# gitouni/Spatial-Temporal-LiDAR-camera-Calibration

Measured on NVIDIA B200. Metric: extrinsic_cost_evals_per_s, higher is better.
Workload: dtype f64

## Files before the change

include/stlcalib.h:

```cpp
#ifndef STLCALIB_H_
#define STLCALIB_H_

#include <stdint.h>

#ifdef __cplusplus
extern "C" {
#endif

#define STL_ABI_VERSION 2
#define STL_MAX_COVIS 10

typedef enum stl_status {
    STL_OK = 0,
    STL_ERR_INVALID = 1,
    STL_ERR_CUDA = 2,
    STL_ERR_NO_DEVICE = 3,
    STL_ERR_STATE = 4,
    STL_ERR_CAPACITY = 5
} stl_status_t;

typedef struct stl_params {
    double max_pixel_dist;
    double corr_3d_2d_threshold;
    double corr_3d_3d_threshold;
// ... 38 lines not shown
    const double *he_Tl;
    const uint8_t *he_valid;
} stl_pack_t;

typedef struct stl_eval_sums {
    double sum_3d2d;
    double sum_3d3d;
    double sum_he;
    double cnt_he;
    double cnt_3d2d;
    double valid_3d2d;
    double cnt_3d3d;
    double valid_3d3d;
    double valid_pl;
    double valid_pt;
    double n_frames;
    double n_corr;
} stl_eval_sums_t;
#define STL_EVAL_NSUMS 12

typedef struct stl_ba_error {
    double f1;
    double f2;
    double C;
    int32_t valid_cnt_3d_2d;
    int32_t cnt_3d_2d;
} stl_ba_error_t;

typedef struct stl_lin_sums {
    double cost;
    double g[7];
    double H[49];
    double n_blocks_2d;
    double n_blocks_pt;
    double n_blocks_pl;
    double n_residuals;
    double n_blocks_gpr;
} stl_lin_sums_t;
#define STL_LIN_NSUMS 62

typedef struct stl_step_sums {
    stl_eval_sums_t eval;
    stl_lin_sums_t lin;
} stl_step_sums_t;
#define STL_STEP_NSUMS (STL_EVAL_NSUMS + STL_LIN_NSUMS)

typedef struct stl_ctx stl_ctx_t;


void stl_default_params(stl_params_t *p);

stl_status_t stl_create(const stl_params_t *params, int32_t device, stl_ctx_t **out);
void stl_destroy(stl_ctx_t *ctx);
const char *stl_last_error(const stl_ctx_t *ctx);
int32_t stl_abi_version(void);

stl_status_t stl_upload_pack(stl_ctx_t *ctx, const stl_pack_t *pack);

stl_status_t stl_allow_oversize_keyframes(stl_ctx_t *ctx, int32_t allow);

stl_status_t stl_oversize_keyframes(stl_ctx_t *ctx, int32_t *kf, int32_t cap, int32_t *n);


stl_status_t stl_eval_batch(stl_ctx_t *ctx, const double *x, int32_t B, stl_eval_sums_t *sums);

stl_status_t stl_eval_batch_device(stl_ctx_t *ctx, const double *x, int32_t B, double *d_sums,
                                   void *stream);

void stl_finalize(const stl_params_t *params, const stl_eval_sums_t *sums, stl_ba_error_t *out);

void stl_bbo(const stl_params_t *params, const stl_ba_error_t *e, double bbo[4]);


stl_status_t stl_associate(stl_ctx_t *ctx, const double *x0, int64_t n_blocks[4]);

stl_status_t stl_linearize_batch(stl_ctx_t *ctx, const double *x, int32_t B, stl_lin_sums_t *out);
stl_status_t stl_linearize_batch_device(stl_ctx_t *ctx, const double *x, int32_t B, double *d_out,
                                        void *stream);

stl_status_t stl_eval_blocks(stl_ctx_t *ctx, const double *x, int32_t rmax, int64_t cap_blocks, int32_t *type, int32_t *kf,
                             int32_t *kp, int32_t *n_res, double *residuals, double *jacobians, int64_t *n_blocks_out);

stl_status_t stl_gpr_nlml(const double *x, const double *y, int32_t n, double sigma_noise, double sigma, double l, int32_t flavour,
                          double *cost, double grad[2]);
stl_status_t stl_gpr_fit(const double *x, const double *y, int32_t n, double sigma_noise, double sigma0, double l0, int32_t max_iter,
                         int32_t flavour, double out[6]);
stl_status_t stl_gpr_hyper(stl_ctx_t *ctx, double *sigma_l, int64_t cap_blocks);

stl_status_t stl_block_counts(stl_ctx_t *ctx, int64_t n_blocks[4]);

#define STL_MAX_PROBLEMS 256

stl_status_t stl_associate_multi(stl_ctx_t *ctx, const double *x0, int32_t P, const uint8_t *rebuild, int64_t *n_blocks);
stl_status_t stl_block_counts_multi(stl_ctx_t *ctx, int64_t *n_blocks, int32_t cap_problems);

stl_status_t stl_linearize_multi(stl_ctx_t *ctx, const double *x, int32_t B, const int32_t *problem, stl_lin_sums_t *out);
stl_status_t stl_linearize_multi_device(stl_ctx_t *ctx, const double *x, int32_t B, const int32_t *problem, double *d_out, void *stream);

stl_status_t stl_step_multi(stl_ctx_t *ctx, const double *x, int32_t P, const uint8_t *rebuild, stl_step_sums_t *out);
stl_status_t stl_step_multi_device(stl_ctx_t *ctx, const double *x, int32_t P, const uint8_t *rebuild, double *d_out, void *stream);

stl_status_t stl_step_batch(stl_ctx_t *ctx, const double *x, int32_t B, int32_t reassociate, stl_step_sums_t *out);
stl_status_t stl_step_batch_device(stl_ctx_t *ctx, const double *x, int32_t B, int32_t reassociate, double *d_out, void *stream);

typedef struct stl_he_edges {
    int32_t n;
    const double *Ta;
    const double *Tb;
    const double *info;
    double huber_delta;
    double regulation;
} stl_he_edges_t;
stl_status_t stl_he_linearize(stl_ctx_t *ctx, const stl_he_edges_t *edges, const double *x, int32_t B, stl_lin_sums_t *out, double *chi2);

typedef struct stl_calib_edges {
    int32_t n_kf;
    int64_t n_edges;
    const int64_t *edge_offset;
    const double *Tlw_quat;
    const float *intrinsics;
    const double *Xw;
    const double *obs;
    const float *inv_sigma2;
    const uint8_t *level;
    double huber_delta;
} stl_calib_edges_t;
stl_status_t stl_calib_linearize(stl_ctx_t *ctx, const stl_calib_edges_t *edges, const double *x, int32_t B, stl_lin_sums_t *out, double *chi2);

#define STL_COMM_ID_BYTES 128
stl_status_t stl_comm_unique_id(uint8_t id[STL_COMM_ID_BYTES]);
stl_status_t stl_comm_init(stl_ctx_t *ctx, const uint8_t id[STL_COMM_ID_BYTES], int32_t rank, int32_t n_ranks);
stl_status_t stl_comm_info(stl_ctx_t *ctx, int32_t *rank, int32_t *n_ranks);
stl_status_t stl_comm_stats(stl_ctx_t *ctx, int64_t out[3]);

stl_status_t stl_select_keyframes(stl_ctx_t *ctx, const int32_t *kf, int32_t n);

stl_status_t stl_eval_frames(stl_ctx_t *ctx, const double *x, int32_t B, double *out);


stl_status_t stl_debug_corrset(stl_ctx_t *ctx, int32_t b, int32_t kf, uint32_t *kp_idx,
                               uint32_t *pt_idx, int32_t cap, int32_t *n);

stl_status_t stl_debug_align(stl_ctx_t *ctx, int32_t b, int32_t kf, uint32_t *kp_idx,
                             uint32_t *nn_idx, int32_t *n_neigh, int32_t *is_plane, double *dist,
                             uint32_t *knn_idx, int32_t cap, int32_t *n);

stl_status_t stl_debug_frame(stl_ctx_t *ctx, int32_t b, int32_t kf, double out[13]);

stl_status_t stl_knn3d(stl_ctx_t *ctx, int32_t kf, const double *q, int32_t nq, int32_t k,
                       double radius2, uint32_t *out_idx, double *out_d2, int32_t *out_count);

stl_status_t stl_debug_trig(stl_ctx_t *ctx, const double *x, int32_t n, double *acos_out, double *cos_out);


#define STL_STAGE_ASSOC2D 0
#define STL_STAGE_KNN3D 1
#define STL_STAGE_REDUCE 2
#define STL_STAGE_LINEARIZE 3
#define STL_STAGE_BUILD 4
#define STL_STAGE_ASSOC_LM 5
#define STL_STAGE_ALLREDUCE 6
#define STL_STAGE_PLANE_INDEX 7
#define STL_NSTAGES 8

stl_status_t stl_set_stream(stl_ctx_t *ctx, void *stream);

stl_status_t stl_set_profiling(stl_ctx_t *ctx, int32_t enabled);
stl_status_t stl_stage_stats(stl_ctx_t *ctx, double ms[STL_NSTAGES], int64_t launches[STL_NSTAGES]);

stl_status_t stl_work_counters(stl_ctx_t *ctx, double out[8]);

#ifdef __cplusplus
}
#endif
#endif
```

spatial-temporal-lidar-camera-calibration_b200/_abi.py:

```python
from __future__ import annotations

import ctypes as C
import os

_HERE = os.path.dirname(os.path.abspath(__file__))

STL_MAX_COVIS = 10
STL_EVAL_NSUMS = 12
STL_LIN_NSUMS = 62
STL_STEP_NSUMS = STL_EVAL_NSUMS + STL_LIN_NSUMS
STL_COMM_ID_BYTES = 128
STL_MAX_PROBLEMS = 256
STL_NSTAGES = 8
STAGE_NAMES = ("assoc2d", "knn3d", "reduce", "linearize", "build", "assoc_lm", "allreduce", "plane_index")

STATUS = {0: "STL_OK", 1: "STL_ERR_INVALID", 2: "STL_ERR_CUDA", 3: "STL_ERR_NO_DEVICE",
          4: "STL_ERR_STATE", 5: "STL_ERR_CAPACITY"}


class StlError(RuntimeError):
    def __init__(self, code: int, msg: str = ""):
        self.code = code
        super().__init__(f"{STATUS.get(code, code)}: {msg}")


class Params(C.Structure):
    _fields_ = [
        ("max_pixel_dist", C.c_double),
        ("corr_3d_2d_threshold", C.c_double),
        ("corr_3d_3d_threshold", C.c_double),
        ("norm_radius", C.c_double),
        ("norm_reg_threshold", C.c_double),
        ("min_diff_dist", C.c_double),
        ("err_weight", C.c_double * 2),
        ("he_threshold", C.c_double),
        ("valid_rate", C.c_double),
        ("max_3d_dist", C.c_double),
        ("robust_kernel_delta", C.c_double),
        ("robust_kernel_3ddelta", C.c_double),
        ("num_min_corr", C.c_int32),
        ("norm_max_pts", C.c_int32),
        ("norm_min_pts", C.c_int32),
        ("use_plane", C.c_int32),
        ("use_gpr", C.c_int32),
        ("gpr_sigma", C.c_double),
        ("gpr_l", C.c_double),
        ("gpr_sigma_noise", C.c_double),
        ("plane_index", C.c_int32),
        ("variant", C.c_int32),
        ("gpr_optimize", C.c_int32),
        ("gpr_grad_flavour", C.c_int32),
    ]


class Pack(C.Structure):
    _fields_ = [
        ("n_kf", C.c_int32),
        ("n_covis", C.c_int32),
        ("scan_offset", C.POINTER(C.c_int64)),
        ("scan_xyz", C.POINTER(C.c_float)),
        ("intrinsics", C.POINTER(C.c_float)),
        ("image_wh", C.POINTER(C.c_int32)),
        ("kp_offset", C.POINTER(C.c_int64)),
        ("kp_xy", C.POINTER(C.c_float)),
        ("kp_mappoint", C.POINTER(C.c_float)),
        ("Tcw", C.POINTER(C.c_float)),
        ("covis_relpose", C.POINTER(C.c_float)),
        ("covis_valid", C.POINTER(C.c_uint8)),
        ("covis_uv", C.POINTER(C.c_float)),
        ("he_Tc", C.POINTER(C.c_float)),
        ("he_Tl", C.POINTER(C.c_double)),
        ("he_valid", C.POINTER(C.c_uint8)),
    ]


class EvalSums(C.Structure):
    _fields_ = [(n, C.c_double) for n in (
        "sum_3d2d", "sum_3d3d", "sum_he", "cnt_he", "cnt_3d2d", "valid_3d2d", "cnt_3d3d",
        "valid_3d3d", "valid_pl", "valid_pt", "n_frames", "n_corr")]


class BAErrorOut(C.Structure):
    _fields_ = [("f1", C.c_double), ("f2", C.c_double), ("C", C.c_double),
                ("valid_cnt_3d_2d", C.c_int32), ("cnt_3d_2d", C.c_int32)]


class LinSums(C.Structure):
    _fields_ = [("cost", C.c_double), ("g", C.c_double * 7), ("H", C.c_double * 49),
                ("n_blocks_2d", C.c_double), ("n_blocks_pt", C.c_double),
                ("n_blocks_pl", C.c_double), ("n_residuals", C.c_double), ("n_blocks_gpr", C.c_double)]


class StepSums(C.Structure):
    _fields_ = [("eval", EvalSums), ("lin", LinSums)]


class HeEdges(C.Structure):
    _fields_ = [("n", C.c_int32), ("Ta", C.POINTER(C.c_double)), ("Tb", C.POINTER(C.c_double)), ("info", C.POINTER(C.c_double)),
                ("huber_delta", C.c_double), ("regulation", C.c_double)]


class CalibEdges(C.Structure):
    _fields_ = [("n_kf", C.c_int32), ("n_edges", C.c_int64), ("edge_offset", C.POINTER(C.c_int64)), ("Tlw_quat", C.POINTER(C.c_double)),
                ("intrinsics", C.POINTER(C.c_float)), ("Xw", C.POINTER(C.c_double)), ("obs", C.POINTER(C.c_double)),
                ("inv_sigma2", C.POINTER(C.c_float)), ("level", C.POINTER(C.c_uint8)), ("huber_delta", C.c_double)]


class SynthCfg(C.Structure):
    _fields_ = [
        ("n_kf", C.c_int32), ("kf_begin", C.c_int32), ("n_kf_total", C.c_int32),
        ("beams", C.c_int32), ("az_steps", C.c_int32), ("n_kp", C.c_int32), ("n_covis", C.c_int32),
        ("width", C.c_int32), ("height", C.c_int32),
        ("fx", C.c_float), ("fy", C.c_float), ("cx", C.c_float), ("cy", C.c_float),
        ("anchored_frac", C.c_double), ("mappoint_frac", C.c_double), ("match_frac", C.c_double),
        ("outlier_frac", C.c_double), ("scale_gt", C.c_double), ("kf_spacing", C.c_double),
        ("max_range", C.c_double), ("elev_top_deg", C.c_double), ("elev_bottom_deg", C.c_double),
        ("x_gt", C.c_double * 7), ("seed", C.c_uint64),
    ]


_vp = C.c_void_p
_dp = C.POINTER(C.c_double)
_u32p = C.POINTER(C.c_uint32)
_i32p = C.POINTER(C.c_int32)
_i64p = C.POINTER(C.c_int64)
_u8p = C.POINTER(C.c_uint8)

CALIB_SYMBOLS = {
    "stl_default_params": (None, [C.POINTER(Params)]),
    "stl_create": (C.c_int, [C.POINTER(Params), C.c_int32, C.POINTER(_vp)]),
    "stl_destroy": (None, [_vp]),
    "stl_last_error": (C.c_char_p, [_vp]),
    "stl_abi_version": (C.c_int32, []),
    "stl_upload_pack": (C.c_int, [_vp, C.POINTER(Pack)]),
    "stl_eval_batch": (C.c_int, [_vp, _dp, C.c_int32, C.POINTER(EvalSums)]),
    "stl_eval_batch_device": (C.c_int, [_vp, _dp, C.c_int32, _vp, _vp]),
    "stl_finalize": (None, [C.POINTER(Params), C.POINTER(EvalSums), C.POINTER(BAErrorOut)]),
    "stl_bbo": (None, [C.POINTER(Params), C.POINTER(BAErrorOut), _dp]),
    "stl_associate": (C.c_int, [_vp, _dp, _i64p]),
    "stl_linearize_batch": (C.c_int, [_vp, _dp, C.c_int32, C.POINTER(LinSums)]),
    "stl_linearize_batch_device": (C.c_int, [_vp, _dp, C.c_int32, _vp, _vp]),
    "stl_eval_blocks": (C.c_int, [_vp, _dp, C.c_int32, C.c_int64, _i32p, _i32p, _i32p, _i32p, _dp, _dp, C.POINTER(C.c_int64)]),
    "stl_block_counts": (C.c_int, [_vp, _i64p]),
    "stl_gpr_nlml": (C.c_int, [_dp, _dp, C.c_int32, C.c_double, C.c_double, C.c_double, C.c_int32, _dp, _dp]),
    "stl_gpr_fit": (C.c_int, [_dp, _dp, C.c_int32, C.c_double, C.c_double, C.c_double, C.c_int32, C.c_int32, _dp]),
    "stl_gpr_hyper": (C.c_int, [_vp, _dp, C.c_int64]),
    "stl_step_batch": (C.c_int, [_vp, _dp, C.c_int32, C.c_int32, C.POINTER(StepSums)]),
    "stl_step_batch_device": (C.c_int, [_vp, _dp, C.c_int32, C.c_int32, _vp, _vp]),
    "stl_associate_multi": (C.c_int, [_vp, _dp, C.c_int32, _u8p, _i64p]),
    "stl_block_counts_multi": (C.c_int, [_vp, _i64p, C.c_int32]),
    "stl_linearize_multi": (C.c_int, [_vp, _dp, C.c_int32, _i32p, C.POINTER(LinSums)]),
    "stl_linearize_multi_device": (C.c_int, [_vp, _dp, C.c_int32, _i32p, _vp, _vp]),
    "stl_step_multi": (C.c_int, [_vp, _dp, C.c_int32, _u8p, C.POINTER(StepSums)]),
    "stl_step_multi_device": (C.c_int, [_vp, _dp, C.c_int32, _u8p, _vp, _vp]),
    "stl_he_linearize": (C.c_int, [_vp, C.POINTER(HeEdges), _dp, C.c_int32, C.POINTER(LinSums), _dp]),
    "stl_calib_linearize": (C.c_int, [_vp, C.POINTER(CalibEdges), _dp, C.c_int32, C.POINTER(LinSums), _dp]),
    "stl_comm_unique_id": (C.c_int, [C.POINTER(C.c_uint8)]),
    "stl_comm_init": (C.c_int, [_vp, C.POINTER(C.c_uint8), C.c_int32, C.c_int32]),
    "stl_comm_info": (C.c_int, [_vp, _i32p, _i32p]),
    "stl_comm_stats": (C.c_int, [_vp, _i64p]),
    "stl_select_keyframes": (C.c_int, [_vp, _i32p, C.c_int32]),
    "stl_eval_frames": (C.c_int, [_vp, _dp, C.c_int32, _dp]),
    "stl_allow_oversize_keyframes": (C.c_int, [_vp, C.c_int32]),
    "stl_oversize_keyframes": (C.c_int, [_vp, _i32p, C.c_int32, _i32p]),
    "stl_debug_corrset": (C.c_int, [_vp, C.c_int32, C.c_int32, _u32p, _u32p, C.c_int32, _i32p]),
    "stl_debug_align": (C.c_int, [_vp, C.c_int32, C.c_int32, _u32p, _u32p, _i32p, _i32p, _dp, _u32p,
                                  C.c_int32, _i32p]),
    "stl_debug_frame": (C.c_int, [_vp, C.c_int32, C.c_int32, _dp]),
    "stl_debug_trig": (C.c_int, [_vp, _dp, C.c_int32, _dp, _dp]),
    "stl_knn3d": (C.c_int, [_vp, C.c_int32, _dp, C.c_int32, C.c_int32, C.c_double, _u32p, _dp, _i32p]),
    "stl_set_stream": (C.c_int, [_vp, _vp]),
    "stl_set_profiling": (C.c_int, [_vp, C.c_int32]),
    "stl_stage_stats": (C.c_int, [_vp, _dp, _i64p]),
    "stl_work_counters": (C.c_int, [_vp, _dp]),
}

SYNTH_SYMBOLS = {
    "stl_synth_default_cfg": (None, [C.POINTER(SynthCfg)]),
    "stl_synth_create": (_vp, [C.POINTER(SynthCfg)]),
    "stl_synth_pack": (C.POINTER(Pack), [_vp]),
    "stl_synth_x_gt": (_dp, [_vp]),
    "stl_synth_Twl": (_dp, [_vp]),
    "stl_synth_destroy": (None, [_vp]),
    "stl_synth_candidates": (None, [_dp, C.c_uint64, C.c_int32, C.c_double, _dp]),
}


def _bind(lib, table):
    for name, (res, args) in table.items():
        fn = getattr(lib, name)
        fn.restype = res
        fn.argtypes = args
    return lib


CALIB_LIB_PATH = os.path.join(_HERE, "libstlcalib.so")
SYNTH_LIB_PATH = os.path.join(_HERE, "libstlsynth.so")

_calib = None
_synth = None


def load_calib():
    global _calib
    if _calib is None:
        if not os.path.exists(CALIB_LIB_PATH):
            raise ImportError(
                f"{CALIB_LIB_PATH} is not built; run `python -c 'import __graft_entry__ as g; g.build()'`."
                " There is no CPU fallback for the cost-evaluation path.")
        _calib = _bind(C.CDLL(CALIB_LIB_PATH), CALIB_SYMBOLS)
    return _calib


def load_synth():
    global _synth
    if _synth is None:
        if not os.path.exists(SYNTH_LIB_PATH):
            raise ImportError(f"{SYNTH_LIB_PATH} is not built; run __graft_entry__.build()")
        _synth = _bind(C.CDLL(SYNTH_LIB_PATH), SYNTH_SYMBOLS)
    return _synth
```

spatial-temporal-lidar-camera-calibration_b200/capi.py:

```python
from __future__ import annotations

import ctypes as C

import numpy as np

from . import _abi
from .pack import KeyFramePack, default_params

_dp = _abi._dp


def _check(lib, h, code):
    if code != 0:
        msg = lib.stl_last_error(h).decode() if h else ""
        raise _abi.StlError(code, msg)


class Context:

    def __init__(self, params: _abi.Params | None = None, device: int = 0):
        self.lib = _abi.load_calib()
        self.params = params if params is not None else default_params()
        h = C.c_void_p()
        code = self.lib.stl_create(C.byref(self.params), device, C.byref(h))
# ... 162 lines not shown
        return nb if wait else None

    def block_counts_multi(self) -> np.ndarray:
        nb = np.zeros((_abi.STL_MAX_PROBLEMS, 4), np.int64)
        _check(self.lib, self.h, self.lib.stl_block_counts_multi(self.h, nb.ctypes.data_as(_abi._i64p), _abi.STL_MAX_PROBLEMS))
        return nb[: self.n_problems].copy()

    def linearize_multi(self, X, problem=None) -> np.ndarray:
        X = np.ascontiguousarray(np.atleast_2d(X), dtype=np.float64)
        B = X.shape[0]
        keep, pp = self._problems(problem, B)
        out = np.empty((B, _abi.STL_LIN_NSUMS), dtype=np.float64)
        _check(self.lib, self.h, self.lib.stl_linearize_multi(self.h, X.ctypes.data_as(_dp), B, pp,
                                                              out.ctypes.data_as(C.POINTER(_abi.LinSums))))
        return out

    def linearize_multi_device(self, X, d_out_ptr: int, problem=None, stream_ptr: int = 0):
        X = np.ascontiguousarray(np.atleast_2d(X), dtype=np.float64)
        keep, pp = self._problems(problem, X.shape[0])
        _check(self.lib, self.h, self.lib.stl_linearize_multi_device(self.h, X.ctypes.data_as(_dp), X.shape[0], pp,
                                                                     C.c_void_p(d_out_ptr), C.c_void_p(stream_ptr)))

    def step_multi(self, X, rebuild=None) -> np.ndarray:
        X = np.ascontiguousarray(np.atleast_2d(X), dtype=np.float64)
        P = X.shape[0]
        keep, m = self._mask(rebuild, P)
        out = np.empty((P, _abi.STL_STEP_NSUMS), dtype=np.float64)
        _check(self.lib, self.h, self.lib.stl_step_multi(self.h, X.ctypes.data_as(_dp), P, m, out.ctypes.data_as(C.POINTER(_abi.StepSums))))
        self.n_blocks = None
        self.n_problems = P
        return out

    def step_multi_device(self, X, d_out_ptr: int, rebuild=None, stream_ptr: int = 0):
        X = np.ascontiguousarray(np.atleast_2d(X), dtype=np.float64)
        keep, m = self._mask(rebuild, X.shape[0])
        _check(self.lib, self.h, self.lib.stl_step_multi_device(self.h, X.ctypes.data_as(_dp), X.shape[0], m,
                                                                C.c_void_p(d_out_ptr), C.c_void_p(stream_ptr)))
        self.n_blocks = None
        self.n_problems = X.shape[0]

    def gpr_hyper(self):
        nb = self.block_counts()
        out = np.zeros((max(int(nb[3]), 1), 2))
        _check(self.lib, self.h, self.lib.stl_gpr_hyper(self.h, out.ctypes.data_as(_dp), int(nb[3])))
        return out[: int(nb[3])]

    def he_linearize(self, edges: "HandEyeEdges", x, want_chi2: bool = False):
        x = np.ascontiguousarray(np.atleast_2d(x), dtype=np.float64)
        B = x.shape[0]
        out = np.zeros((B, _abi.STL_LIN_NSUMS))
        chi2 = np.zeros((B, max(edges.n, 1))) if want_chi2 else None
        c = edges.as_c()
        _check(self.lib, self.h, self.lib.stl_he_linearize(self.h, C.byref(c), x.ctypes.data_as(_dp), B, out.ctypes.data_as(C.POINTER(_abi.LinSums)),
                                                           chi2.ctypes.data_as(_dp) if want_chi2 else None))
        return (out, chi2[:, : edges.n]) if want_chi2 else out

    def calib_linearize(self, edges: "CalibBAEdges", x, want_chi2: bool = False):
        x = np.ascontiguousarray(np.atleast_2d(x), dtype=np.float64)
        B = x.shape[0]
        out = np.zeros((B, _abi.STL_LIN_NSUMS))
        chi2 = np.zeros((B, max(edges.n_edges, 1))) if want_chi2 else None
        c = edges.as_c()
        _check(self.lib, self.h, self.lib.stl_calib_linearize(self.h, C.byref(c), x.ctypes.data_as(_dp), B, out.ctypes.data_as(C.POINTER(_abi.LinSums)),
                                                              chi2.ctypes.data_as(_dp) if want_chi2 else None))
        return (out, chi2[:, : edges.n_edges]) if want_chi2 else out

    def comm_unique_id(self) -> bytes:
        buf = (C.c_uint8 * _abi.STL_COMM_ID_BYTES)()
        _check(self.lib, self.h, self.lib.stl_comm_unique_id(buf))
        return bytes(buf)

    def comm_init(self, uid: bytes, rank: int, n_ranks: int):
        buf = (C.c_uint8 * _abi.STL_COMM_ID_BYTES).from_buffer_copy(uid)
        _check(self.lib, self.h, self.lib.stl_comm_init(self.h, buf, rank, n_ranks))

    def comm_stats(self):
        out = np.zeros(3, np.int64)
        _check(self.lib, self.h, self.lib.stl_comm_stats(self.h, out.ctypes.data_as(_abi._i64p)))
        return dict(p2p=bool(out[0]), p2p_exchanges=int(out[1]), nccl_exchanges=int(out[2]))

    def comm_info(self):
        r, n = C.c_int32(0), C.c_int32(1)
        _check(self.lib, self.h, self.lib.stl_comm_info(self.h, C.byref(r), C.byref(n)))
        return r.value, n.value

    def linearize(self, x) -> np.ndarray:
        x = np.ascontiguousarray(np.atleast_2d(x), dtype=np.float64)
        B = x.shape[0]
        out = np.empty((B, _abi.STL_LIN_NSUMS), dtype=np.float64)
        _check(self.lib, self.h, self.lib.stl_linearize_batch(self.h, x.ctypes.data_as(_dp), B,
                                                              out.ctypes.data_as(C.POINTER(_abi.LinSums))))
        return out

    def linearize_device(self, x, d_out_ptr: int, stream_ptr: int = 0):
        x = np.ascontiguousarray(np.atleast_2d(x), dtype=np.float64)
        _check(self.lib, self.h, self.lib.stl_linearize_batch_device(self.h, x.ctypes.data_as(_dp), x.shape[0],
                                                                     C.c_void_p(d_out_ptr), C.c_void_p(stream_ptr)))

    def eval_blocks(self, x, rmax: int = 0):
        x = np.ascontiguousarray(x, dtype=np.float64).reshape(7)
        ncov = int(self.pack.n_covis) if self.pack is not None else _abi.STL_MAX_COVIS
        rmax = int(rmax) if rmax else max(3, 2 * ncov)
        if getattr(self, "n_blocks", None) is None:
            self.block_counts()
        nb = int(self.n_blocks.sum())
        cap = max(nb, 1)
        out = dict(type=np.zeros(cap, np.int32), kf=np.zeros(cap, np.int32), kp=np.zeros(cap, np.int32), n_res=np.zeros(cap, np.int32),
                   residuals=np.zeros((cap, rmax)), jacobians=np.zeros((cap, rmax, 7)))
        n = C.c_int64(0)
        _check(self.lib, self.h, self.lib.stl_eval_blocks(
            self.h, x.ctypes.data_as(_dp), rmax, cap, out["type"].ctypes.data_as(_abi._i32p), out["kf"].ctypes.data_as(_abi._i32p),
            out["kp"].ctypes.data_as(_abi._i32p), out["n_res"].ctypes.data_as(_abi._i32p), out["residuals"].ctypes.data_as(_dp),
            out["jacobians"].ctypes.data_as(_dp), C.byref(n)))
        return {k: v[: n.value] for k, v in out.items()}

    def debug_corrset(self, b: int, kf: int):
        cap = int(self.pack.kp_offset[kf + 1] - self.pack.kp_offset[kf]) if self.pack is not None else 65536
        kp = np.zeros(max(cap, 1), np.uint32)
        pt = np.zeros(max(cap, 1), np.uint32)
        n = C.c_int32(0)
        _check(self.lib, self.h, self.lib.stl_debug_corrset(self.h, b, kf, kp.ctypes.data_as(_abi._u32p),
                                                            pt.ctypes.data_as(_abi._u32p), cap, C.byref(n)))
        return kp[:n.value], pt[:n.value]

    def debug_align(self, b: int, kf: int):
        cap = int(self.pack.kp_offset[kf + 1] - self.pack.kp_offset[kf]) if self.pack is not None else 65536
        cap = max(cap, 1)
        kp = np.zeros(cap, np.uint32)
        nn = np.zeros(cap, np.uint32)
        m = np.zeros(cap, np.int32)
        pl = np.zeros(cap, np.int32)
        d = np.zeros(cap, np.float64)
        knn = np.zeros((cap, 32), np.uint32)
        n = C.c_int32(0)
        _check(self.lib, self.h, self.lib.stl_debug_align(
            self.h, b, kf, kp.ctypes.data_as(_abi._u32p), nn.ctypes.data_as(_abi._u32p), m.ctypes.data_as(_abi._i32p),
            pl.ctypes.data_as(_abi._i32p), d.ctypes.data_as(_dp), knn.ctypes.data_as(_abi._u32p), cap, C.byref(n)))
        k = n.value
        return dict(kp=kp[:k], nn=nn[:k], m=m[:k], is_plane=pl[:k], dist=d[:k], knn=knn[:k])

    def debug_frame(self, b: int, kf: int):
        out = np.zeros(13)
        _check(self.lib, self.h, self.lib.stl_debug_frame(self.h, b, kf, out.ctypes.data_as(_dp)))
        names = ("sum_3d2d", "valid_3d2d", "cnt_3d2d", "sum_he", "cnt_he", "kept", "n_corr", "n_queries",
                 "sum_3d3d", "valid_3d3d", "cnt_3d3d", "valid_pl", "valid_pt")
        return dict(zip(names, out))

    def debug_trig(self, x):
        x = np.ascontiguousarray(x, dtype=np.float64).reshape(-1)
        a, c = np.zeros_like(x), np.zeros_like(x)
        _check(self.lib, self.h, self.lib.stl_debug_trig(self.h, x.ctypes.data_as(_dp), len(x), a.ctypes.data_as(_dp), c.ctypes.data_as(_dp)))
        return a, c

    def knn3d(self, kf: int, q, k: int, radius2: float = 0.0):
        q = np.ascontiguousarray(q, dtype=np.float64).reshape(-1, 3)
        nq = q.shape[0]
        idx = np.zeros((nq, k), np.uint32)
        d2 = np.zeros((nq, k), np.float64)
        cnt = np.zeros(nq, np.int32)
        _check(self.lib, self.h, self.lib.stl_knn3d(self.h, kf, q.ctypes.data_as(_dp), nq, k, radius2,
                                                    idx.ctypes.data_as(_abi._u32p), d2.ctypes.data_as(_dp),
                                                    cnt.ctypes.data_as(_abi._i32p)))
        return idx, d2, cnt

    def set_stream(self, stream_ptr: int = 0):
        _check(self.lib, self.h, self.lib.stl_set_stream(self.h, C.c_void_p(stream_ptr)))

    def set_profiling(self, on: bool):
        _check(self.lib, self.h, self.lib.stl_set_profiling(self.h, int(on)))

    def stage_stats(self):
        ms = np.zeros(_abi.STL_NSTAGES)
        n = np.zeros(_abi.STL_NSTAGES, np.int64)
        _check(self.lib, self.h, self.lib.stl_stage_stats(self.h, ms.ctypes.data_as(_dp), n.ctypes.data_as(_abi._i64p)))
        return {name: (float(ms[i]), int(n[i])) for i, name in enumerate(_abi.STAGE_NAMES)}

    def work_counters(self):
        out = np.zeros(8)
        _check(self.lib, self.h, self.lib.stl_work_counters(self.h, out.ctypes.data_as(_dp)))
        return dict(points=out[0], q2d=out[1], q3d_nn=out[2], q3d_knn=out[3], k1_bytes=out[4], launches=out[5], k1_overflow_units=out[6],
                    assoc_reused=out[7])


class HandEyeEdges:

    def __init__(self, Ta, Tb, info=None, huber_delta: float = 0.0, regulation: float = 0.0):
        self.Ta = np.ascontiguousarray(Ta, dtype=np.float64).reshape(-1, 12)
        self.Tb = np.ascontiguousarray(Tb, dtype=np.float64).reshape(-1, 12)
        self.n = len(self.Ta)
        self.info = None if info is None else np.ascontiguousarray(info, dtype=np.float64)
        self.huber_delta, self.regulation = float(huber_delta), float(regulation)

    def as_c(self):
        c = _abi.HeEdges(self.n, self.Ta.ctypes.data_as(_dp), self.Tb.ctypes.data_as(_dp),
                         self.info.ctypes.data_as(_dp) if self.info is not None else None, self.huber_delta, self.regulation)
        c._keep = self
        return c


class CalibBAEdges:

    def __init__(self, edge_offset, Tlw_quat, intrinsics, Xw, obs, inv_sigma2, level=None, huber_delta: float = 5.991 ** 0.5):
        self.edge_offset = np.ascontiguousarray(edge_offset, dtype=np.int64)
        self.Tlw_quat = np.ascontiguousarray(Tlw_quat, dtype=np.float64).reshape(-1, 6)
        self.intrinsics = np.ascontiguousarray(intrinsics, dtype=np.float32).reshape(-1, 4)
        self.Xw = np.ascontiguousarray(Xw, dtype=np.float64).reshape(-1, 3)
        self.obs = np.ascontiguousarray(obs, dtype=np.float64).reshape(-1, 2)
        self.inv_sigma2 = np.ascontiguousarray(inv_sigma2, dtype=np.float32)
        self.level = None if level is None else np.ascontiguousarray(level, dtype=np.uint8)
        self.n_kf, self.n_edges = len(self.Tlw_quat), len(self.Xw)
        self.huber_delta = float(huber_delta)

    def as_c(self):
        c = _abi.CalibEdges(self.n_kf, self.n_edges, self.edge_offset.ctypes.data_as(_abi._i64p), self.Tlw_quat.ctypes.data_as(_dp),
                            self.intrinsics.ctypes.data_as(C.POINTER(C.c_float)), self.Xw.ctypes.data_as(_dp), self.obs.ctypes.data_as(_dp),
                            self.inv_sigma2.ctypes.data_as(C.POINTER(C.c_float)),
                            self.level.ctypes.data_as(C.POINTER(C.c_uint8)) if self.level is not None else None, self.huber_delta)
        c._keep = self
        return c


def gpr_nlml(x, y, sigma, l, sigma_noise: float = 1e-10, flavour: int = 0):
    lib = _abi.load_calib()
    x = np.ascontiguousarray(x, dtype=np.float64).reshape(-1, 2)
    y = np.ascontiguousarray(y, dtype=np.float64)
    cost, g = C.c_double(0), np.zeros(2)
    code = lib.stl_gpr_nlml(x.ctypes.data_as(_dp), y.ctypes.data_as(_dp), len(y), sigma_noise, sigma, l, flavour, C.byref(cost), g.ctypes.data_as(_dp))
    if code != 0:
        raise _abi.StlError(code, "Cholesky factorisation of the kernel matrix failed")
    return cost.value, g


def gpr_fit(x, y, sigma0: float = 10.0, l0: float = 10.0, sigma_noise: float = 1e-10, max_iter: int = 15, flavour: int = 0):
    lib = _abi.load_calib()
    x = np.ascontiguousarray(x, dtype=np.float64).reshape(-1, 2)
    y = np.ascontiguousarray(y, dtype=np.float64)
    out = np.zeros(6)
    code = lib.stl_gpr_fit(x.ctypes.data_as(_dp), y.ctypes.data_as(_dp), len(y), sigma_noise, sigma0, l0, max_iter, flavour, out.ctypes.data_as(_dp))
    if code != 0:
        raise _abi.StlError(code, "the objective could not be evaluated at the starting point")
    return dict(sigma=out[0], l=out[1], cost0=out[2], cost=out[3], iterations=int(out[4]), evaluations=int(out[5]))
```

spatial-temporal-lidar-camera-calibration_b200/csrc/build.cu:

```cuda
#include <cub/cub.cuh>

#include "kernels.h"

namespace stl {
namespace {

__device__ __forceinline__ unsigned long long spread16(unsigned v) {
    unsigned long long x = v & 0xffffull;
    x = (x | (x << 16)) & 0x0000ff0000ffull;
    x = (x | (x << 8)) & 0x00f00f00f00full;
    x = (x | (x << 4)) & 0x0c30c30c30c3ull;
    x = (x | (x << 2)) & 0x249249249249ull;
    return x;
}

__global__ void k_bbox(const float *__restrict__ raw, const long long *__restrict__ raw_off, float *__restrict__ bbox, DevKf *kf,
                       int kf_begin) {
    const int f = blockIdx.x;
    const long long b = raw_off[f], e = raw_off[f + 1];
    float lo[3] = {INFINITY, INFINITY, INFINITY}, hi[3] = {-INFINITY, -INFINITY, -INFINITY};
    for (long long i = b + threadIdx.x; i < e; i += blockDim.x) {
#pragma unroll
        for (int a = 0; a < 3; ++a) {
            const float v = raw[i * 3 + a];
            lo[a] = fminf(lo[a], v);
            hi[a] = fmaxf(hi[a], v);
        }
    }
    __shared__ float slo[3][32], shi[3][32];
    const int lane = threadIdx.x & 31, w = threadIdx.x >> 5;
#pragma unroll
    for (int a = 0; a < 3; ++a) {
        for (int o = 16; o; o >>= 1) {
            lo[a] = fminf(lo[a], __shfl_xor_sync(0xffffffffu, lo[a], o));
            hi[a] = fmaxf(hi[a], __shfl_xor_sync(0xffffffffu, hi[a], o));
        }
        if (lane == 0) { slo[a][w] = lo[a]; shi[a][w] = hi[a]; }
    }
    __syncthreads();
    if (threadIdx.x == 0) {
        const int nw = blockDim.x >> 5;
        float pm = 0.f;
        for (int a = 0; a < 3; ++a) {
            float l = slo[a][0], h = shi[a][0];
            for (int i = 1; i < nw; ++i) { l = fminf(l, slo[a][i]); h = fmaxf(h, shi[a][i]); }
            bbox[f * 6 + a] = l;
            bbox[f * 6 + 3 + a] = h;
            pm = fmaxf(pm, fmaxf(fabsf(l), fabsf(h)));
        }
        if (!(pm >= 1.f)) pm = 1.f;
        kf[kf_begin + f].pmax = pm;
    }
}

__global__ void k_morton(const float *__restrict__ raw, const long long *__restrict__ raw_off, const float *__restrict__ bbox,
                         unsigned long long *__restrict__ keys, uint32_t *__restrict__ vals) {
    const int f = blockIdx.y;
    const long long b = raw_off[f], e = raw_off[f + 1];
    const float lx = bbox[f * 6], ly = bbox[f * 6 + 1], lz = bbox[f * 6 + 2];
    float ext = fmaxf(fmaxf(bbox[f * 6 + 3] - lx, bbox[f * 6 + 4] - ly), bbox[f * 6 + 5] - lz);
    if (!(ext > 0.f)) ext = 1.f;
    const float scale = 65535.0f / ext;
    for (long long i = b + (long long)blockIdx.x * blockDim.x + threadIdx.x; i < e; i += (long long)gridDim.x * blockDim.x) {
        const float x = raw[i * 3], y = raw[i * 3 + 1], z = raw[i * 3 + 2];
        const unsigned qx = (unsigned)fminf(fmaxf((x - lx) * scale, 0.f), 65535.f);
        const unsigned qy = (unsigned)fminf(fmaxf((y - ly) * scale, 0.f), 65535.f);
        const unsigned qz = (unsigned)fminf(fmaxf((z - lz) * scale, 0.f), 65535.f);
        const unsigned long long m = spread16(qx) | (spread16(qy) << 1) | (spread16(qz) << 2);
        keys[i] = ((unsigned long long)f << 48) | m;
        vals[i] = (uint32_t)(i - b);
    }
}

__global__ void k_scatter(const float *__restrict__ raw, const long long *__restrict__ raw_off, const uint32_t *__restrict__ vals,
                          const DevKf *__restrict__ kf, int kf_begin, float *__restrict__ px, float *__restrict__ py,
                          float *__restrict__ pz, uint32_t *__restrict__ orig) {
    const int f = blockIdx.y;
    const DevKf K = kf[kf_begin + f];
    const long long b = raw_off[f];
    for (int j = blockIdx.x * blockDim.x + threadIdx.x; j < K.n_pad; j += gridDim.x * blockDim.x) {
        const long long dst = K.pt_off + j;
        if (j < K.n_pts) {
            const uint32_t v = vals[b + j];
            const float *p = raw + (b + v) * 3;
            px[dst] = p[0]; py[dst] = p[1]; pz[dst] = p[2];
            orig[dst] = v;
        } else {
            const float qn = __int_as_float(0x7fc00000);
            px[dst] = qn; py[dst] = qn; pz[dst] = qn;
            orig[dst] = 0xffffffffu;
        }
    }
}


constexpr int kGroup = 8192;
constexpr int kRefThreads = 1024;
constexpr int kGroupLevels = 8;

__device__ __forceinline__ int f2ord(float f) { const int b = __float_as_int(f); return b >= 0 ? b : b ^ 0x7fffffff; }

struct RefineSmem {
    float x[kGroup], y[kGroup], z[kGroup];
    uint32_t o[kGroup];
    float key[kGroup];
    unsigned short perm[kGroup];
    int bb[128][6];
    unsigned char axis[128];
};

__device__ __forceinline__ void cmp_swap(RefineSmem &S, int i, int l) {
    const float ki = S.key[i], kl = S.key[l];
    const unsigned short pi = S.perm[i], pl = S.perm[l];
    if (ki > kl || (ki == kl && pi > pl)) { S.key[i] = kl; S.key[l] = ki; S.perm[i] = pl; S.perm[l] = pi; }
}

__global__ void __launch_bounds__(kRefThreads, 1)
k_kd_refine(const DevKf *__restrict__ kf, int kf_begin, float *__restrict__ px, float *__restrict__ py, float *__restrict__ pz,
            uint32_t *__restrict__ orig) {
    extern __shared__ __align__(16) unsigned char refine_raw[];
    RefineSmem &S = *reinterpret_cast<RefineSmem *>(refine_raw);
    const DevKf K = kf[kf_begin + blockIdx.y];
    const int g0 = blockIdx.x * kGroup;
    if (g0 >= K.n_pad) return;
    const int M = min(kGroup, K.n_pad - g0);
    const long long base = K.pt_off + g0;
    const int tid = threadIdx.x;
    const float qn = __int_as_float(0x7fc00000);
    for (int i = tid; i < kGroup; i += kRefThreads) {
        const bool in = i < M;
        S.x[i] = in ? px[base + i] : qn;
        S.y[i] = in ? py[base + i] : qn;
        S.z[i] = in ? pz[base + i] : qn;
        S.o[i] = in ? orig[base + i] : 0xffffffffu;
        S.perm[i] = (unsigned short)i;
    }
    __syncthreads();
    for (int lev = 0; lev < kGroupLevels; ++lev) {
        const int seg_size = kGroup >> lev, nseg = 1 << lev, seg_shift = 13 - lev;
        for (int i = tid; i < nseg * 6; i += kRefThreads) S.bb[i / 6][i % 6] = (i % 6) < 3 ? 0x7fffffff : (int)0x80000000;
        __syncthreads();
        for (int i = tid; i < kGroup; i += kRefThreads) {
            const int p = S.perm[i];
            const float x = S.x[p];
            if (x == x) {
                const int sg = i >> seg_shift;
                atomicMin(&S.bb[sg][0], f2ord(x)); atomicMax(&S.bb[sg][3], f2ord(x));
                atomicMin(&S.bb[sg][1], f2ord(S.y[p])); atomicMax(&S.bb[sg][4], f2ord(S.y[p]));
                atomicMin(&S.bb[sg][2], f2ord(S.z[p])); atomicMax(&S.bb[sg][5], f2ord(S.z[p]));
            }
        }
        __syncthreads();
        if (tid < nseg) {
            int ax = 0;
            if (S.bb[tid][0] <= S.bb[tid][3]) {
                float e[3];
                for (int a = 0; a < 3; ++a) {
                    const int lo = S.bb[tid][a], hi = S.bb[tid][3 + a];
                    const float fl = __int_as_float(lo >= 0 ? lo : lo ^ 0x7fffffff), fh = __int_as_float(hi >= 0 ? hi : hi ^ 0x7fffffff);
                    e[a] = fh - fl;
                }
                if (e[1] > e[ax]) ax = 1;
                if (e[2] > e[ax]) ax = 2;
            }
            S.axis[tid] = (unsigned char)ax;
        }
        __syncthreads();
        for (int i = tid; i < kGroup; i += kRefThreads) {
            const int p = S.perm[i], ax = S.axis[i >> seg_shift];
            const float v = ax == 0 ? S.x[p] : (ax == 1 ? S.y[p] : S.z[p]);
            S.key[i] = (v == v) ? v : INFINITY;
        }
        __syncthreads();
        for (int k = 2; k <= seg_size; k <<= 1) {
            const int hk = k >> 1;
            for (int p = tid; p < kGroup / 2; p += kRefThreads) {
                const int i = (p / hk) * k + (p % hk);
                cmp_swap(S, i, i ^ (k - 1));
            }
            __syncthreads();
            for (int j = hk >> 1; j > 0; j >>= 1) {
                for (int p = tid; p < kGroup / 2; p += kRefThreads) {
                    const int i = (p / j) * 2 * j + (p % j);
                    cmp_swap(S, i, i + j);
                }
                __syncthreads();
            }
        }
    }
    for (int i = tid; i < M; i += kRefThreads) {
        const int p = S.perm[i];
        px[base + i] = S.x[p]; py[base + i] = S.y[p]; pz[base + i] = S.z[p];
        orig[base + i] = S.o[p];
    }
}

__device__ __forceinline__ void warp_box(float4 &lo, float4 &hi) {
    for (int o = 16; o; o >>= 1) {
        lo.x = fminf(lo.x, __shfl_xor_sync(0xffffffffu, lo.x, o));
        lo.y = fminf(lo.y, __shfl_xor_sync(0xffffffffu, lo.y, o));
        lo.z = fminf(lo.z, __shfl_xor_sync(0xffffffffu, lo.z, o));
        hi.x = fmaxf(hi.x, __shfl_xor_sync(0xffffffffu, hi.x, o));
        hi.y = fmaxf(hi.y, __shfl_xor_sync(0xffffffffu, hi.y, o));
        hi.z = fmaxf(hi.z, __shfl_xor_sync(0xffffffffu, hi.z, o));
    }
}

__global__ void k_leaf_aabb(const DevKf *__restrict__ kf, int kf_begin, const float *__restrict__ px, const float *__restrict__ py,
                            const float *__restrict__ pz, float4 *__restrict__ node_lo, float4 *__restrict__ node_hi) {
    const DevKf K = kf[kf_begin + blockIdx.y];
    const int lane = threadIdx.x & 31;
    const int leaf = blockIdx.x * (blockDim.x >> 5) + (threadIdx.x >> 5);
    if (leaf >= K.n0) return;
    float4 lo = make_float4(INFINITY, INFINITY, INFINITY, 0.f), hi = make_float4(-INFINITY, -INFINITY, -INFINITY, 0.f);
    const int j = leaf * kLeaf + lane;
    if (j < K.n_pts) {
        const long long s = K.pt_off + j;
        lo.x = hi.x = px[s]; lo.y = hi.y = py[s]; lo.z = hi.z = pz[s];
    }
    warp_box(lo, hi);
    if (lane == 0) { node_lo[K.node_off + leaf] = lo; node_hi[K.node_off + leaf] = hi; }
}

__global__ void k_inner_aabb(const DevKf *__restrict__ kf, int kf_begin, int level, float4 *__restrict__ node_lo,
                             float4 *__restrict__ node_hi) {
    const DevKf K = kf[kf_begin + blockIdx.y];
    const int lane = threadIdx.x & 31;
    const int node = blockIdx.x * (blockDim.x >> 5) + (threadIdx.x >> 5);
    const int n_here = level == 1 ? K.n1 : 32;
    if (node >= n_here) return;
    const long long child_base = K.node_off + (level == 1 ? 0 : K.n0);
    const int n_child = level == 1 ? K.n0 : K.n1;
    const long long out_base = K.node_off + (level == 1 ? K.n0 : K.n0 + K.n1);
    float4 lo = make_float4(INFINITY, INFINITY, INFINITY, 0.f), hi = make_float4(-INFINITY, -INFINITY, -INFINITY, 0.f);
    const int c = node * 32 + lane;
    if (c < n_child) { lo = node_lo[child_base + c]; hi = node_hi[child_base + c]; }
    warp_box(lo, hi);
    if (lane == 0) { node_lo[out_base + node] = lo; node_hi[out_base + node] = hi; }
}

constexpr int kAdjCand = 256;

__device__ __forceinline__ float boxbox_lb(float4 alo, float4 ahi, float4 blo, float4 bhi) {
    const float dx = fmaxf(fmaxf(__fsub_rd(blo.x, ahi.x), __fsub_rd(alo.x, bhi.x)), 0.f);
    const float dy = fmaxf(fmaxf(__fsub_rd(blo.y, ahi.y), __fsub_rd(alo.y, bhi.y)), 0.f);
    const float dz = fmaxf(fmaxf(__fsub_rd(blo.z, ahi.z), __fsub_rd(alo.z, bhi.z)), 0.f);
    const float s = __fadd_rd(__fadd_rd(__fmul_rd(dx, dx), __fmul_rd(dy, dy)), __fmul_rd(dz, dz));
    return __fmul_rd(s, 0.99999976f);
}

__device__ __forceinline__ unsigned long long warp_min64(unsigned long long v) {
    for (int o = 16; o; o >>= 1) {
        const unsigned long long w = __shfl_xor_sync(0xffffffffu, v, o);
        v = w < v ? w : v;
    }
    return v;
}

__global__ void __launch_bounds__(256)
k_leaf_adj(const DevKf *__restrict__ kf, int kf_begin, const float4 *__restrict__ node_lo, const float4 *__restrict__ node_hi,
           uint16_t *__restrict__ adj, float *__restrict__ adj_cov, const float r2, const float min_cov) {
    __shared__ unsigned long long cand[8][kAdjCand];
    constexpr unsigned long long kNone = 0xffffffffffffffffull;
    const DevKf K = kf[kf_begin + blockIdx.y];
    const int lane = threadIdx.x & 31, warp = threadIdx.x >> 5;
    const int leaf = blockIdx.x * 8 + warp;
    if (leaf >= K.n0) return;
    const float4 *lo0 = node_lo + K.node_off, *hi0 = node_hi + K.node_off;
    const float4 *lo1 = lo0 + K.n0, *hi1 = hi0 + K.n0, *lo2 = lo1 + K.n1, *hi2 = hi1 + K.n1;
    const float4 alo = lo0[leaf], ahi = hi0[leaf];
    int cnt = 0;
    bool over = !(alo.x <= ahi.x) || K.n0 > 65535;
    if (!over) {
        unsigned m2 = __ballot_sync(0xffffffffu, boxbox_lb(alo, ahi, lo2[lane], hi2[lane]) <= r2);
        while (m2 && !over) {
            const int s2 = __ffs(m2) - 1;
            m2 &= m2 - 1;
            unsigned m1 = __ballot_sync(0xffffffffu, boxbox_lb(alo, ahi, lo1[s2 * 32 + lane], hi1[s2 * 32 + lane]) <= r2);
            while (m1 && !over) {
                const int s1 = __ffs(m1) - 1;
                m1 &= m1 - 1;
                const int n0i = (s2 * 32 + s1) * 32 + lane;
                const float lb = boxbox_lb(alo, ahi, lo0[n0i], hi0[n0i]);
                const unsigned m0 = __ballot_sync(0xffffffffu, lb <= r2);
                const int c = __popc(m0);
                if (cnt + c > kAdjCand) { over = true; break; }
                if ((m0 >> lane) & 1u) cand[warp][cnt + __popc(m0 & ((1u << lane) - 1))] = ((unsigned long long)__float_as_uint(lb) << 32) | (unsigned)n0i;
                cnt += c;
            }
        }
    }
    __syncwarp();
    unsigned long long mine = kNone;
    float cov = -1.f;
    if (!over) {
        for (int t = 0; t <= 32; ++t) {
            unsigned long long best = kNone;
            for (int i = lane; i < cnt; i += 32) best = cand[warp][i] < best ? cand[warp][i] : best;
            best = warp_min64(best);
            if (t == 32) {
                cov = best == kNone ? __int_as_float(0x7f800000) : __uint_as_float((unsigned)(best >> 32));
                break;
            }
            if (best == kNone) { cov = __int_as_float(0x7f800000); break; }
            if (lane == t) mine = best;
            for (int i = lane; i < cnt; i += 32)
                if (cand[warp][i] == best) cand[warp][i] = kNone;
            __syncwarp();
        }
    }
    if (cov >= 0.f && cov < min_cov) { cov = -1.f; mine = kNone; }
    adj[(K.node_off + leaf) * 32 + lane] = mine == kNone ? (uint16_t)0xffffu : (uint16_t)(mine & 0xffffu);
    if (lane == 0) adj_cov[K.node_off + leaf] = cov;
}

}

cudaError_t build_scan_index(const float *d_raw, const long long *h_raw_off, int nkf, int kf_begin, const DevKf *h_kf, DevPack &pack,
                             float adj_r2, cudaStream_t st, BuildScratch &scr, float *kernel_ms) {
    const long long n = h_raw_off[nkf] - h_raw_off[0];
    cudaError_t err = cudaSuccess;
    cudaEvent_t ev0 = nullptr, ev1 = nullptr;
    long long *d_off = nullptr;
    float *d_bbox = nullptr;
    unsigned long long *d_keys = nullptr, *d_keys2 = nullptr;
    uint32_t *d_vals = nullptr, *d_vals2 = nullptr;
    void *d_tmp = nullptr;
    size_t tmp_bytes = 0;
    int max_pad = 0, max_n0 = 0, max_n1 = 0;
    for (int f = 0; f < nkf; ++f) {
        max_pad = max_pad > h_kf[kf_begin + f].n_pad ? max_pad : h_kf[kf_begin + f].n_pad;
        max_n0 = max_n0 > h_kf[kf_begin + f].n0 ? max_n0 : h_kf[kf_begin + f].n0;
        max_n1 = max_n1 > h_kf[kf_begin + f].n1 ? max_n1 : h_kf[kf_begin + f].n1;
    }
    long long *h_rel = (long long *)malloc(sizeof(long long) * (nkf + 1));
    for (int f = 0; f <= nkf; ++f) h_rel[f] = h_raw_off[f] - h_raw_off[0];
#define STL_TRY(x) do { err = (x); if (err != cudaSuccess) goto done; } while (0)
    STL_TRY(scr.need(0, sizeof(long long) * (nkf + 1))); d_off = (long long *)scr.buf[0];
    STL_TRY(cudaMemcpyAsync(d_off, h_rel, sizeof(long long) * (nkf + 1), cudaMemcpyHostToDevice, st));
    STL_TRY(scr.need(1, sizeof(float) * 6 * nkf)); d_bbox = (float *)scr.buf[1];
    if (n > 0) {
        STL_TRY(scr.need(2, sizeof(unsigned long long) * n)); d_keys = (unsigned long long *)scr.buf[2];
        STL_TRY(scr.need(3, sizeof(unsigned long long) * n)); d_keys2 = (unsigned long long *)scr.buf[3];
        STL_TRY(scr.need(4, sizeof(uint32_t) * n)); d_vals = (uint32_t *)scr.buf[4];
        STL_TRY(scr.need(5, sizeof(uint32_t) * n)); d_vals2 = (uint32_t *)scr.buf[5];
    }
    if (n > 0) {
        int kf_bits0 = 1;
        while ((1 << kf_bits0) < nkf) ++kf_bits0;
        STL_TRY(cub::DeviceRadixSort::SortPairs(nullptr, tmp_bytes, d_keys, d_keys2, d_vals, d_vals2, n, 0, 48 + kf_bits0, st));
        STL_TRY(scr.need(6, tmp_bytes)); d_tmp = scr.buf[6];
    }
    if (kernel_ms) {
        STL_TRY(cudaEventCreate(&ev0)); STL_TRY(cudaEventCreate(&ev1));
        STL_TRY(cudaEventRecord(ev0, st));
    }
    k_bbox<<<nkf, 512, 0, st>>>(d_raw, d_off, d_bbox, pack.kf, kf_begin);
    if (n > 0) {
        const int tiles = (max_pad + 256 * 8 - 1) / (256 * 8);
        k_morton<<<dim3(tiles, nkf), 256, 0, st>>>(d_raw, d_off, d_bbox, d_keys, d_vals);
        int kf_bits = 1;
        while ((1 << kf_bits) < nkf) ++kf_bits;
        STL_TRY(cub::DeviceRadixSort::SortPairs(d_tmp, tmp_bytes, d_keys, d_keys2, d_vals, d_vals2, n, 0, 48 + kf_bits, st));
    }
    {
        const int tiles = (max_pad + 256 * 8 - 1) / (256 * 8);
        k_scatter<<<dim3(tiles > 0 ? tiles : 1, nkf), 256, 0, st>>>(d_raw, d_off, d_vals2, pack.kf, kf_begin, pack.px, pack.py, pack.pz,
                                                                    pack.orig);
        if (max_pad > 0) {
            static bool configured = false;
            if (!configured) {
                STL_TRY(cudaFuncSetAttribute(k_kd_refine, cudaFuncAttributeMaxDynamicSharedMemorySize, (int)sizeof(RefineSmem)));
                configured = true;
            }
            k_kd_refine<<<dim3((max_pad + kGroup - 1) / kGroup, nkf), kRefThreads, sizeof(RefineSmem), st>>>(pack.kf, kf_begin, pack.px, pack.py,
                                                                                                          pack.pz, pack.orig);
        }
        k_leaf_aabb<<<dim3((max_n0 + 7) / 8, nkf), 256, 0, st>>>(pack.kf, kf_begin, pack.px, pack.py, pack.pz, pack.node_lo, pack.node_hi);
        k_inner_aabb<<<dim3((max_n1 + 7) / 8, nkf), 256, 0, st>>>(pack.kf, kf_begin, 1, pack.node_lo, pack.node_hi);
        k_inner_aabb<<<dim3(4, nkf), 256, 0, st>>>(pack.kf, kf_begin, 2, pack.node_lo, pack.node_hi);
        if (pack.adj && adj_r2 > 0.f)
            k_leaf_adj<<<dim3((max_n0 + 7) / 8, nkf), 256, 0, st>>>(pack.kf, kf_begin, pack.node_lo, pack.node_hi, pack.adj, pack.adj_cov, adj_r2,
                                                                    adj_r2 * (getenv("STL_ADJ_TRUNC") ? (float)atof(getenv("STL_ADJ_TRUNC")) : 1.f / 9.f));
    }
    STL_TRY(cudaGetLastError());
    if (kernel_ms) STL_TRY(cudaEventRecord(ev1, st));
    STL_TRY(cudaStreamSynchronize(st));
    if (kernel_ms) {
        float ms = 0.f;
        STL_TRY(cudaEventElapsedTime(&ms, ev0, ev1));
        *kernel_ms += ms;
    }
#undef STL_TRY
done:
    if (ev0) cudaEventDestroy(ev0);
    if (ev1) cudaEventDestroy(ev1);
    free(h_rel);
    return err;
}

}
```

spatial-temporal-lidar-camera-calibration_b200/csrc/capi.cu:

```cuda
#include <algorithm>
#include <cfloat>
#include <climits>
#include <cmath>
#include <cstdarg>
#include <cstdio>
#include <cstdlib>
#include <cstring>
#include <mutex>
#include <string>
#include <vector>

#include <nccl.h>

#include "../../include/stlcalib.h"
#include "gprfit.hpp"
#include "hostmath.hpp"
#include "kernels.h"
#include "lm.h"
#include "packlayout.hpp"

using namespace stl;

struct stl_ctx {
    int device = 0;
    stl_params_t params;
    DevParams dpr;
    cudaStream_t own_stream = nullptr;
    cudaStream_t stream = nullptr;
    cudaStream_t last_stream = nullptr;
    cudaEvent_t handoff = nullptr;
    cudaStream_t aux_stream = nullptr;
    cudaEvent_t ev_k1 = nullptr, ev_k2a = nullptr, ev_k3 = nullptr, ev_aux = nullptr;
    long long overlapped_steps = 0;
    long long launches = 0;
    std::mutex mu;
    std::string err;
    bool has_pack = false;
    float adj_r2 = 0.f;
    DevPack pk;
    int n_sm = 0;
    PackLayout lay;
    bool allow_oversize = false;
    OvKf *d_ov = nullptr;
    KfRoute route;
    struct DevRoute {
        int *lists = nullptr;
        int *sel = nullptr;
        int2 *sel_mp = nullptr;
        int cap = 0;
    } d_all, d_sel;
    double *d_frames = nullptr;
    DevWork wk;
    int wk_cap = 0;
    bool dbg_alloc = false;
    double *d_sums = nullptr;
    int d_sums_cap = 0;
    DevCand *h_cand = nullptr;
    double *h_sums = nullptr;
    int h_cap = 0;
    cudaEvent_t h2d_done = nullptr;
    std::vector<double> last_x;
    int dbg_b = -1;
    std::vector<double> wk_x;
    bool wk_has_nn = false;
    long long assoc_reused = 0;
    ncclComm_t comm = nullptr;
    int comm_rank = 0, comm_size = 1;
    bool p2p_on = false;
    unsigned p2p_seq = 0;
    P2pView p2p;
    double *p2p_data = nullptr;
    unsigned *p2p_flag = nullptr;
    long long p2p_exchanges = 0, nccl_exchanges = 0;
    LmState lm;
    double *d_lin = nullptr;
    double *h_lin = nullptr;
    long long lin_cap = 0;
    bool profiling = false;
    struct Ev { cudaEvent_t a, b; int stage; bool count; };
    std::vector<Ev> evs;
    std::vector<cudaEvent_t> ev_pool;
    double stage_ms[STL_NSTAGES] = {0};
    long long stage_n[STL_NSTAGES] = {0};
    double counters[8] = {0};
};

namespace {

stl_status_t fail(stl_ctx *c, stl_status_t code, const char *fmt, ...) {
    char buf[512];
    va_list ap;
    va_start(ap, fmt);
    vsnprintf(buf, sizeof(buf), fmt, ap);
    va_end(ap);
    if (c) c->err = buf;
    return code;
}

cudaStream_t acquire_stream(stl_ctx *c, void *requested) {
    cudaStream_t st = requested ? (cudaStream_t)requested : c->stream;
    if (st != c->last_stream) {
        if (c->last_stream) {
            cudaEventRecord(c->handoff, c->last_stream);
            cudaStreamWaitEvent(st, c->handoff, 0);
        }
        c->last_stream = st;
    }
    return st;
}

#define CK(call)                                                                                          \
    do {                                                                                                  \
        cudaError_t e_ = (call);                                                                          \
        if (e_ != cudaSuccess) return fail(ctx, STL_ERR_CUDA, "%s: %s (%s:%d)", #call, cudaGetErrorString(e_), __FILE__, __LINE__); \
    } while (0)

template <class T> void dfree(T *&p) { if (p) { cudaFree(p); p = nullptr; } }

void free_pack(stl_ctx *c) {
    DevPack &p = c->pk;
    dfree(p.kf); dfree(p.px); dfree(p.py); dfree(p.pz); dfree(p.orig); dfree(p.node_lo); dfree(p.node_hi); dfree(p.adj); dfree(p.adj_cov);
    dfree(p.pl_rec); dfree(p.pl_m);
    dfree(p.k1tab); dfree(p.bitmap); dfree(p.grid_start); dfree(p.grid_kp); dfree(p.kp_xy); dfree(p.kp_xyd); dfree(p.kp_mp); dfree(p.Tcw);
    dfree(p.relpose); dfree(p.covis_valid); dfree(p.covis_uv); dfree(p.he_Tc); dfree(p.he_Tl);
    p = DevPack();
    dfree(c->d_frames); dfree(c->d_ov);
    for (stl_ctx::DevRoute *d : {&c->d_all, &c->d_sel}) { dfree(d->lists); dfree(d->sel); dfree(d->sel_mp); *d = stl_ctx::DevRoute(); }
    c->lay = PackLayout();
    c->route = KfRoute();
    c->has_pack = false;
}
void free_work(stl_ctx *c) {
    DevWork &w = c->wk;
    dfree(w.cand); dfree(w.corr_kp); dfree(w.corr_pt); dfree(w.corr_sp); dfree(w.q_corr); dfree(w.q_kpsp); dfree(w.n_corr); dfree(w.n_q);
    dfree(w.k1_ticket); dfree(w.k1_rec); dfree(w.k1_match); dfree(w.k1_ov_match); dfree(w.k1_surv); dfree(w.k1_cnt); dfree(w.k1_best_d2); dfree(w.k1_best_key);
    dfree(w.frame); dfree(w.align); dfree(w.nn_pos); dfree(w.nn_g2); dfree(w.nb); dfree(w.nbx); dfree(w.nb_m); dfree(w.nb_last); dfree(w.dbg_nn); dfree(w.dbg_m); dfree(w.dbg_plane); dfree(w.dbg_dist); dfree(w.dbg_knn); dfree(w.dbg_stats);
    dfree(w.overflow); dfree(w.k1_clk);
    w = DevWork();
    dfree(c->d_frames);
    c->wk_cap = 0;
    c->dbg_alloc = false;
}

void set_dev_params(stl_ctx *c) {
    const stl_params_t &p = c->params;
    DevParams &d = c->dpr;
    d.max_pixel_dist2 = p.max_pixel_dist * p.max_pixel_dist;
    d.thr2d = p.corr_3d_2d_threshold;
    d.thr3d = p.corr_3d_3d_threshold;
    d.radius2 = p.norm_radius * p.norm_radius;
    d.reg_thr = p.norm_reg_threshold;
    d.min_diff2 = p.min_diff_dist * p.min_diff_dist;
    d.max_3d_dist2 = p.max_3d_dist * p.max_3d_dist;
    d.delta2d = p.robust_kernel_delta;
    d.delta3d = p.robust_kernel_3ddelta;
    d.w0 = p.err_weight[0];
    d.w1 = p.err_weight[1];
    d.num_min_corr = p.num_min_corr;
    d.k = p.norm_max_pts;
    d.min_pts = p.norm_min_pts;
    d.use_plane = p.use_plane;
    d.use_gpr = p.use_gpr; d.plane_index = p.plane_index;
    d.variant = p.variant; d.min_diff = p.min_diff_dist;
    c->adj_r2 = 0.f; d.adj_r = 0.f;
    if (!getenv("STL_NO_ADJ") && p.use_plane && p.norm_radius > 0 && p.norm_radius < 1e3) {
        c->adj_r2 = nextafterf((float)d.radius2, INFINITY);
        d.adj_r = nextafterf((float)sqrt(d.radius2), 0.f);
    }
    d.gpr_sigma = p.gpr_sigma; d.gpr_l = p.gpr_l; d.gpr_noise = p.gpr_sigma_noise;
}

struct StageTimer {
    stl_ctx *c; int stage; cudaStream_t st; cudaEvent_t a = nullptr, b = nullptr; bool count;
    StageTimer(stl_ctx *c_, int s, cudaStream_t st_, bool count_ = true) : c(c_), stage(s), st(st_), count(count_) {
        if (!c->profiling) return;
        auto get = [&]() { cudaEvent_t e; if (c->ev_pool.empty()) cudaEventCreate(&e); else { e = c->ev_pool.back(); c->ev_pool.pop_back(); } return e; };
        a = get(); b = get();
        cudaEventRecord(a, st);
    }
    ~StageTimer() {
        if (!a) return;
        cudaEventRecord(b, st);
        c->evs.push_back({a, b, stage, count});
    }
};

void drain_events(stl_ctx *c) {
    for (auto &e : c->evs) {
        cudaEventSynchronize(e.b);
        float ms = 0;
        if (cudaEventElapsedTime(&ms, e.a, e.b) == cudaSuccess) { c->stage_ms[e.stage] += ms; c->stage_n[e.stage] += e.count ? 1 : 0; }
        c->ev_pool.push_back(e.a);
        c->ev_pool.push_back(e.b);
    }
    c->evs.clear();
}

P2pView p2p_view(stl_ctx *ctx, int B, int off, int width) {
    P2pView v;
    if (!ctx->p2p_on || B > kP2pMaxB || width > kP2pWidth) return v;
    v = ctx->p2p;
    v.seq = ++ctx->p2p_seq;
    v.off = off; v.width = width;
    ctx->p2p_exchanges += 1;
    return v;
}

stl_status_t ensure_work(stl_ctx *ctx, int B, bool debug) {
    const DevPack &pk = ctx->pk;
    if (ctx->wk_cap == 0) {
        size_t free_b = 0, total_b = 0;
        CK(cudaMemGetInfo(&free_b, &total_b));
        const size_t per_cand = (size_t)pk.n_kp_total * 24 + (size_t)pk.n_mp_total * (20 * kMaxK + 16) + (size_t)pk.n_kf * (sizeof(FrameRec) + 4 * sizeof(AlignRec) + 24) + (size_t)pk.n_ov_match * sizeof(ulonglong2) + (size_t)pk.n_ov_surv * 4 + (size_t)pk.n_kp_total * 16 + sizeof(DevCand);
        size_t budget = std::min<size_t>((size_t)12 << 30, free_b / 4);
        int cap = (int)std::max<size_t>(1, std::min<size_t>(budget / std::max<size_t>(per_cand, 1), 256));
        if (const char *e = getenv("STL_MAX_CHUNK")) cap = std::max(1, std::min(cap, atoi(e)));
        DevWork &w = ctx->wk;
        w.Bc = cap;
        w.sub = 4;
        if (getenv("STL_SUB")) w.sub = std::max(1, std::min(16, atoi(getenv("STL_SUB"))));
        const size_t nk = (size_t)std::max<long long>(pk.n_kp_total, 1) * cap, nf = (size_t)pk.n_kf * cap;
        const size_t nm = (size_t)std::max<long long>(pk.n_mp_total, 1) * cap;
        auto alloc_all = [&]() -> cudaError_t {
            cudaError_t e;
#define A_(p, bytes) do { e = cudaMalloc(&(p), (bytes)); if (e != cudaSuccess) return e; } while (0)
            A_(w.cand, sizeof(DevCand) * cap);
            A_(w.corr_kp, 4 * nk); A_(w.corr_pt, 4 * nk); A_(w.corr_sp, 4 * nk); A_(w.q_corr, 4 * nk); A_(w.q_kpsp, 8 * nk);
            A_(w.n_corr, 4 * nf); A_(w.n_q, 4 * nf);
            if (ctx->lay.n_fit > 0) {
                w.k1_slots = 2 * std::max(ctx->n_sm, 1);
                A_(w.k1_match, sizeof(ulonglong2) * kK1MatchCap * (size_t)w.k1_slots);
                A_(w.k1_rec, sizeof(float4) * kK1SurvCap * (size_t)w.k1_slots);
                A_(w.k1_ticket, 8);
                e = cudaMemsetAsync(w.k1_ticket, 0, 8, ctx->last_stream); if (e != cudaSuccess) return e;
            }
            if (pk.n_ov > 0) {
                const size_t c = (size_t)cap;
                A_(w.k1_ov_match, sizeof(ulonglong2) * (size_t)pk.n_ov_match * c); A_(w.k1_surv, 4 * (size_t)pk.n_ov_surv * c);
                A_(w.k1_cnt, 16 * (size_t)pk.n_ov * c);
                A_(w.k1_best_d2, 8 * (size_t)std::max<long long>(pk.n_ov_kp, 1) * c); A_(w.k1_best_key, 8 * (size_t)std::max<long long>(pk.n_ov_kp, 1) * c);
            }
            A_(w.frame, sizeof(FrameRec) * nf); A_(w.align, sizeof(AlignRec) * nf * w.sub);
            A_(w.nn_pos, 4 * nm); A_(w.nn_g2, 4 * nm); A_(w.nb, 4 * nm * kMaxK); A_(w.nbx, sizeof(float4) * nm * kMaxK); A_(w.nb_m, 4 * nm); A_(w.nb_last, 8 * nm);
            w.nbx_stride = (long long)nm;
            if (getenv("STL_K1_CLK")) { A_(w.k1_clk, 64 * nf); e = cudaMemsetAsync(w.k1_clk, 0, 64 * nf, ctx->last_stream); if (e != cudaSuccess) return e; }
            A_(w.overflow, 4);
#undef A_
            return cudaMemsetAsync(w.overflow, 0, 4, ctx->last_stream);
        };
        const cudaError_t e = alloc_all();
        if (e != cudaSuccess) {
            free_work(ctx);
            return fail(ctx, STL_ERR_CUDA, "workspace allocation: %s", cudaGetErrorString(e));
        }
        ctx->wk_cap = cap;
    }
    if (debug && !ctx->dbg_alloc) {
        DevWork &w = ctx->wk;
        const size_t nk = (size_t)std::max<long long>(pk.n_kp_total, 1);
        cudaError_t e = cudaMalloc(&w.dbg_nn, 4 * nk);
        if (e == cudaSuccess) e = cudaMalloc(&w.dbg_m, 4 * nk);
        if (e == cudaSuccess) e = cudaMalloc(&w.dbg_plane, 4 * nk);
        if (e == cudaSuccess) e = cudaMalloc(&w.dbg_dist, 8 * nk);
        if (e == cudaSuccess) e = cudaMalloc(&w.dbg_knn, 4 * nk * kMaxK);
        if (e == cudaSuccess) e = cudaMalloc(&w.dbg_stats, 64);
        if (e == cudaSuccess) e = cudaMemsetAsync(w.dbg_stats, 0, 64, ctx->last_stream);
        if (e != cudaSuccess) {
            dfree(w.dbg_nn); dfree(w.dbg_m); dfree(w.dbg_plane); dfree(w.dbg_dist); dfree(w.dbg_knn); dfree(w.dbg_stats);
            return fail(ctx, STL_ERR_CUDA, "debug workspace allocation: %s", cudaGetErrorString(e));
        }
        ctx->dbg_alloc = true;
    }
    if (B > ctx->h_cap) {
        if (ctx->h_cand) cudaFreeHost(ctx->h_cand);
// ... 175 lines not shown

void use_route(stl_ctx *c, KfRoute &&r) {
    const stl_ctx::DevRoute &d = r.all ? c->d_all : c->d_sel;
    DevPack &pk = c->pk;
    pk.sel = r.all ? nullptr : d.sel; pk.sel_mp = r.all ? nullptr : d.sel_mp;
    pk.n_sel = r.n_sel; pk.n_sel_mp = r.n_sel_mp;
    pk.ov_sel = d.lists ? d.lists + pk.n_kf : nullptr; pk.n_ov_sel = r.n_ov;
    c->route = std::move(r);
}

void drop_selection_state(stl_ctx *c) {
    c->lm.ready = false;
    c->wk_x.clear();
    c->wk_has_nn = false;
    c->last_x.clear();
    c->dbg_b = -1;
}

bool kf_selected(const stl_ctx *c, int kf) { return c->route.mask[(size_t)kf] != 0; }

stl_status_t run_debug(stl_ctx *ctx, int b) {
    if (!ctx->has_pack) return fail(ctx, STL_ERR_STATE, "no pack uploaded");
    if (b < 0 || (size_t)b * 7 + 7 > ctx->last_x.size()) return fail(ctx, STL_ERR_INVALID, "candidate %d was not part of the last batch", b);
    if (ctx->dbg_b == b) return STL_OK;
    std::vector<double> keep = ctx->last_x;
    double xb[7];
    memcpy(xb, &keep[(size_t)b * 7], sizeof(xb));
    stl_status_t s = ensure_work(ctx, 1, true);
    if (s != STL_OK) return s;
    cudaStream_t st = acquire_stream(ctx, nullptr);
    s = enqueue_eval(ctx, xb, 1, ctx->d_sums, st, true);
    ctx->last_x = keep;
    if (s != STL_OK) return s;
    CK(cudaStreamSynchronize(st));
    ctx->dbg_b = b;
    return STL_OK;
}

}

extern "C" {

int32_t stl_abi_version(void) { return STL_ABI_VERSION; }

void stl_default_params(stl_params_t *p) {
    memset(p, 0, sizeof(*p));
    p->max_pixel_dist = 1.5; p->corr_3d_2d_threshold = 40.0; p->corr_3d_3d_threshold = 10.0;
    p->norm_radius = 0.6; p->norm_reg_threshold = 0.02; p->min_diff_dist = 0.2;
    p->err_weight[0] = 1.0; p->err_weight[1] = 1.0;
    p->he_threshold = 0.094; p->valid_rate = 0.95;
    p->max_3d_dist = 1.0; p->robust_kernel_delta = 2.98; p->robust_kernel_3ddelta = 1.0;
    p->num_min_corr = 30; p->norm_max_pts = 30; p->norm_min_pts = 5; p->use_plane = 1;
    p->use_gpr = 0; p->gpr_sigma = 10.0; p->gpr_l = 10.0; p->gpr_sigma_noise = 1e-10;
    p->plane_index = 1; p->variant = 0;
    p->gpr_optimize = 0; p->gpr_grad_flavour = 0;
}

stl_status_t stl_create(const stl_params_t *params, int32_t device, stl_ctx_t **out) {
    if (!out || !params) return STL_ERR_INVALID;
    *out = nullptr;
    int n = 0;
    if (cudaGetDeviceCount(&n) != cudaSuccess || n <= 0 || device < 0 || device >= n) { cudaGetLastError(); return STL_ERR_NO_DEVICE; }
    cudaDeviceProp prop;
    if (cudaGetDeviceProperties(&prop, device) != cudaSuccess) return STL_ERR_NO_DEVICE;
    if (prop.major != 10 || prop.minor != 0) return STL_ERR_NO_DEVICE;
    if (params->norm_max_pts < 1 || params->norm_max_pts > kMaxK) return STL_ERR_CAPACITY;
    if (params->variant != 0 && params->variant != 1) return STL_ERR_INVALID;
    if (cudaSetDevice(device) != cudaSuccess) return STL_ERR_CUDA;
    stl_ctx *c = new stl_ctx();
    c->device = device;
    c->params = *params;
    set_dev_params(c);
    if (cudaStreamCreateWithFlags(&c->own_stream, cudaStreamNonBlocking) != cudaSuccess) { delete c; return STL_ERR_CUDA; }
    c->stream = c->own_stream;
    c->last_stream = c->own_stream;
    cudaEventCreateWithFlags(&c->handoff, cudaEventDisableTiming);
    *out = c;
    return STL_OK;
}

void stl_destroy(stl_ctx_t *c) {
    if (!c) return;
    cudaSetDevice(c->device);
    cudaDeviceSynchronize();
    for (int q = 0; q < kP2pMaxRanks; ++q) {
        if (q != c->comm_rank && c->p2p.data[q]) cudaIpcCloseMemHandle(c->p2p.data[q]);
        if (q != c->comm_rank && c->p2p.flag[q]) cudaIpcCloseMemHandle(c->p2p.flag[q]);
    }
    dfree(c->p2p_data); dfree(c->p2p_flag); dfree(c->p2p.err);
    if (c->comm) { ncclCommDestroy(c->comm); c->comm = nullptr; }
    drain_events(c);
    for (auto e : c->ev_pool) cudaEventDestroy(e);
    free_work(c);
    free_pack(c);
    lm_free(c->lm);
    dfree(c->d_sums); dfree(c->d_lin);
    if (c->h_cand) cudaFreeHost(c->h_cand);
    if (c->h_sums) cudaFreeHost(c->h_sums);
    if (c->h_lin) cudaFreeHost(c->h_lin);
    if (c->h2d_done) cudaEventDestroy(c->h2d_done);
    if (c->handoff) cudaEventDestroy(c->handoff);
    if (c->aux_stream) cudaStreamDestroy(c->aux_stream);
    for (cudaEvent_t e : {c->ev_k1, c->ev_k2a, c->ev_k3, c->ev_aux}) if (e) cudaEventDestroy(e);
    if (c->own_stream) cudaStreamDestroy(c->own_stream);
    delete c;
}

const char *stl_last_error(const stl_ctx_t *c) { return c ? c->err.c_str() : "null context"; }

stl_status_t stl_upload_pack(stl_ctx_t *ctx, const stl_pack_t *p) {
    if (!ctx || !p) return STL_ERR_INVALID;
    std::lock_guard<std::mutex> lk(ctx->mu);
    CK(cudaSetDevice(ctx->device));
    K1Limits lim;
    CK(cudaDeviceGetAttribute(&lim.smem_optin, cudaDevAttrMaxSharedMemoryPerBlockOptin, ctx->device));
    lim.k1_smem = assoc2d_smem_bytes;
    lim.split_smem = assoc2d_split_smem_bytes;
    lim.allow_oversize = ctx->allow_oversize;
    const char *route_env = getenv("STL_K1_OVERSIZE");
    lim.route_all = (route_env && strcmp(route_env, "all") == 0) || getenv("STL_K1_SPLIT");
    PackLayout lay;
    const stl_status_t s = layout_pack(p, lim, lay, ctx->err);
    if (s != STL_OK) return s;
    if (lay.n_fit > 0) CK(assoc2d_configure(lay.k1_smem));
    if (!lay.ov.empty()) CK(assoc2d_split_configure(lay.k1_split_smem));

    free_work(ctx);
    free_pack(ctx);
    lm_free(ctx->lm);
    ctx->lay = std::move(lay);
    const PackLayout &L = ctx->lay;
    std::vector<DevKf> &hk = ctx->lay.kf;
    const int F = L.n_kf, C = L.n_covis;
    const long long NK = L.n_kp_total;
    CK(cudaDeviceGetAttribute(&ctx->n_sm, cudaDevAttrMultiProcessorCount, ctx->device));
    cudaStream_t st = acquire_stream(ctx, nullptr);
    struct Scope {
        cudaEvent_t ev0 = nullptr, ev1 = nullptr; float *d_raw = nullptr; BuildScratch scr;
        ~Scope() { if (ev0) cudaEventDestroy(ev0); if (ev1) cudaEventDestroy(ev1); if (d_raw) cudaFree(d_raw); scr.release(); }
    } scope;
    CK(cudaEventCreate(&scope.ev0)); CK(cudaEventCreate(&scope.ev1));
    cudaEvent_t ev0 = scope.ev0, ev1 = scope.ev1;
    CK(cudaEventRecord(ev0, st));
    PackTables tab;
    build_tables(p, L, ctx->params.variant, ctx->params.max_pixel_dist, tab);
    KfRoute all = route_keyframes(L, nullptr, 0);

    DevPack &pk = ctx->pk;
    pk.n_kf = F; pk.n_covis = C; pk.n_pad_total = L.n_pad_total; pk.n_nodes_total = L.n_nodes_total; pk.n_kp_total = NK; pk.n_mp_total = L.n_mp_total;
    const long long nodes = L.n_nodes_total;
    const size_t npt = (size_t)std::max<long long>(L.n_pad_total, 4), nkk = (size_t)std::max<long long>(NK, 1);
    CK(cudaMalloc(&pk.kf, sizeof(DevKf) * F));
    CK(cudaMalloc(&pk.px, 4 * npt)); CK(cudaMalloc(&pk.py, 4 * npt)); CK(cudaMalloc(&pk.pz, 4 * npt)); CK(cudaMalloc(&pk.orig, 4 * npt));
    CK(cudaMalloc(&pk.node_lo, sizeof(float4) * nodes)); CK(cudaMalloc(&pk.node_hi, sizeof(float4) * nodes));
    if (ctx->adj_r2 > 0.f) { CK(cudaMalloc(&pk.adj, sizeof(uint16_t) * 32 * (size_t)nodes)); CK(cudaMalloc(&pk.adj_cov, sizeof(float) * (size_t)nodes)); }
    CK(cudaMalloc(&pk.k1tab, tab.k1tab.size()));
    CK(cudaMemcpyAsync(pk.k1tab, tab.k1tab.data(), tab.k1tab.size(), cudaMemcpyHostToDevice, st));
    CK(cudaMalloc(&pk.bitmap, 4 * (size_t)L.bm_words)); CK(cudaMalloc(&pk.grid_start, 4 * (size_t)L.grid_cells)); CK(cudaMalloc(&pk.grid_kp, 4 * nkk));
    CK(cudaMalloc(&pk.kp_xy, sizeof(float2) * nkk)); CK(cudaMalloc(&pk.kp_mp, 12 * nkk));
    CK(cudaMalloc(&pk.Tcw, 48 * (size_t)F)); CK(cudaMalloc(&pk.relpose, 48 * (size_t)std::max(F * C, 1)));
    CK(cudaMalloc(&pk.covis_valid, (size_t)std::max(F * C, 1))); CK(cudaMalloc(&pk.covis_uv, sizeof(float2) * std::max<size_t>(nkk * C, 1)));
    CK(cudaMalloc(&pk.he_Tc, 48 * (size_t)F)); CK(cudaMalloc(&pk.he_Tl, 96 * (size_t)F));
    CK(cudaMemcpyAsync(pk.kf, hk.data(), sizeof(DevKf) * F, cudaMemcpyHostToDevice, st));
    CK(cudaMemcpyAsync(pk.bitmap, tab.bitmap.data(), 4 * (size_t)L.bm_words, cudaMemcpyHostToDevice, st));
    CK(cudaMemcpyAsync(pk.grid_start, tab.grid_start.data(), 4 * (size_t)L.grid_cells, cudaMemcpyHostToDevice, st));
    if (NK > 0) {
        CK(cudaMemcpyAsync(pk.grid_kp, tab.grid_kp.data(), 4 * (size_t)NK, cudaMemcpyHostToDevice, st));
        CK(cudaMemcpyAsync(pk.kp_xy, tab.kp_xy, 8 * (size_t)NK, cudaMemcpyHostToDevice, st));
        if (ctx->params.variant == 1) {
            CK(cudaMalloc(&pk.kp_xyd, sizeof(double2) * nkk));
            CK(cudaMemcpyAsync(pk.kp_xyd, tab.kp_xyd.data(), 16 * (size_t)NK, cudaMemcpyHostToDevice, st));
        }
        CK(cudaMemcpyAsync(pk.kp_mp, p->kp_mappoint, 12 * (size_t)NK, cudaMemcpyHostToDevice, st));
        if (C > 0) CK(cudaMemcpyAsync(pk.covis_uv, p->covis_uv, 8 * (size_t)NK * C, cudaMemcpyHostToDevice, st));
    }
    CK(cudaMemcpyAsync(pk.Tcw, p->Tcw, 48 * (size_t)F, cudaMemcpyHostToDevice, st));
    if (C > 0) {
        CK(cudaMemcpyAsync(pk.relpose, p->covis_relpose, 48 * (size_t)F * C, cudaMemcpyHostToDevice, st));
        CK(cudaMemcpyAsync(pk.covis_valid, p->covis_valid, (size_t)F * C, cudaMemcpyHostToDevice, st));
    }
    CK(cudaMemcpyAsync(pk.he_Tc, p->he_Tc, 48 * (size_t)F, cudaMemcpyHostToDevice, st));
    CK(cudaMemcpyAsync(pk.he_Tl, p->he_Tl, 96 * (size_t)F, cudaMemcpyHostToDevice, st));
    if (!L.ov.empty()) {
        const int n_ov = (int)L.ov.size();
        pk.n_ov = n_ov; pk.n_ov_kp = L.n_ov_kp; pk.n_ov_surv = L.n_ov_surv; pk.n_ov_match = L.n_ov_match;
        CK(cudaMalloc(&ctx->d_ov, sizeof(OvKf) * (size_t)n_ov));
        CK(cudaMemcpyAsync(ctx->d_ov, L.ov.data(), sizeof(OvKf) * (size_t)n_ov, cudaMemcpyHostToDevice, st));
        pk.ov = ctx->d_ov;
        CK(cudaMalloc(&ctx->d_all.lists, sizeof(int) * 2 * (size_t)F));
        CK(cudaMalloc(&ctx->d_sel.lists, sizeof(int) * 2 * (size_t)F));
        CK(cudaMemcpyAsync(ctx->d_all.lists, all.lists.data(), sizeof(int) * 2 * (size_t)F, cudaMemcpyHostToDevice, st));
    }
    CK(cudaStreamSynchronize(st));

    {
        const long long chunk_pts = 32ll << 20;
        float *&d_raw = scope.d_raw;
        float k0_ms = 0.f;
        long long raw_cap = 0;
        int f0 = 0;
        while (f0 < F) {
            int f1 = f0 + 1;
            while (f1 < F && p->scan_offset[f1 + 1] - p->scan_offset[f0] <= chunk_pts && f1 - f0 < 32768) ++f1;
            const long long n = p->scan_offset[f1] - p->scan_offset[f0];
            if (n > raw_cap) { dfree(d_raw); raw_cap = std::max(n, std::min(chunk_pts, (long long)p->scan_offset[F])); CK(cudaMalloc(&d_raw, 12 * (size_t)std::max<long long>(raw_cap, 1))); }
            if (n > 0) CK(cudaMemcpyAsync(d_raw, p->scan_xyz + p->scan_offset[f0] * 3, 12 * (size_t)n, cudaMemcpyHostToDevice, st));
            std::vector<long long> off(f1 - f0 + 1);
            for (int f = f0; f <= f1; ++f) off[f - f0] = p->scan_offset[f];
            cudaError_t e = build_scan_index(d_raw, off.data(), f1 - f0, f0, hk.data(), pk, ctx->adj_r2, st, scope.scr, &k0_ms);
            if (e != cudaSuccess) return fail(ctx, STL_ERR_CUDA, "index build: %s", cudaGetErrorString(e));
            f0 = f1;
        }
        dfree(d_raw);
        ctx->stage_ms[STL_STAGE_BUILD] += k0_ms;
        ctx->stage_n[STL_STAGE_BUILD] += 1;
    }
    CK(cudaMemcpy(hk.data(), pk.kf, sizeof(DevKf) * F, cudaMemcpyDeviceToHost));
    if (pk.adj && getenv("STL_DEBUG_STATS")) {
        long long real = 0, empty = 0, entries = 0, partial = 0;
        double cov_sum = 0;
        std::vector<uint16_t> row;
        std::vector<float> cov;
        for (int f = 0; f < F; f += std::max(1, F / 16)) {
            const int nl = (hk[f].n_pts + kLeaf - 1) / kLeaf;
            row.resize((size_t)nl * 32);
            CK(cudaMemcpy(row.data(), pk.adj + hk[f].node_off * 32, row.size() * 2, cudaMemcpyDeviceToHost));
            cov.resize((size_t)nl);
            CK(cudaMemcpy(cov.data(), pk.adj_cov + hk[f].node_off, cov.size() * 4, cudaMemcpyDeviceToHost));
            for (int l = 0; l < nl; ++l) if (cov[l] >= 0 && cov[l] < 1e30f) { ++partial; cov_sum += std::sqrt((double)cov[l]); }
            for (int l = 0; l < nl; ++l) {
                int c = 0;
                for (int t = 0; t < 32; ++t) c += row[(size_t)l * 32 + t] != 0xffffu;
                ++real; empty += c == 0; entries += c;
            }
        }
        fprintf(stderr, "[stl] leaf adjacency (sampled keyframes): %lld leaves, %.2f%% without a row, %.1f neighbours per row, %.1f%% truncated (mean coverage %.3f m)\n", real,
                100.0 * empty / std::max<long long>(real, 1), (double)entries / std::max<long long>(real - empty, 1),
                100.0 * partial / std::max<long long>(real, 1), cov_sum / std::max<long long>(partial, 1));
    }
    if (ctx->params.plane_index) {
        CK(cudaMalloc(&pk.pl_rec, sizeof(PlaneRec) * npt));
        CK(cudaMalloc(&pk.pl_m, 4 * npt));
        CK(cudaEventRecord(ev0, st));
        for (int f0 = 0; f0 < F;) {
            int f1 = f0 + 1;
            long long pts = hk[f0].n_pad;
            while (f1 < F && pts + hk[f1].n_pad <= (4ll << 20)) pts += hk[f1++].n_pad;
            cudaError_t e = build_plane_index(pk, hk.data(), f0, f1 - f0, ctx->dpr, st, scope.scr);
            if (e != cudaSuccess) return fail(ctx, STL_ERR_CUDA, "plane index: %s", cudaGetErrorString(e));
            f0 = f1;
        }
        CK(cudaEventRecord(ev1, st));
        CK(cudaStreamSynchronize(st));
        float ms = 0;
        CK(cudaEventElapsedTime(&ms, ev0, ev1));
        ctx->stage_ms[STL_STAGE_PLANE_INDEX] += ms;
        ctx->stage_n[STL_STAGE_PLANE_INDEX] += 1;
    }
    use_route(ctx, std::move(all));
    ctx->has_pack = true;
    return STL_OK;
}

stl_status_t stl_eval_batch_device(stl_ctx_t *ctx, const double *x, int32_t B, double *d_sums, void *stream) {
    if (!ctx || !x || !d_sums || B <= 0) return STL_ERR_INVALID;
    std::lock_guard<std::mutex> lk(ctx->mu);
    if (!ctx->has_pack) return fail(ctx, STL_ERR_STATE, "stl_upload_pack has not been called");
    CK(cudaSetDevice(ctx->device));
    cudaStream_t st = acquire_stream(ctx, stream);
    bool done = false;
    stl_status_t s = enqueue_eval(ctx, x, B, d_sums, st, false, STL_EVAL_NSUMS, true, &done);
    if (s != STL_OK || done) return s;
    return allreduce_record(ctx, d_sums, (size_t)B * STL_EVAL_NSUMS, st);
}

stl_status_t stl_eval_batch(stl_ctx_t *ctx, const double *x, int32_t B, stl_eval_sums_t *sums) {
    if (!ctx || !x || !sums || B <= 0) return STL_ERR_INVALID;
    std::lock_guard<std::mutex> lk(ctx->mu);
    if (!ctx->has_pack) return fail(ctx, STL_ERR_STATE, "stl_upload_pack has not been called");
    CK(cudaSetDevice(ctx->device));
    stl_status_t s = ensure_work(ctx, B, false);
    if (s != STL_OK) return s;
    cudaStream_t st = acquire_stream(ctx, nullptr);
    bool done = false;
    s = enqueue_eval(ctx, x, B, ctx->d_sums, st, false, STL_EVAL_NSUMS, true, &done);
    if (s != STL_OK) return s;
    if (!done) s = allreduce_record(ctx, ctx->d_sums, (size_t)B * STL_EVAL_NSUMS, st);
    if (s != STL_OK) return s;
    CK(cudaMemcpyAsync(ctx->h_sums, ctx->d_sums, sizeof(double) * STL_EVAL_NSUMS * B, cudaMemcpyDeviceToHost, st));
    CK(cudaStreamSynchronize(st));
    memcpy(sums, ctx->h_sums, sizeof(double) * STL_EVAL_NSUMS * B);
    double q3 = 0;
    for (int b = 0; b < B; ++b) q3 += sums[b].cnt_3d3d;
    set_query_counters(ctx, q3);
    return STL_OK;
}

void stl_finalize(const stl_params_t *pr, const stl_eval_sums_t *s, stl_ba_error_t *o) {
    if (s->valid_3d2d == 0 && pr->err_weight[0] > 1e-10) o->f1 = DBL_MAX; else o->f1 = s->sum_3d2d / s->valid_3d2d;
    if (s->valid_3d3d == 0 && pr->err_weight[1] > 1e-10) o->f2 = DBL_MAX; else o->f2 = s->sum_3d3d / s->valid_3d3d;
    o->C = s->sum_he / s->cnt_he;
    o->valid_cnt_3d_2d = (int32_t)s->valid_3d2d;
    o->cnt_3d_2d = (int32_t)s->cnt_3d2d;
}

void stl_bbo(const stl_params_t *pr, const stl_ba_error_t *e, double bbo[4]) {
// ... 56 lines not shown
    std::lock_guard<std::mutex> lk(ctx->mu);
    CK(cudaSetDevice(ctx->device));
    stl_status_t s = run_debug(ctx, b);
    if (s != STL_OK) return s;
    if (kf < 0 || kf >= ctx->pk.n_kf) return fail(ctx, STL_ERR_INVALID, "keyframe out of range");
    if (!kf_selected(ctx, kf)) { for (int i = 0; i < 13; ++i) out[i] = 0; return STL_OK; }
    FrameRec r;
    CK(cudaMemcpy(&r, ctx->wk.frame + kf, sizeof(r), cudaMemcpyDeviceToHost));
    std::vector<AlignRec> a(ctx->wk.sub);
    CK(cudaMemcpy(a.data(), ctx->wk.align + (size_t)kf * ctx->wk.sub, sizeof(AlignRec) * ctx->wk.sub, cudaMemcpyDeviceToHost));
    out[0] = r.s2d; out[1] = r.v2d; out[2] = r.c2d; out[3] = r.she; out[4] = r.che; out[5] = r.kept; out[6] = r.ncorr; out[7] = r.nq;
    for (int i = 8; i < 13; ++i) out[i] = 0;
    if (ctx->wk.k1_clk) {
        std::vector<long long> h((size_t)ctx->pk.n_kf * 8);
        cudaMemcpy(h.data(), ctx->wk.k1_clk, 64 * (size_t)ctx->pk.n_kf, cudaMemcpyDeviceToHost);
        double a[8] = {0};
        for (int f = 0; f < ctx->pk.n_kf; ++f) for (int i = 0; i < 8; ++i) a[i] += (double)h[(size_t)f * 8 + i] / ctx->pk.n_kf;
        fprintf(stderr, "[stl] K1 mean clocks/unit: prologue %.0f | cells + table wait %.0f | stream %.0f | exact-1 %.0f | tie pass %.0f | corrset + covisible term %.0f | reduction %.0f | epilogue %.0f\n", a[7], a[0], a[1], a[2], a[3], a[4], a[5], a[6]);
    }
    if (getenv("STL_DEBUG_STATS")) {
        unsigned long long st[8];
        cudaMemcpy(st, ctx->wk.dbg_stats, 64, cudaMemcpyDeviceToHost);
        if (st[0] + st[4]) fprintf(stderr, "[stl] K2a search paths (cumulative): k-NN %llu = adjacency %.1f%% + restart %.1f%% + no row %.1f%% | 1-NN %llu = adjacency %.1f%% + descent after scan %.1f%% + no row %.1f%%\n",
                st[0], 100.0 * st[1] / std::max(st[0], 1ull), 100.0 * st[2] / std::max(st[0], 1ull), 100.0 * st[3] / std::max(st[0], 1ull),
                st[4], 100.0 * st[5] / std::max(st[4], 1ull), 100.0 * st[6] / std::max(st[4], 1ull), 100.0 * st[7] / std::max(st[4], 1ull));
    }
    for (auto &x : a) { out[8] += x.s3d; out[9] += x.v3d; out[10] += x.c3d; out[11] += x.vpl; out[12] += x.vpt; }
    return STL_OK;
}

stl_status_t stl_select_keyframes(stl_ctx_t *ctx, const int32_t *kf, int32_t n) {
    if (!ctx) return STL_ERR_INVALID;
    std::lock_guard<std::mutex> lk(ctx->mu);
    if (!ctx->has_pack) return fail(ctx, STL_ERR_STATE, "stl_upload_pack has not been called");
    const int F = ctx->pk.n_kf;
    if (kf) {
        if (n < 0 || n > F) return fail(ctx, STL_ERR_INVALID, "stl_select_keyframes: n = %d is outside [0, n_kf = %d]", n, F);
        for (int i = 0; i < n; ++i) {
            if (kf[i] < 0 || kf[i] >= F) return fail(ctx, STL_ERR_INVALID, "stl_select_keyframes: kf[%d] = %d is outside [0, %d)", i, kf[i], F);
            if (i > 0 && kf[i] <= kf[i - 1]) return fail(ctx, STL_ERR_INVALID, "stl_select_keyframes: the list is not strictly increasing at %d", i);
        }
    }
    CK(cudaSetDevice(ctx->device));
    cudaStream_t st = acquire_stream(ctx, nullptr);
    CK(cudaStreamSynchronize(st));
    drop_selection_state(ctx);
    use_route(ctx, route_keyframes(ctx->lay, nullptr, 0));
    if (!kf) return STL_OK;
    KfRoute r = route_keyframes(ctx->lay, kf, n);
    stl_ctx::DevRoute &d = ctx->d_sel;
    cudaError_t e = cudaSuccess;
    if (n > d.cap || !d.sel) {
        dfree(d.sel); dfree(d.sel_mp);
        d.cap = 0;
        const size_t cap = (size_t)std::max(n, 1);
        e = cudaMalloc(&d.sel, sizeof(int) * cap);
        if (e == cudaSuccess) e = cudaMalloc(&d.sel_mp, sizeof(int2) * (cap + 1));
        if (e == cudaSuccess) d.cap = (int)cap;
        else { dfree(d.sel); dfree(d.sel_mp); }
    }
    if (e == cudaSuccess && n > 0) e = cudaMemcpyAsync(d.sel, r.sel.data(), sizeof(int) * (size_t)n, cudaMemcpyHostToDevice, st);
    if (e == cudaSuccess) e = cudaMemcpyAsync(d.sel_mp, r.sel_mp.data(), sizeof(int2) * ((size_t)n + 1), cudaMemcpyHostToDevice, st);
    if (e == cudaSuccess && d.lists) e = cudaMemcpyAsync(d.lists, r.lists.data(), sizeof(int) * 2 * (size_t)F, cudaMemcpyHostToDevice, st);
    if (e == cudaSuccess) e = cudaStreamSynchronize(st);
    if (e != cudaSuccess) return fail(ctx, STL_ERR_CUDA, "stl_select_keyframes: %s (every keyframe stays selected)", cudaGetErrorString(e));
    use_route(ctx, std::move(r));
    return STL_OK;
}

stl_status_t stl_allow_oversize_keyframes(stl_ctx_t *ctx, int32_t allow) {
    if (!ctx) return STL_ERR_INVALID;
    std::lock_guard<std::mutex> lk(ctx->mu);
    if (allow != 0 && allow != 1) return fail(ctx, STL_ERR_INVALID, "stl_allow_oversize_keyframes: allow = %d is neither 0 nor 1", allow);
    ctx->allow_oversize = allow != 0;
    return STL_OK;
}

stl_status_t stl_oversize_keyframes(stl_ctx_t *ctx, int32_t *kf, int32_t cap, int32_t *n) {
    if (!ctx || !n || cap < 0) return STL_ERR_INVALID;
    std::lock_guard<std::mutex> lk(ctx->mu);
    if (!ctx->has_pack) return fail(ctx, STL_ERR_STATE, "stl_upload_pack has not been called");
    *n = (int32_t)ctx->lay.ov.size();
    const int m = std::min(*n, cap);
    if (kf) for (int i = 0; i < m; ++i) kf[i] = ctx->lay.ov[(size_t)i].f;
    return STL_OK;
}

stl_status_t stl_eval_frames(stl_ctx_t *ctx, const double *x, int32_t B, double *out) {
    if (!ctx || !x || !out || B <= 0) return STL_ERR_INVALID;
    std::lock_guard<std::mutex> lk(ctx->mu);
    if (!ctx->has_pack) return fail(ctx, STL_ERR_STATE, "stl_upload_pack has not been called");
    CK(cudaSetDevice(ctx->device));
    stl_status_t s = ensure_work(ctx, B, false);
    if (s != STL_OK) return s;
    const int F = ctx->pk.n_kf, Bc = ctx->wk.Bc;
    const size_t row = (size_t)F * 13;
    if (!ctx->d_frames) CK(cudaMalloc(&ctx->d_frames, sizeof(double) * row * Bc));
    cudaStream_t st = acquire_stream(ctx, nullptr);
    for (int c0 = 0; c0 < B; c0 += Bc) {
        const int nb = std::min(Bc, B - c0);
        s = enqueue_eval(ctx, x + (size_t)c0 * 7, nb, ctx->d_sums, st, false);
        if (s != STL_OK) return s;
        CK(cudaMemsetAsync(ctx->d_frames, 0, sizeof(double) * row * nb, st));
        CK(launch_frames(ctx->pk, ctx->wk, ctx->dpr, nb, ctx->d_frames, st));
        ctx->launches += 1;
        CK(cudaMemcpyAsync(out + row * c0, ctx->d_frames, sizeof(double) * row * nb, cudaMemcpyDeviceToHost, st));
    }
    CK(cudaStreamSynchronize(st));
    set_eval_counters(ctx, B);
    double q3 = 0;
    for (size_t r = 0; r < (size_t)B * F; ++r) q3 += out[r * 13 + 10];
    set_query_counters(ctx, q3);
    ctx->last_x.assign(x, x + (size_t)B * 7);
    return STL_OK;
}

stl_status_t stl_knn3d(stl_ctx_t *ctx, int32_t kf, const double *q, int32_t nq, int32_t k, double radius2, uint32_t *out_idx, double *out_d2,
                       int32_t *out_count) {
    if (!ctx || !q || nq < 0 || k < 1 || k > kMaxK) return STL_ERR_INVALID;
    std::lock_guard<std::mutex> lk(ctx->mu);
    if (!ctx->has_pack) return fail(ctx, STL_ERR_STATE, "no pack uploaded");
    if (kf < 0 || kf >= ctx->pk.n_kf) return fail(ctx, STL_ERR_INVALID, "keyframe out of range");
    if (nq == 0) return STL_OK;
    CK(cudaSetDevice(ctx->device));
    double *dq = nullptr, *dd = nullptr; uint32_t *di = nullptr; int *dc = nullptr;
    CK(cudaMalloc(&dq, 24 * (size_t)nq)); CK(cudaMalloc(&dd, 8 * (size_t)nq * k)); CK(cudaMalloc(&di, 4 * (size_t)nq * k)); CK(cudaMalloc(&dc, 4 * (size_t)nq));
    cudaStream_t st = acquire_stream(ctx, nullptr);
    CK(cudaMemcpyAsync(dq, q, 24 * (size_t)nq, cudaMemcpyHostToDevice, st));
    cudaError_t e = launch_knn3d(ctx->pk, kf, dq, nq, k, radius2, di, dd, dc, st);
    if (e == cudaSuccess && out_idx) e = cudaMemcpyAsync(out_idx, di, 4 * (size_t)nq * k, cudaMemcpyDeviceToHost, st);
    if (e == cudaSuccess && out_d2) e = cudaMemcpyAsync(out_d2, dd, 8 * (size_t)nq * k, cudaMemcpyDeviceToHost, st);
    if (e == cudaSuccess && out_count) e = cudaMemcpyAsync(out_count, dc, 4 * (size_t)nq, cudaMemcpyDeviceToHost, st);
    if (e == cudaSuccess) e = cudaStreamSynchronize(st);
    cudaFree(dq); cudaFree(dd); cudaFree(di); cudaFree(dc);
    if (e != cudaSuccess) return fail(ctx, STL_ERR_CUDA, "knn3d: %s", cudaGetErrorString(e));
    return STL_OK;
}

stl_status_t stl_debug_trig(stl_ctx_t *ctx, const double *x, int32_t n, double *acos_out, double *cos_out) {
    if (!ctx || !x || !acos_out || !cos_out || n < 0) return STL_ERR_INVALID;
    std::lock_guard<std::mutex> lk(ctx->mu);
    CK(cudaSetDevice(ctx->device));
    if (n == 0) return STL_OK;
    double *d = nullptr;
    CK(cudaMalloc(&d, 24 * (size_t)n));
    cudaStream_t st = acquire_stream(ctx, nullptr);
    cudaError_t e = cudaMemcpyAsync(d, x, 8 * (size_t)n, cudaMemcpyHostToDevice, st);
    if (e == cudaSuccess) e = launch_debug_trig(d, n, d + n, d + 2 * (size_t)n, st);
    if (e == cudaSuccess) e = cudaMemcpyAsync(acos_out, d + n, 8 * (size_t)n, cudaMemcpyDeviceToHost, st);
    if (e == cudaSuccess) e = cudaMemcpyAsync(cos_out, d + 2 * (size_t)n, 8 * (size_t)n, cudaMemcpyDeviceToHost, st);
    if (e == cudaSuccess) e = cudaStreamSynchronize(st);
    cudaFree(d);
    if (e != cudaSuccess) return fail(ctx, STL_ERR_CUDA, "debug_trig: %s", cudaGetErrorString(e));
    return STL_OK;
}


static stl_status_t check_set_args(stl_ctx *ctx, const char *call, int P, const uint8_t *rebuild) {
    if (P < 1) return fail(ctx, STL_ERR_INVALID, "%s: P = %d", call, P);
    if (P > STL_MAX_PROBLEMS) return fail(ctx, STL_ERR_CAPACITY, "%s: P = %d exceeds STL_MAX_PROBLEMS = %d", call, P, STL_MAX_PROBLEMS);
    if (rebuild && (!ctx->lm.ready || ctx->lm.P != P))
        return fail(ctx, STL_ERR_INVALID, "%s: a rebuild mask needs P equal to the size of the frozen set (%d)", call, ctx->lm.ready ? ctx->lm.P : 0);
    if (!ctx->has_pack) return fail(ctx, STL_ERR_STATE, "stl_upload_pack has not been called");
    if (ctx->params.variant != 0)
        return fail(ctx, STL_ERR_STATE, "%s follows iba_local.cpp, which has no iba_global_stable variant: create the context with variant = 0", call);
    const long long ns = std::max<long long>(ctx->pk.n_mp_total, 1);
    if ((long long)P * ((ns + 15) / 16 * 16) > INT_MAX) return fail(ctx, STL_ERR_CAPACITY, "%s: %d problems of %lld block slots", call, P, ns);
    return STL_OK;
}

static stl_status_t check_problems(stl_ctx *ctx, int B, const int32_t *problem, std::vector<int> &out) {
    if (!ctx->lm.ready) return fail(ctx, STL_ERR_STATE, "stl_associate_multi has not been called");
    const int P = ctx->lm.P;
    if (!problem && B != P) return fail(ctx, STL_ERR_INVALID, "problem = NULL needs B = P (B = %d, P = %d)", B, P);
    out.resize(B);
    for (int b = 0; b < B; ++b) {
        out[b] = problem ? problem[b] : b;
        if (out[b] < 0 || out[b] >= P) return fail(ctx, STL_ERR_INVALID, "problem[%d] = %d is outside [0, %d)", b, out[b], P);
    }
    return STL_OK;
}

stl_status_t stl_associate_multi(stl_ctx_t *ctx, const double *x0, int32_t P, const uint8_t *rebuild, int64_t *n_blocks) {
    if (!ctx || !x0) return STL_ERR_INVALID;
    std::lock_guard<std::mutex> lk(ctx->mu);
    stl_status_t s = check_set_args(ctx, P == 1 && !rebuild ? "stl_associate" : "stl_associate_multi", P, rebuild);
    if (s != STL_OK) return s;
    CK(cudaSetDevice(ctx->device));
    s = ensure_work(ctx, 1, false);
    if (s != STL_OK) return s;
    cudaStream_t st = acquire_stream(ctx, nullptr);
    s = enqueue_associate(ctx, x0, P, rebuild, st);
    if (s != STL_OK) return s;
    if (n_blocks) {
        const cudaError_t e = lm_block_counts(ctx->lm);
        if (e != cudaSuccess) return fail(ctx, STL_ERR_CUDA, "associate: %s", cudaGetErrorString(e));
        for (int i = 0; i < 4 * P; ++i) n_blocks[i] = ctx->lm.n_blocks[i];
    }
    return STL_OK;
}

stl_status_t stl_associate(stl_ctx_t *ctx, const double *x0, int64_t n_blocks[4]) { return stl_associate_multi(ctx, x0, 1, nullptr, n_blocks); }

static stl_status_t block_counts_locked(stl_ctx *ctx, int64_t *n_blocks, int cap_problems) {
    if (!ctx->lm.ready) return fail(ctx, STL_ERR_STATE, "stl_associate has not been called");
    if (cap_problems < ctx->lm.P) return fail(ctx, STL_ERR_CAPACITY, "%d problems, room for %d", ctx->lm.P, cap_problems);
    CK(cudaSetDevice(ctx->device));
    const cudaError_t e = lm_block_counts(ctx->lm);
    if (e != cudaSuccess) return fail(ctx, STL_ERR_CUDA, "block counts: %s", cudaGetErrorString(e));
    for (int i = 0; i < 4 * ctx->lm.P; ++i) n_blocks[i] = ctx->lm.n_blocks[i];
    return STL_OK;
}

stl_status_t stl_block_counts_multi(stl_ctx_t *ctx, int64_t *n_blocks, int32_t cap_problems) {
    if (!ctx || !n_blocks) return STL_ERR_INVALID;
    std::lock_guard<std::mutex> lk(ctx->mu);
    return block_counts_locked(ctx, n_blocks, cap_problems);
}

stl_status_t stl_block_counts(stl_ctx_t *ctx, int64_t n_blocks[4]) {
    if (!ctx || !n_blocks) return STL_ERR_INVALID;
    std::lock_guard<std::mutex> lk(ctx->mu);
    const stl_status_t s = need_single(ctx, "stl_block_counts", "stl_block_counts_multi");
    return s != STL_OK ? s : block_counts_locked(ctx, n_blocks, 1);
}

static stl_status_t lin_enqueue(stl_ctx *ctx, const double *x, const int *problem, int B, double *d_out, cudaStream_t st, int out_stride = STL_LIN_NSUMS,
                                int exch_off = 0, int exch_width = 0, bool *exchanged = nullptr, cudaEvent_t before_finish = nullptr, bool cand_staged = false) {
    if (!ctx->lm.ready) return fail(ctx, STL_ERR_STATE, "stl_associate has not been called");
    cudaError_t e;
    const P2pView pv = exch_width > 0 ? p2p_view(ctx, B, exch_off, exch_width) : P2pView();
    if (exchanged) *exchanged = pv.n > 1;
    { StageTimer t(ctx, STL_STAGE_LINEARIZE, st); e = lm_linearize(ctx->pk, ctx->dpr, ctx->lm, x, problem, B, d_out, st, nullptr, out_stride, &pv, before_finish, cand_staged); }
    if (e != cudaSuccess) return fail(ctx, STL_ERR_CUDA, "linearize: %s", cudaGetErrorString(e));
    ctx->launches += 2 + (ctx->lm.use_gpr ? 1 : 0);
    return STL_OK;
}

static stl_status_t ensure_lin(stl_ctx *ctx, int B, int width) {
    if ((long long)B * width > ctx->lin_cap) {
        dfree(ctx->d_lin);
        if (ctx->h_lin) cudaFreeHost(ctx->h_lin);
        ctx->h_lin = nullptr;
        ctx->lin_cap = 0;
        CK(cudaMalloc(&ctx->d_lin, sizeof(double) * width * B));
        CK(cudaMallocHost(&ctx->h_lin, sizeof(double) * width * B));
        ctx->lin_cap = (long long)B * width;
    }
    return STL_OK;
}

static stl_status_t step_enqueue(stl_ctx *ctx, const double *x, int B, int reassociate, double *d_out, cudaStream_t st) {
    stl_status_t s = ensure_work(ctx, B, false);
    if (s != STL_OK) return s;
    const bool overlap = reassociate && B <= ctx->wk.Bc && ctx->dpr.plane_index && !ctx->dpr.use_gpr &&
                         !getenv("STL_NO_ASSOC_REUSE") && !getenv("STL_NO_OVERLAP");
    if (overlap) {
        if (!ctx->aux_stream) {
            CK(cudaStreamCreateWithFlags(&ctx->aux_stream, cudaStreamNonBlocking));
            CK(cudaEventCreateWithFlags(&ctx->ev_k1, cudaEventDisableTiming)); CK(cudaEventCreateWithFlags(&ctx->ev_k2a, cudaEventDisableTiming));
            CK(cudaEventCreateWithFlags(&ctx->ev_k3, cudaEventDisableTiming)); CK(cudaEventCreateWithFlags(&ctx->ev_aux, cudaEventDisableTiming));
        }
        cudaStream_t ax = ctx->aux_stream;
        {
            const cudaError_t e = lm_reserve(ctx->pk, ctx->dpr, ctx->lm, 1, 1, st);
            if (e != cudaSuccess) return fail(ctx, STL_ERR_CUDA, "association buffers: %s", cudaGetErrorString(e));
        }
        s = enqueue_eval(ctx, x, B, d_out, st, false, STL_STEP_NSUMS, false, nullptr, true);
        if (s != STL_OK) return s;
        CK(cudaStreamWaitEvent(ax, ctx->ev_k1, 0));
        {
            const cudaError_t e = lm_stage_candidates(ctx->lm, x, nullptr, B, ax);
            if (e != cudaSuccess) return fail(ctx, STL_ERR_CUDA, "candidate staging: %s", cudaGetErrorString(e));
        }
        s = enqueue_associate(ctx, x, 1, nullptr, ax, ctx->ev_k2a);
        bool done = false;
        if (s == STL_OK) s = lin_enqueue(ctx, x, nullptr, B, d_out + STL_EVAL_NSUMS, ax, STL_STEP_NSUMS, -STL_EVAL_NSUMS, STL_STEP_NSUMS, &done, ctx->ev_k3, true);
        if (s == STL_OK && lm_copy_counts(ctx->lm, ax) != cudaSuccess) s = fail(ctx, STL_ERR_CUDA, "block-count read-back");
        cudaEventRecord(ctx->ev_aux, ax);
        cudaStreamWaitEvent(st, ctx->ev_aux, 0);
        if (s != STL_OK) return s;
        ctx->overlapped_steps += 1;
        ctx->last_x.assign(x, x + (size_t)B * 7);
        return done ? STL_OK : allreduce_record(ctx, d_out, (size_t)B * STL_STEP_NSUMS, st);
    }
    s = enqueue_eval(ctx, x, B, d_out, st, false, STL_STEP_NSUMS);
    if (s != STL_OK) return s;
    if (reassociate) {
        s = enqueue_associate(ctx, x, 1, nullptr, st);
        if (s != STL_OK) return s;
    }
    bool done = false;
    s = lin_enqueue(ctx, x, nullptr, B, d_out + STL_EVAL_NSUMS, st, STL_STEP_NSUMS, -STL_EVAL_NSUMS, STL_STEP_NSUMS, &done);
    if (s != STL_OK) return s;
    ctx->last_x.assign(x, x + (size_t)B * 7);
    return done ? STL_OK : allreduce_record(ctx, d_out, (size_t)B * STL_STEP_NSUMS, st);
}

stl_status_t stl_step_batch_device(stl_ctx_t *ctx, const double *x, int32_t B, int32_t reassociate, double *d_out, void *stream) {
    if (!ctx || !x || !d_out || B <= 0) return STL_ERR_INVALID;
    std::lock_guard<std::mutex> lk(ctx->mu);
    if (!ctx->has_pack) return fail(ctx, STL_ERR_STATE, "stl_upload_pack has not been called");
    if (ctx->params.variant != 0) return fail(ctx, STL_ERR_STATE, "stl_step_batch needs variant = 0 (iba_local.cpp has no iba_global_stable variant)");
    if (!reassociate && !ctx->lm.ready) return fail(ctx, STL_ERR_STATE, "stl_step_batch without reassociate needs a previous association");
    if (!reassociate && need_single(ctx, "stl_step_batch", "stl_step_multi") != STL_OK) return STL_ERR_STATE;
    CK(cudaSetDevice(ctx->device));
// ... 349 lines not shown
```

spatial-temporal-lidar-camera-calibration_b200/csrc/kernels.h:

```cpp
#pragma once
#include <cstddef>
#include <cstdint>
#include <cuda_runtime.h>

#include "common.cuh"
#include "p2p.cuh"

namespace stl {

struct OvKf {
    int f;
    int surv_cap;
    int match_cap;
    int n_bands;
    long long kp_off;
    long long surv_off;
    long long match_off;
};

struct DevPack {
    int n_kf = 0, n_covis = 0;
    long long n_pad_total = 0, n_nodes_total = 0, n_kp_total = 0, n_mp_total = 0;
    DevKf *kf = nullptr;
    float *px = nullptr, *py = nullptr, *pz = nullptr;
    uint32_t *orig = nullptr;
    float4 *node_lo = nullptr, *node_hi = nullptr;
    uint16_t *adj = nullptr;
    float *adj_cov = nullptr;
    PlaneRec *pl_rec = nullptr;
    int *pl_m = nullptr;
    uint8_t *k1tab = nullptr;
    uint32_t *bitmap = nullptr;
    uint32_t *grid_start = nullptr;
    uint32_t *grid_kp = nullptr;
    float2 *kp_xy = nullptr;
    double2 *kp_xyd = nullptr;
    float *kp_mp = nullptr;
    float *Tcw = nullptr;
    float *relpose = nullptr;
    uint8_t *covis_valid = nullptr;
    float2 *covis_uv = nullptr;
    float *he_Tc = nullptr;
    double *he_Tl = nullptr;
    int n_sel = 0;
    const int *sel = nullptr;
    const int2 *sel_mp = nullptr;
    long long n_sel_mp = 0;
    int n_ov = 0;
    const OvKf *ov = nullptr;
    long long n_ov_kp = 0, n_ov_surv = 0, n_ov_match = 0;
    int n_ov_sel = 0;
    const int *ov_sel = nullptr;
};

#ifdef __CUDACC__
__device__ __forceinline__ int sel_kf(const DevPack &pk, int i) { return pk.sel ? pk.sel[i] : i; }
#endif

struct DevWork {
    int Bc = 0;
    int sub = 4;
    DevCand *cand = nullptr;
    uint32_t *corr_kp = nullptr;
    uint32_t *corr_pt = nullptr;
    uint32_t *corr_sp = nullptr;
    uint32_t *q_corr = nullptr;
    uint2 *q_kpsp = nullptr;
    int *n_corr = nullptr;
    int *n_q = nullptr;
    FrameRec *frame = nullptr;
    AlignRec *align = nullptr;
    uint32_t *nn_pos = nullptr;
    float *nn_g2 = nullptr;
    uint32_t *nb = nullptr;
    float4 *nbx = nullptr;
    long long nbx_stride = 0;
    int *nb_m = nullptr;
    double *nb_last = nullptr;
    uint32_t *dbg_nn = nullptr;
    int *dbg_m = nullptr;
    int *dbg_plane = nullptr;
    double *dbg_dist = nullptr;
    uint32_t *dbg_knn = nullptr;
    unsigned long long *dbg_stats = nullptr;
    int k1_slots = 0;
    int *k1_ticket = nullptr;
    float4 *k1_rec = nullptr;
    ulonglong2 *k1_match = nullptr;
    ulonglong2 *k1_ov_match = nullptr;
    uint32_t *k1_surv = nullptr;
    int *k1_cnt = nullptr;
    unsigned long long *k1_best_d2 = nullptr;
    unsigned long long *k1_best_key = nullptr;
    long long *k1_clk = nullptr;
    int *overflow = nullptr;
};

struct BuildScratch {
    void *buf[8] = {nullptr, nullptr, nullptr, nullptr, nullptr, nullptr, nullptr, nullptr};
    size_t cap[8] = {0, 0, 0, 0, 0, 0, 0, 0};
    cudaError_t need(int i, size_t bytes) {
        if (bytes <= cap[i]) return cudaSuccess;
        if (buf[i]) cudaFree(buf[i]);
        buf[i] = nullptr; cap[i] = 0;
        const cudaError_t e = cudaMalloc(&buf[i], bytes);
        if (e == cudaSuccess) cap[i] = bytes;
        return e;
    }
    void release() {
        for (int i = 0; i < 8; ++i) { if (buf[i]) cudaFree(buf[i]); buf[i] = nullptr; cap[i] = 0; }
    }
};

cudaError_t build_scan_index(const float *d_raw, const long long *h_raw_off, int nkf, int kf_begin, const DevKf *h_kf,
                             DevPack &pack, float adj_r2, cudaStream_t st, BuildScratch &scr, float *kernel_ms = nullptr);

cudaError_t build_plane_index(const DevPack &pk, const DevKf *h_kf, int kf_begin, int nkf, const DevParams &pr, cudaStream_t st,
                              BuildScratch &scr);

constexpr int kK1SurvCap = 4096;
constexpr int kK1MatchCap = 8192;
constexpr int kK1BandWords = 4096;
__host__ __device__ inline int k1_band_rows(int bm_wpr) { return bm_wpr >= kK1BandWords ? 1 : kK1BandWords / bm_wpr; }

size_t assoc2d_smem_bytes(int max_kp, int max_tab_bytes, int max_groups);
cudaError_t assoc2d_configure(size_t smem);
cudaError_t launch_assoc2d(const DevPack &pk, const DevWork &wk, const DevParams &pr, int B, size_t smem, int max_kp, int max_tab_bytes,
                           int max_groups, cudaStream_t st, int with_terms = 1);
size_t assoc2d_split_smem_bytes(int max_band_words, int max_groups);
cudaError_t assoc2d_split_configure(size_t smem);
cudaError_t launch_assoc2d_split(const DevPack &pk, const DevWork &wk, const DevParams &pr, int B, size_t smem, int max_bands, int max_surv_cap,
                                 cudaStream_t st, int with_terms = 1);

cudaError_t launch_align3d(const DevPack &pk, const DevWork &wk, const DevParams &pr, int B, int debug, cudaStream_t st,
                           cudaEvent_t after_traversal = nullptr, uint32_t *lm_pos = nullptr, int *lm_m = nullptr);
cudaError_t launch_knn3d(const DevPack &pk, int kf, const double *d_q, int nq, int k, double radius2, uint32_t *d_idx, double *d_d2,
                         int *d_cnt, cudaStream_t st);

cudaError_t launch_debug_trig(const double *d_x, int n, double *d_acos, double *d_cos, cudaStream_t st);

cudaError_t launch_reduce(const DevPack &pk, const DevWork &wk, const DevParams &pr, int B, double *d_out, cudaStream_t st, int out_stride = 0,
                          const P2pView *p2p = nullptr);
cudaError_t launch_frames(const DevPack &pk, const DevWork &wk, const DevParams &pr, int B, double *d_out, cudaStream_t st);

}
struct stl_he_edges;
struct stl_calib_edges;
namespace stl {
cudaError_t he_linearize(const stl_he_edges &ed, const double *x, int B, double *h_out, double *h_chi2, cudaStream_t st);
cudaError_t calib_linearize(const stl_calib_edges &ed, const double *x, int B, double *h_out, double *h_chi2, cudaStream_t st);

}
```

spatial-temporal-lidar-camera-calibration_b200/csrc/knn.cuh:

```cuda
#pragma once
#include <cfloat>
#include <cmath>

#include "common.cuh"
#include "geom.cuh"
#include "kernels.h"

namespace stl {

constexpr unsigned kFull = 0xffffffffu;

struct ScanView {
    const float *px, *py, *pz;
    const uint32_t *orig;
    const float4 *lo, *hi;
    const uint16_t *adj;
    const float *adj_cov;
    unsigned long long *stats;
    int n0, n1;
};

__device__ __forceinline__ ScanView make_view(const DevPack &pk, const DevKf &K) {
    ScanView v;
    v.px = pk.px + K.pt_off; v.py = pk.py + K.pt_off; v.pz = pk.pz + K.pt_off;
    v.orig = pk.orig + K.pt_off;
    v.lo = pk.node_lo + K.node_off; v.hi = pk.node_hi + K.node_off;
    v.adj = pk.adj ? pk.adj + K.node_off * 32 : nullptr;
    v.adj_cov = pk.adj ? pk.adj_cov + K.node_off : nullptr;
    v.stats = nullptr;
    v.n0 = K.n0; v.n1 = K.n1;
    return v;
}

struct QueryF { float xl, xh, yl, yh, zl, zh; };
__device__ __forceinline__ QueryF make_queryf(double x, double y, double z) {
    QueryF q;
    q.xl = __double2float_rd(x); q.xh = __double2float_ru(x);
    q.yl = __double2float_rd(y); q.yh = __double2float_ru(y);
    q.zl = __double2float_rd(z); q.zh = __double2float_ru(z);
    return q;
}
__device__ __forceinline__ float box_lbf(const QueryF &q, float4 lo, float4 hi) {
    const float dx = fmaxf(fmaxf(__fsub_rd(lo.x, q.xh), __fsub_rd(q.xl, hi.x)), 0.f);
    const float dy = fmaxf(fmaxf(__fsub_rd(lo.y, q.yh), __fsub_rd(q.yl, hi.y)), 0.f);
    const float dz = fmaxf(fmaxf(__fsub_rd(lo.z, q.zh), __fsub_rd(q.zl, hi.z)), 0.f);
    const float s = __fadd_rd(__fadd_rd(__fmul_rd(dx, dx), __fmul_rd(dy, dy)), __fmul_rd(dz, dz));
    return __fmul_rd(s, 0.99999976f);
}

struct Sink1 {
    double d = DBL_MAX;
    float df = 3.402823466e+38f;
    float g2 = HUGE_VALF;
    uint32_t oi = 0xffffffffu, pos = 0xffffffffu;
    __device__ __forceinline__ bool may_contain(float lb) const { return lb <= df; }
    __device__ __forceinline__ static float below(double dd) { return __fmul_rd(__double2float_rd(dd), 0.99999976f); }
    __device__ __forceinline__ void note_pruned(float lb, bool pruned) {
        const unsigned k = __reduce_min_sync(kFull, pruned ? __float_as_uint(lb) : 0x7f800000u);
        g2 = fminf(g2, __uint_as_float(k));
    }
    __device__ __forceinline__ void note_bound(float b) { g2 = fminf(g2, b); }
    __device__ __forceinline__ void seed(const ScanView &S, uint32_t p, double qx, double qy, double qz) {
        const double dd = dist3e(qx, qy, qz, (double)S.px[p], (double)S.py[p], (double)S.pz[p]);
        if (dd == dd) { d = dd; df = __double2float_ru(dd); oi = S.orig[p]; pos = p; }
    }
    __device__ __forceinline__ void visit(const ScanView &S, int leaf, double qx, double qy, double qz, int lane) {
        const int g = leaf * kLeaf + lane;
        const double dd = dist3e(qx, qy, qz, (double)S.px[g], (double)S.py[g], (double)S.pz[g]);
        const float lowf = dd == dd ? below(dd) : __int_as_float(0x7f800000);
        const bool q = dd <= d;
        if (!__any_sync(kFull, q)) {
            note_pruned(lowf, (uint32_t)g != pos);
            return;
        }
        const uint32_t o = q ? S.orig[g] : 0xffffffffu;
        unsigned hi = q ? (unsigned)__double2hiint(dd) : 0xffffffffu;
        const unsigned mhi = __reduce_min_sync(kFull, hi);
        unsigned lo = (q && hi == mhi) ? (unsigned)__double2loint(dd) : 0xffffffffu;
        const unsigned mlo = __reduce_min_sync(kFull, lo);
        const bool tie = q && hi == mhi && (unsigned)__double2loint(dd) == mlo;
        const unsigned mo = __reduce_min_sync(kFull, tie ? o : 0xffffffffu);
        const double cd = __hiloint2double((int)mhi, (int)mlo);
        if (cd < d || (cd == d && mo < oi)) {
            const int src = __ffs(__ballot_sync(kFull, tie && o == mo)) - 1;
            if (pos != 0xffffffffu) g2 = fminf(g2, below(d));
            note_pruned(lowf, lane != src);
            d = cd; oi = mo; pos = (uint32_t)(leaf * kLeaf + src);
            df = __double2float_ru(cd);
        } else {
            note_pruned(lowf, (uint32_t)g != pos);
        }
    }
};

struct SinkK {
    double kd = DBL_MAX;
    uint32_t ki = 0xffffffffu, kpos = 0xffffffffu;
    int count = 0, k;
    double r2, wd;
    float r2f, wdf;
    uint32_t wi = 0xffffffffu;
    __device__ __forceinline__ SinkK(int k_, double r2_) : k(k_), r2(r2_), wd(r2_) {
        r2f = r2_ < 3.0e38 ? __double2float_ru(r2_) : 3.402823466e+38f;
        wdf = r2f;
    }
    __device__ __forceinline__ bool accept(double d, uint32_t i) const {
        return d < r2 && (count < k || d < wd || (d == wd && i < wi));
    }
    __device__ __forceinline__ bool may_contain(float lb) const { return lb <= r2f && (count < k || lb <= wdf); }
    __device__ __forceinline__ void note_pruned(float, bool) {}
    __device__ __forceinline__ void note_bound(float) {}
    __device__ __forceinline__ void visit(const ScanView &S, int leaf, double qx, double qy, double qz, int lane) {
        const int g = leaf * kLeaf + lane;
        const double dd = dist3e(qx, qy, qz, (double)S.px[g], (double)S.py[g], (double)S.pz[g]);
        const bool pre = dd < r2 && (count < k || dd <= wd);
        unsigned mask = __ballot_sync(kFull, pre);
        if (!mask) return;
        const uint32_t o = pre ? S.orig[g] : 0xffffffffu;
        if (__popc(mask) >= (count == 0 ? 4 : 8)) {
            bulk_merge(pre ? dd : (double)INFINITY, o, (uint32_t)g, lane);
            return;
        }
        while (mask) {
            const int src = __ffs(mask) - 1;
            mask &= mask - 1;
            const double cd = __shfl_sync(kFull, dd, src);
            const uint32_t ci = __shfl_sync(kFull, o, src);
            if (!accept(cd, ci)) continue;
            const bool less = lane < count && (kd < cd || (kd == cd && ki < ci));
            const int at = __popc(__ballot_sync(kFull, less));
            const double sd = __shfl_up_sync(kFull, kd, 1);
            const uint32_t si = __shfl_up_sync(kFull, ki, 1), sp = __shfl_up_sync(kFull, kpos, 1);
            if (lane > at) { kd = sd; ki = si; kpos = sp; }
            else if (lane == at) { kd = cd; ki = ci; kpos = (uint32_t)(leaf * kLeaf + src); }
            if (count < k) ++count;
            if (count == k) { wd = __shfl_sync(kFull, kd, k - 1); wi = __shfl_sync(kFull, ki, k - 1); wdf = __double2float_ru(wd); }
        }
    }

    __device__ __forceinline__ static void cx(double &d, uint32_t &i, uint32_t &p, int j, bool keep_min) {
        const double od = __shfl_xor_sync(kFull, d, j);
        const uint32_t oi = __shfl_xor_sync(kFull, i, j), op = __shfl_xor_sync(kFull, p, j);
        const bool other_less = od < d || (od == d && oi < i);
        const bool other_more = od > d || (od == d && oi > i);
        if (keep_min ? other_less : other_more) { d = od; i = oi; p = op; }
    }

    __device__ __forceinline__ void bulk_merge(double cd, uint32_t ci, uint32_t cp, int lane) {
        unsigned key = cd < (double)INFINITY ? ((__float_as_uint(__double2float_rd(cd)) & ~31u) | (unsigned)lane) : (0xffffffe0u | (unsigned)lane);
#pragma unroll
        for (int kk = 2; kk <= 32; kk <<= 1) {
#pragma unroll
            for (int j = kk >> 1; j > 0; j >>= 1) {
                const unsigned o = __shfl_xor_sync(kFull, key, j);
                const bool keep_min = ((lane & kk) == 0) == ((lane & j) == 0);
                key = keep_min ? min(key, o) : max(key, o);
            }
        }
        {
            const int src = (int)(key & 31u);
            const double sd = __shfl_sync(kFull, cd, src);
            const uint32_t si = __shfl_sync(kFull, ci, src), sp = __shfl_sync(kFull, cp, src);
            cd = sd; ci = si; cp = sp;
        }
        const unsigned next_key = __shfl_down_sync(kFull, key, 1);
        if (__ballot_sync(kFull, lane < 31 && (key >> 5) == (next_key >> 5) && cd < (double)INFINITY)) {
            for (;;) {
                bool moved = false;
#pragma unroll 1
                for (int parity = 0; parity < 2; ++parity) {
                    const bool lower = (lane & 1) == parity;
                    const int partner = lower ? lane + 1 : lane - 1;
                    const bool ok = partner >= 0 && partner < 32;
                    const double od = __shfl_sync(kFull, cd, ok ? partner : lane);
                    const uint32_t oi = __shfl_sync(kFull, ci, ok ? partner : lane), op = __shfl_sync(kFull, cp, ok ? partner : lane);
                    const bool other_less = od < cd || (od == cd && oi < ci);
                    const bool other_more = od > cd || (od == cd && oi > ci);
                    if (ok && (lower ? other_less : other_more)) { cd = od; ci = oi; cp = op; moved = true; }
                }
                if (!__any_sync(kFull, moved)) break;
            }
        }
        if (count == 0) {
            kd = cd; ki = ci; kpos = cp;
        } else {
            if (lane >= count) { kd = (double)INFINITY; ki = 0xffffffffu; }
            const double rd = __shfl_sync(kFull, cd, 31 - lane);
            const uint32_t ri = __shfl_sync(kFull, ci, 31 - lane), rp = __shfl_sync(kFull, cp, 31 - lane);
            if (rd < kd || (rd == kd && ri < ki)) { kd = rd; ki = ri; kpos = rp; }
#pragma unroll
            for (int j = 16; j > 0; j >>= 1) cx(kd, ki, kpos, j, (lane & j) == 0);
        }
        const int nvalid = __popc(__ballot_sync(kFull, kd < (double)INFINITY));
        count = nvalid < k ? nvalid : k;
        if (count == k) { wd = __shfl_sync(kFull, kd, k - 1); wi = __shfl_sync(kFull, ki, k - 1); wdf = __double2float_ru(wd); }
    }
};

template <class Sink>
__device__ __forceinline__ void traverse(const ScanView &S, double qx, double qy, double qz, Sink &sink, int lane, int first_leaf = -1) {
    if (first_leaf >= 0) sink.visit(S, first_leaf, qx, qy, qz, lane);
    const float4 *lo2 = S.lo + S.n0 + S.n1, *hi2 = S.hi + S.n0 + S.n1;
    const float4 *lo1 = S.lo + S.n0, *hi1 = S.hi + S.n0;
    const QueryF qf = make_queryf(qx, qy, qz);
    const float lb2 = box_lbf(qf, lo2[lane], hi2[lane]);
    const unsigned key2 = __float_as_uint(lb2);
    unsigned done2 = 0;
    for (;;) {
        const bool c2 = !((done2 >> lane) & 1u) && sink.may_contain(lb2);
        const unsigned m2 = __reduce_min_sync(kFull, c2 ? key2 : 0xffffffffu);
        if (m2 == 0xffffffffu) break;
        const int s2 = __ffs(__ballot_sync(kFull, c2 && key2 == m2)) - 1;
        done2 |= 1u << s2;
        const int n1i = s2 * 32 + lane;
        const float lb1 = box_lbf(qf, lo1[n1i], hi1[n1i]);
        const unsigned key1 = __float_as_uint(lb1);
        unsigned done1 = 0;
        for (;;) {
                const bool c1 = !((done1 >> lane) & 1u) && sink.may_contain(lb1);
            const unsigned m1 = __reduce_min_sync(kFull, c1 ? key1 : 0xffffffffu);
            if (m1 == 0xffffffffu) break;
            const int s1 = __ffs(__ballot_sync(kFull, c1 && key1 == m1)) - 1;
            done1 |= 1u << s1;
            const int n0i = (s2 * 32 + s1) * 32 + lane;
            const float lb0 = box_lbf(qf, S.lo[n0i], S.hi[n0i]);
            const unsigned key0 = __float_as_uint(lb0);
            unsigned done0 = ((s2 * 32 + s1) == (first_leaf >> 5) && first_leaf >= 0) ? (1u << (first_leaf & 31)) : 0u;
            for (;;) {
                        const bool c0 = !((done0 >> lane) & 1u) && sink.may_contain(lb0);
                const unsigned m0 = __reduce_min_sync(kFull, c0 ? key0 : 0xffffffffu);
                if (m0 == 0xffffffffu) break;
                const int s0 = __ffs(__ballot_sync(kFull, c0 && key0 == m0)) - 1;
                done0 |= 1u << s0;
                sink.visit(S, (s2 * 32 + s1) * 32 + s0, qx, qy, qz, lane);
            }
            sink.note_pruned(lb0, !((done0 >> lane) & 1u));
        }
        sink.note_pruned(lb1, !((done1 >> lane) & 1u));
    }
    sink.note_pruned(lb2, !((done2 >> lane) & 1u));
}

__device__ __forceinline__ int next_ticket(int *ticket, int lane) {
    int t = 0;
    if (lane == 0) t = atomicAdd(ticket, 1);
    return __shfl_sync(kFull, t, 0);
}

template <class Sink>
__device__ __forceinline__ float scan_adjacent(const ScanView &S, int home, double qx, double qy, double qz, Sink &sink, int lane) {
    if (S.adj == nullptr) return -1.f;
    const float cov = S.adj_cov[home];
    if (cov < 0.f) return -1.f;
    const unsigned id = S.adj[(long long)home * 32 + lane];
    const QueryF qf = make_queryf(qx, qy, qz);
    const float lb = id != 0xffffu ? box_lbf(qf, S.lo[id], S.hi[id]) : __int_as_float(0x7f800000);
    const unsigned key = __float_as_uint(lb);
    unsigned done = 0;
    for (;;) {
        const bool c = !((done >> lane) & 1u) && sink.may_contain(lb);
        const unsigned m = __reduce_min_sync(kFull, c ? key : 0xffffffffu);
        if (m == 0xffffffffu) break;
        const int s = __ffs(__ballot_sync(kFull, c && key == m)) - 1;
        done |= 1u << s;
        sink.visit(S, (int)__shfl_sync(kFull, id, s), qx, qy, qz, lane);
    }
    sink.note_pruned(lb, !((done >> lane) & 1u));
    return cov;
}

__device__ __forceinline__ void knn_around_point(const ScanView &S, uint32_t pos, SinkK &kn, int lane) {
    const double x = (double)S.px[pos], y = (double)S.py[pos], z = (double)S.pz[pos];
    const float cov = scan_adjacent(S, (int)(pos >> 5), x, y, z, kn, lane);
    const bool done = cov > 3.0e38f || (cov >= 0.f && kn.count == kn.k && kn.wdf < cov);
    if (S.stats && lane == 0) { atomicAdd(S.stats + 0, 1ull); atomicAdd(S.stats + (done ? 1 : (cov >= 0.f ? 2 : 3)), 1ull); }
    if (done) return;
    if (cov >= 0.f) kn = SinkK(kn.k, kn.r2);
    traverse(S, x, y, z, kn, lane, (int)(pos >> 5));
}

__device__ __forceinline__ float home_box_delta(const ScanView &S, int home, double qx, double qy, double qz) {
    const float4 lo = S.lo[home], hi = S.hi[home];
    const float xl = __double2float_rd(qx), xh = __double2float_ru(qx), yl = __double2float_rd(qy), yh = __double2float_ru(qy);
    const float zl = __double2float_rd(qz), zh = __double2float_ru(qz);
    const float gx = fmaxf(fmaxf(__fsub_ru(lo.x, xl), __fsub_ru(xh, hi.x)), 0.f);
    const float gy = fmaxf(fmaxf(__fsub_ru(lo.y, yl), __fsub_ru(yh, hi.y)), 0.f);
    const float gz = fmaxf(fmaxf(__fsub_ru(lo.z, zl), __fsub_ru(zh, hi.z)), 0.f);
    return __fsqrt_ru(__fadd_ru(__fadd_ru(__fmul_ru(gx, gx), __fmul_ru(gy, gy)), __fmul_ru(gz, gz)));
}

__device__ __forceinline__ void nn_near_leaf_seeded(const ScanView &S, float adj_r, int home, double qx, double qy, double qz, Sink1 &nn,
                                                    int lane, float delta) {
    const float cov = scan_adjacent(S, home, qx, qy, qz, nn, lane);
    if (S.stats && lane == 0) atomicAdd(S.stats + 4, 1ull);
    if (cov >= 0.f && nn.pos != 0xffffffffu) {
        const float reach = __fadd_ru(__fsqrt_ru(nn.df), delta);
        if (cov > 3.0e38f ? reach <= adj_r : reach < __fsqrt_rd(cov)) {
            if (S.stats && lane == 0) atomicAdd(S.stats + 5, 1ull);
            const float u = __fsub_rd(cov > 3.0e38f ? adj_r : __fsqrt_rd(cov), delta);
            nn.note_bound(u > 0.f ? __fmul_rd(u, u) : 0.f);
            return;
        }
        const int l1 = (int)(nn.pos >> 5);
        if (l1 != home) {
            const float cov1 = S.adj_cov[l1];
            const float two_rho = __fmul_ru(2.f, __fsqrt_ru(nn.df));
            if (cov1 >= 0.f && (cov1 > 3.0e38f ? two_rho <= adj_r : two_rho < __fsqrt_rd(cov1))) {
                const float rho_up = __fsqrt_ru(nn.df);
                scan_adjacent(S, l1, qx, qy, qz, nn, lane);
                if (S.stats && lane == 0) atomicAdd(S.stats + 5, 1ull);
                const float u = __fsub_rd(cov1 > 3.0e38f ? adj_r : __fsqrt_rd(cov1), rho_up);
                nn.note_bound(u > 0.f ? __fmul_rd(u, u) : 0.f);
                return;
            }
        }
    }
    if (S.stats && lane == 0) atomicAdd(S.stats + (cov >= 0.f ? 6 : 7), 1ull);
    traverse(S, qx, qy, qz, nn, lane);
}

__device__ __forceinline__ void nn_near_leaf(const ScanView &S, float adj_r, int home, double qx, double qy, double qz, Sink1 &nn,
                                             int lane, uint32_t hint = 0xffffffffu) {
    if (hint != 0xffffffffu) nn.seed(S, hint, qx, qy, qz);
    nn_near_leaf_seeded(S, adj_r, home, qx, qy, qz, nn, lane, home_box_delta(S, home, qx, qy, qz));
}

struct PlaneOut { V3 n; double reg; int m; bool gates_ok; };

struct NbGather {
    const ScanView &S;
    const uint32_t *__restrict__ nb;
    __device__ __forceinline__ void get(int j, double &x, double &y, double &z) const {
        const uint32_t p = nb[j];
        x = (double)S.px[p]; y = (double)S.py[p]; z = (double)S.pz[p];
    }
};
struct NbCoords {
    const float4 *__restrict__ base;
    long long stride;
    __device__ __forceinline__ void get(int j, double &x, double &y, double &z) const {
        const float4 v = base[(long long)j * stride];
        x = (double)v.x; y = (double)v.y; z = (double)v.z;
    }
};
__device__ __forceinline__ void store_nb_coords(float4 *__restrict__ nbx, long long stride, long long slot, const ScanView &S, int lane,
                                                int count, uint32_t kpos) {
    float4 v = make_float4(0.f, 0.f, 0.f, 0.f);
    if (lane < count) v = make_float4(S.px[kpos], S.py[kpos], S.pz[kpos], __uint_as_float(kpos));
    nbx[(long long)lane * stride + slot] = v;
}

template <class Src>
__device__ __forceinline__ PlaneOut plane_fit(const Src &src, int m, double last, double cx, double cy, double cz, const DevParams &pr,
                                              const bool stable = false) {
    PlaneOut out;
    out.m = m;
    out.n = {0.0, 0.0, 0.0};
    out.reg = 0;
    out.gates_ok = false;
    if (stable) {
        if (m < 3) return out;
    } else if (m == 0 || (last < pr.min_diff2) || (m < pr.min_pts)) {
        return out;
    }
    out.gates_ok = true;
    double c0 = 0, c1 = 0, c2 = 0, c3 = 0, c4 = 0, c5 = 0, c6 = 0, c7 = 0, c8 = 0;
    for (int j = 0; j < m; ++j) {
        double x, y, z;
        src.get(j, x, y, z);
        c0 += x; c1 += y; c2 += z;
        c3 += x * x; c4 += x * y; c5 += x * z;
        c6 += y * y; c7 += y * z; c8 += z * z;
    }
    const double dm = (double)m;
    c0 /= dm; c1 /= dm; c2 /= dm; c3 /= dm; c4 /= dm; c5 /= dm; c6 /= dm; c7 /= dm; c8 /= dm;
    const double cov[6] = {c3 - c0 * c0, c4 - c0 * c1, c5 - c0 * c2, c6 - c1 * c1, c7 - c1 * c2, c8 - c2 * c2};
    const V3 n = normalized(smallest_eigvec(cov));
    double reg = 0;
    for (int j = 0; j < m; ++j) {
        double x, y, z;
        src.get(j, x, y, z);
        const V3 d = {x - cx, y - cy, z - cz};
        reg += fabs(dot(d, n));
    }
    out.n = n;
    out.reg = reg / (double)(m - 1);
    if (stable && sqrt(last) < pr.min_diff) out.reg = __longlong_as_double(0x7ff0000000000000ll);
    return out;
}


__device__ __forceinline__ PlaneOut plane_thread(const ScanView &S, const uint32_t *__restrict__ nb, int m, double last, double cx,
                                                 double cy, double cz, const DevParams &pr, const bool stable = false) {
    return plane_fit(NbGather{S, nb}, m, last, cx, cy, cz, pr, stable);
}

__device__ __forceinline__ PlaneOut plane_lookup(const DevPack &pk, const DevKf &K, uint32_t pos) {
    const PlaneRec r = pk.pl_rec[K.pt_off + pos];
    const int mm = pk.pl_m[K.pt_off + pos];
    PlaneOut out;
    out.gates_ok = mm >= 0;
    out.m = mm >= 0 ? mm : -(mm + 1);
    out.n = {r.nx, r.ny, r.nz};
    out.reg = r.reg;
    return out;
}

}
```

spatial-temporal-lidar-camera-calibration_b200/csrc/knn3d.cu:

```cuda
#include <algorithm>
#include <cstdlib>

#include "kernels.h"
#include "knn.cuh"

namespace stl {
namespace {

constexpr int kWarps = 8;
#ifndef STL_KNN_MINB
#define STL_KNN_MINB 8
#endif
constexpr int kPlaneThreads = 128;
#ifndef STL_PLANE_MINB
#define STL_PLANE_MINB 5
#endif

__device__ __forceinline__ void map_point_lidar(const DevPack &pk, const DevKf &K, const DevCand &c, int f, uint32_t kp, double &qx,
                                                double &qy, double &qz) {
    const float *Tcw = pk.Tcw + (long long)f * 12;
    const float *mp = pk.kp_mp + (K.kp_off + kp) * 3;
    const double wx = (double)__fmul_rn(mp[0], c.sf), wy = (double)__fmul_rn(mp[1], c.sf), wz = (double)__fmul_rn(mp[2], c.sf);
    const double cxm = dadd(dot3e((double)Tcw[0], (double)Tcw[1], (double)Tcw[2], wx, wy, wz), dmul((double)Tcw[3], c.s));
    const double cym = dadd(dot3e((double)Tcw[4], (double)Tcw[5], (double)Tcw[6], wx, wy, wz), dmul((double)Tcw[7], c.s));
    const double czm = dadd(dot3e((double)Tcw[8], (double)Tcw[9], (double)Tcw[10], wx, wy, wz), dmul((double)Tcw[11], c.s));
    xform(c.Ri, c.ti, cxm, cym, czm, qx, qy, qz);
}

__global__ void __launch_bounds__(kWarps * 32, STL_KNN_MINB)
k_nn_knn(const DevPack pk, const DevWork wk, const DevParams pr, const int B, const int batch, uint32_t *__restrict__ lm_pos,
         int *__restrict__ lm_m) {
    const int sub = wk.sub;
    const int j = blockIdx.x % sub;
    const int bf = blockIdx.x / sub;
    const int fi = bf / B, f = sel_kf(pk, fi), b = bf - fi * B;
    const int nq = wk.n_q[(long long)b * pk.n_kf + f];
    if (nq <= 0) return;
    const int lane = threadIdx.x & 31;
    const DevKf K = pk.kf[f];
    const DevCand &c = wk.cand[b];
    ScanView S = make_view(pk, K);
    S.stats = wk.dbg_stats;
    const long long cbase = (long long)b * pk.n_kp_total + K.kp_off;
    const long long qbase = (long long)b * pk.n_mp_total + K.mp_off;
    __shared__ int ticket;
    if (threadIdx.x == 0) ticket = 0;
    __syncthreads();
    for (;;) {
        const int t0 = next_ticket(&ticket, lane) * batch;
        if ((long long)t0 * sub + j >= nq) break;
        const int qi = (t0 + lane) * sub + j;
        const bool valid = lane < batch && qi < nq;
        double qx = 0, qy = 0, qz = 0, sd = DBL_MAX;
        uint32_t hint = 0, soi = 0xffffffffu, spos = 0xffffffffu;
        float delta = 0.f;
        if (valid) {
            const uint2 ks = wk.q_kpsp[cbase + qi];
            hint = ks.y;
            map_point_lidar(pk, K, c, f, ks.x, qx, qy, qz);
            const double dd = dist3e(qx, qy, qz, (double)S.px[hint], (double)S.py[hint], (double)S.pz[hint]);
            if (dd == dd) { sd = dd; soi = S.orig[hint]; spos = hint; }
            delta = home_box_delta(S, (int)(hint >> 5), qx, qy, qz);
        }
        uint32_t out_pos = 0xffffffffu;
        float out_g2 = 0.f;
        unsigned todo = __ballot_sync(kFull, valid);
        while (todo) {
            const int src = __ffs(todo) - 1;
            todo &= todo - 1;
            const double x = __shfl_sync(kFull, qx, src), y = __shfl_sync(kFull, qy, src), z = __shfl_sync(kFull, qz, src);
            const uint32_t h = __shfl_sync(kFull, hint, src);
            Sink1 nn;
            nn.d = __shfl_sync(kFull, sd, src);
            nn.oi = __shfl_sync(kFull, soi, src);
            nn.pos = __shfl_sync(kFull, spos, src);
            if (nn.pos != 0xffffffffu) nn.df = __double2float_ru(nn.d);
            nn_near_leaf_seeded(S, pr.adj_r, (int)(h >> 5), x, y, z, nn, lane, __shfl_sync(kFull, delta, src));
            if (lane == src) { out_pos = nn.pos; out_g2 = nn.g2; }
            if (pr.use_plane && !pr.plane_index) {
                const long long slot = qbase + (long long)(t0 + src) * sub + j;
                SinkK kn(pr.k, pr.radius2);
                knn_around_point(S, nn.pos, kn, lane);
                wk.nb[slot * kMaxK + lane] = lane < kn.count ? kn.kpos : 0xffffffffu;
                store_nb_coords(wk.nbx, wk.nbx_stride, slot, S, lane, kn.count, kn.kpos);
                const double last = __shfl_sync(kFull, kn.kd, kn.count > 0 ? kn.count - 1 : 0);
                if (lane == 0) { wk.nb_m[slot] = kn.count; wk.nb_last[slot] = last; }
            }
        }
        if (valid) { wk.nn_pos[qbase + qi] = out_pos; wk.nn_g2[qbase + qi] = out_g2; }
        if (lm_pos != nullptr && b == 0) {
            double lx = 0, ly = 0, lz = 0, nn_d = DBL_MAX;
            uint32_t nn_p = 0xffffffffu;
            bool need = false;
            if (valid) {
                const float *Tcw = pk.Tcw + (long long)f * 12;
                const float *mp = pk.kp_mp + (K.kp_off + wk.q_kpsp[cbase + qi].x) * 3;
                const double ma = (double)mp[0], mb = (double)mp[1], mc = (double)mp[2];
                const double Mx = dadd(dot3e((double)Tcw[0], (double)Tcw[1], (double)Tcw[2], ma, mb, mc), (double)Tcw[3]);
                const double My = dadd(dot3e((double)Tcw[4], (double)Tcw[5], (double)Tcw[6], ma, mb, mc), (double)Tcw[7]);
                const double Mz = dadd(dot3e((double)Tcw[8], (double)Tcw[9], (double)Tcw[10], ma, mb, mc), (double)Tcw[11]);
                xform(c.Ri, c.ti, dmul(Mx, c.s), dmul(My, c.s), dmul(Mz, c.s), lx, ly, lz);
                need = true;
                if (out_pos != 0xffffffffu) {
                    const double move = sqrt(dist3e(qx, qy, qz, lx, ly, lz)) * (1.0 + 1e-9) + 1e-12;
                    const double dh = dist3e(lx, ly, lz, (double)S.px[out_pos], (double)S.py[out_pos], (double)S.pz[out_pos]);
                    const double reach = (double)__fsqrt_rd(out_g2) - move;
                    if (reach > 0.0 && reach * reach > dh * (1.0 + 1e-6) + 1e-18) { need = false; nn_p = out_pos; nn_d = dh; }
                }
            }
            unsigned todo2 = __ballot_sync(kFull, need);
            while (todo2) {
                const int src = __ffs(todo2) - 1;
                todo2 &= todo2 - 1;
                const double x = __shfl_sync(kFull, lx, src), y = __shfl_sync(kFull, ly, src), z = __shfl_sync(kFull, lz, src);
                uint32_t h = __shfl_sync(kFull, out_pos, src);
                if (h == 0xffffffffu) h = __shfl_sync(kFull, hint, src);
                Sink1 nn;
                nn_near_leaf(S, pr.adj_r, (int)(h >> 5), x, y, z, nn, lane, h);
                if (lane == src) { nn_p = nn.pos; nn_d = nn.d; }
            }
            if (valid) {
                const long long slot = K.mp_off + qi;
                if (nn_d > pr.max_3d_dist2) {
                    lm_pos[slot] = 0xffffffffu;
                } else {
                    lm_pos[slot] = nn_p;
                    lm_m[slot] = nn_p == hint ? -2 : -3;
                }
            }
        }
    }
}

__global__ void __launch_bounds__(kPlaneThreads, STL_PLANE_MINB)
k_plane_dist(const DevPack pk, const DevWork wk, const DevParams pr, const int B, const int debug) {
    const int sub = wk.sub;
    const int j = blockIdx.x % sub;
    const int bf = blockIdx.x / sub;
    const int fi = bf / B, f = sel_kf(pk, fi), b = bf - fi * B;
    const long long rec = (long long)b * pk.n_kf + f;
    const int nq = wk.n_q[rec];
    double s3d = 0, v3d = 0, c3d = 0, vpl = 0, vpt = 0;
    if (nq > 0) {
        const DevKf K = pk.kf[f];
        const DevCand &c = wk.cand[b];
        const ScanView S = make_view(pk, K);
        const long long cbase = (long long)b * pk.n_kp_total + K.kp_off;
        const long long qbase = (long long)b * pk.n_mp_total + K.mp_off;
        for (int qi = j * kPlaneThreads + threadIdx.x; qi < nq; qi += sub * kPlaneThreads) {
            const uint32_t kp = wk.corr_kp[cbase + wk.q_corr[cbase + qi]];
            double qx, qy, qz;
            map_point_lidar(pk, K, c, f, kp, qx, qy, qz);
            const uint32_t np = wk.nn_pos[qbase + qi];
            const double nx = (double)S.px[np], ny = (double)S.py[np], nz = (double)S.pz[np];
            const double dx = dsub(nx, qx), dy = dsub(ny, qy), dz = dsub(nz, qz);
            double dist = sqrt(dot3e(dx, dy, dz, dx, dy, dz));
            int is_plane = 0, m = 0;
            if (pr.use_plane) {
                const PlaneOut po = pr.plane_index ? plane_lookup(pk, K, np)
                                                   : plane_fit(NbCoords{wk.nbx + qbase + qi, wk.nbx_stride}, wk.nb_m[qbase + qi], wk.nb_last[qbase + qi], nx, ny, nz, pr, pr.variant == 1);
                m = po.m;
                if (po.gates_ok && !(po.reg > pr.reg_thr)) {
                    is_plane = 1;
                    dist = fabs(dot3e(dx, dy, dz, po.n.x, po.n.y, po.n.z));
                }
            }
            if (dist < pr.thr3d) {
                s3d += dist; v3d += 1.0;
                if (is_plane) vpl += 1.0; else vpt += 1.0;
            }
            c3d += 1.0;
            if (debug) {
                const long long o = K.kp_off + qi;
                wk.dbg_nn[o] = S.orig[np];
                wk.dbg_m[o] = m;
                wk.dbg_plane[o] = is_plane;
                wk.dbg_dist[o] = dist;
                for (int t = 0; t < kMaxK; ++t) {
                    const uint32_t p = (pr.use_plane && !pr.plane_index && t < m) ? wk.nb[(qbase + qi) * kMaxK + t] : 0xffffffffu;
                    wk.dbg_knn[o * kMaxK + t] = p == 0xffffffffu ? 0xffffffffu : S.orig[p];
                }
            }
        }
    }
    __shared__ double red[5][kPlaneThreads / 32];
    const int lane = threadIdx.x & 31, warp = threadIdx.x >> 5;
    for (int o = 16; o; o >>= 1) {
        s3d += __shfl_down_sync(0xffffffffu, s3d, o); v3d += __shfl_down_sync(0xffffffffu, v3d, o);
        c3d += __shfl_down_sync(0xffffffffu, c3d, o); vpl += __shfl_down_sync(0xffffffffu, vpl, o);
        vpt += __shfl_down_sync(0xffffffffu, vpt, o);
    }
    if (lane == 0) { red[0][warp] = s3d; red[1][warp] = v3d; red[2][warp] = c3d; red[3][warp] = vpl; red[4][warp] = vpt; }
    __syncthreads();
    if (threadIdx.x == 0) {
        AlignRec r = {0, 0, 0, 0, 0};
        for (int w = 0; w < kPlaneThreads / 32; ++w) { r.s3d += red[0][w]; r.v3d += red[1][w]; r.c3d += red[2][w]; r.vpl += red[3][w]; r.vpt += red[4][w]; }
        wk.align[rec * sub + j] = r;
    }
}

__global__ void __launch_bounds__(kWarps * 32)
k_knn3d(const DevPack pk, const int kf, const double *__restrict__ q, const int nq, const int k, const double radius2,
        uint32_t *__restrict__ out_idx, double *__restrict__ out_d2, int *__restrict__ out_cnt) {
    const int lane = threadIdx.x & 31;
    const int qi = blockIdx.x * kWarps + (threadIdx.x >> 5);
    if (qi >= nq) return;
    const DevKf K = pk.kf[kf];
    const ScanView S = make_view(pk, K);
    SinkK kn(k, radius2 > 0 ? radius2 : DBL_MAX);
    traverse(S, q[qi * 3], q[qi * 3 + 1], q[qi * 3 + 2], kn, lane);
    if (lane < k) {
        out_idx[(long long)qi * k + lane] = lane < kn.count ? kn.ki : 0xffffffffu;
        out_d2[(long long)qi * k + lane] = lane < kn.count ? kn.kd : INFINITY;
    }
    if (lane == 0) out_cnt[qi] = kn.count;
}

__global__ void __launch_bounds__(kWarps * 32, STL_KNN_MINB)
k_index_knn(const DevPack pk, const int kf_begin, const DevParams pr, const long long first_pt, uint32_t *__restrict__ nb,
            int *__restrict__ nb_m, double *__restrict__ nb_last) {
    const DevKf K = pk.kf[kf_begin + blockIdx.y];
    const int lane = threadIdx.x & 31, warp = threadIdx.x >> 5;
    const ScanView S = make_view(pk, K);
    for (int p = blockIdx.x * kWarps + warp; p < K.n_pts; p += gridDim.x * kWarps) {
        SinkK kn(pr.k, pr.radius2);
        knn_around_point(S, (uint32_t)p, kn, lane);
        const long long o = K.pt_off - first_pt + p;
        nb[o * kMaxK + lane] = lane < kn.count ? kn.kpos : 0xffffffffu;
        const double last = __shfl_sync(kFull, kn.kd, kn.count > 0 ? kn.count - 1 : 0);
        if (lane == 0) { nb_m[o] = kn.count; nb_last[o] = last; }
    }
}

__global__ void __launch_bounds__(kPlaneThreads)
k_index_plane(const DevPack pk, const int kf_begin, const DevParams pr, const long long first_pt, const uint32_t *__restrict__ nb,
              const int *__restrict__ nb_m, const double *__restrict__ nb_last) {
    const DevKf K = pk.kf[kf_begin + blockIdx.y];
    const ScanView S = make_view(pk, K);
    for (int p = blockIdx.x * kPlaneThreads + threadIdx.x; p < K.n_pad; p += gridDim.x * kPlaneThreads) {
        PlaneRec r = {0.0, 0.0, 0.0, 0.0};
        int mm = -1;
        if (p < K.n_pts) {
            const long long o = K.pt_off - first_pt + p;
            const PlaneOut po = plane_thread(S, nb + o * kMaxK, nb_m[o], nb_last[o], (double)S.px[p], (double)S.py[p], (double)S.pz[p], pr, pr.variant == 1);
            r.nx = po.n.x; r.ny = po.n.y; r.nz = po.n.z; r.reg = po.reg;
            mm = po.gates_ok ? po.m : -(po.m + 1);
        }
        pk.pl_rec[K.pt_off + p] = r;
        pk.pl_m[K.pt_off + p] = mm;
    }
}

}

cudaError_t build_plane_index(const DevPack &pk, const DevKf *h_kf, int kf_begin, int nkf, const DevParams &pr, cudaStream_t st,
                              BuildScratch &scr) {
    const long long first = h_kf[kf_begin].pt_off;
    const long long npts = h_kf[kf_begin + nkf - 1].pt_off + h_kf[kf_begin + nkf - 1].n_pad - first;
    if (npts <= 0) return cudaSuccess;
    int max_pts = 0;
    for (int f = 0; f < nkf; ++f) max_pts = max_pts > h_kf[kf_begin + f].n_pad ? max_pts : h_kf[kf_begin + f].n_pad;
    cudaError_t e = scr.need(2, 4 * (size_t)npts * kMaxK);
    if (e == cudaSuccess) e = scr.need(4, 4 * (size_t)npts);
    if (e == cudaSuccess) e = scr.need(3, 8 * (size_t)npts);
    if (e != cudaSuccess) return e;
    uint32_t *nb = (uint32_t *)scr.buf[2]; int *m = (int *)scr.buf[4]; double *last = (double *)scr.buf[3];
    const int bx = (max_pts + kWarps * 16 - 1) / (kWarps * 16);
    k_index_knn<<<dim3(bx, nkf), kWarps * 32, 0, st>>>(pk, kf_begin, pr, first, nb, m, last);
    k_index_plane<<<dim3((max_pts + kPlaneThreads * 4 - 1) / (kPlaneThreads * 4), nkf), kPlaneThreads, 0, st>>>(pk, kf_begin, pr, first, nb, m, last);
    return cudaGetLastError();
}

namespace {
__global__ void k_debug_trig(const double *__restrict__ x, int n, double *__restrict__ ac, double *__restrict__ co) {
    const int i = blockIdx.x * blockDim.x + threadIdx.x;
    if (i >= n) return;
    ac[i] = acos_cr(fmin(fmax(x[i], -1.0), 1.0));
    co[i] = cos_cr(x[i]);
}
}

cudaError_t launch_debug_trig(const double *d_x, int n, double *d_acos, double *d_cos, cudaStream_t st) {
    if (n <= 0) return cudaSuccess;
    k_debug_trig<<<(n + 255) / 256, 256, 0, st>>>(d_x, n, d_acos, d_cos);
    return cudaGetLastError();
}

cudaError_t launch_align3d(const DevPack &pk, const DevWork &wk, const DevParams &pr, int B, int debug, cudaStream_t st, cudaEvent_t after_traversal,
                           uint32_t *lm_pos, int *lm_m) {
    if (B <= 0) return cudaSuccess;
    if (pk.n_sel <= 0) return after_traversal ? cudaEventRecord(after_traversal, st) : cudaSuccess;
    int batch = (long long)pk.n_sel * B >= 600 ? 8 : 4;
    if (const char *e = getenv("STL_K2_BATCH")) batch = std::max(1, std::min(32, atoi(e)));
    k_nn_knn<<<(unsigned)(pk.n_sel * B * wk.sub), kWarps * 32, 0, st>>>(pk, wk, pr, B, batch, lm_pos, lm_m);
    cudaError_t e = cudaGetLastError();
    if (e != cudaSuccess) return e;
    if (after_traversal && (e = cudaEventRecord(after_traversal, st)) != cudaSuccess) return e;
    k_plane_dist<<<(unsigned)(pk.n_sel * B * wk.sub), kPlaneThreads, 0, st>>>(pk, wk, pr, B, debug);
    return cudaGetLastError();
}

cudaError_t launch_knn3d(const DevPack &pk, int kf, const double *d_q, int nq, int k, double radius2, uint32_t *d_idx, double *d_d2,
                         int *d_cnt, cudaStream_t st) {
    if (nq <= 0) return cudaSuccess;
    k_knn3d<<<(nq + kWarps - 1) / kWarps, kWarps * 32, 0, st>>>(pk, kf, d_q, nq, k, radius2, d_idx, d_d2, d_cnt);
    return cudaGetLastError();
}

}
```

spatial-temporal-lidar-camera-calibration_b200/csrc/lm.cu:

```cuda
#include <cub/cub.cuh>

#include "../../include/stlcalib.h"
#include "dual.cuh"
#include "gprfit.hpp"
#include "knn.cuh"
#include "lm.h"

namespace stl {
namespace {

constexpr int kWarps = 8;
#ifndef STL_LM_MINB
#define STL_LM_MINB 6
#endif
constexpr int kLinVals = 41;
constexpr int kGprWarps = 1;
constexpr int kLinThreads = 128;


__device__ __forceinline__ void lm_lane(const DevPack &pk, DevWork &wk, LmState &lm, bool arg0 = true) {
    const int2 am = arg0 && blockIdx.y == 0 ? lm.lane0 : lm.amap[blockIdx.y];
    const long long nk = pk.n_kp_total, F = pk.n_kf, nm = lm.n_slots;
    const long long wc = am.x, wq = wc * nm;
    wk.cand += wc;
    wk.corr_kp += wc * nk; wk.corr_sp += wc * nk; wk.q_corr += wc * nk; wk.q_kpsp += wc * nk;
    wk.n_corr += wc * F; wk.n_q += wc * F;
    wk.nn_pos += wq; wk.nn_g2 += wq; wk.nb += wq * kMaxK; wk.nbx += wq; wk.nb_m += wq; wk.nb_last += wq;
    const long long lo = (long long)blockIdx.y * nm;
    lm.stage += lo; lm.plane_a += lo * 4; lm.nnb_pos += lo; lm.nbb += lo * kMaxK; lm.nbbx += lo; lm.nbb_m += lo; lm.nbb_last += lo;
    const long long po = (long long)am.y * lm.slot_stride;
    lm.slot_kf += po; lm.slot_kp += po; lm.flag2d += po; lm.type3d += po; lm.flag3d += po; lm.flagG += po;
    lm.geo2d += po * 6; lm.geo3d += po * 9; lm.gpr_nb += po * kMaxK; lm.gpr_m += po;
    lm.d_counts += am.y * 4;
}

__global__ void k_lm_clear(LmState lm) {
    const long long po = (long long)lm.amap[blockIdx.y].y * lm.slot_stride, n = lm.slot_stride, ptot = (long long)lm.P * n;
    for (long long i = (long long)blockIdx.x * blockDim.x + threadIdx.x; i < n; i += (long long)gridDim.x * blockDim.x) {
        lm.flags[po + i] = 0; lm.flags[ptot + po + i] = 0; lm.flags[2 * ptot + po + i] = 0; lm.flags[3 * ptot + po + i] = 0;
    }
    if (blockIdx.x == 0 && threadIdx.x < 4) lm.d_counts[lm.amap[blockIdx.y].y * 4 + threadIdx.x] = 0;
}

__device__ __forceinline__ bool lm_frame_active(const DevWork &wk, const DevParams &pr, int f, int &nq) {
    nq = wk.n_q[f];
    return wk.n_corr[f] >= pr.num_min_corr && nq > 0;
}

__device__ __forceinline__ void lm_map_point(const DevPack &pk, const DevKf &K, int f, uint32_t kp, double &Mx, double &My, double &Mz) {
    const float *Tcw = pk.Tcw + (long long)f * 12;
    const float *mp = pk.kp_mp + (K.kp_off + kp) * 3;
    const double a = (double)mp[0], b = (double)mp[1], c = (double)mp[2];
    Mx = dadd(dot3e((double)Tcw[0], (double)Tcw[1], (double)Tcw[2], a, b, c), (double)Tcw[3]);
    My = dadd(dot3e((double)Tcw[4], (double)Tcw[5], (double)Tcw[6], a, b, c), (double)Tcw[7]);
    Mz = dadd(dot3e((double)Tcw[8], (double)Tcw[9], (double)Tcw[10], a, b, c), (double)Tcw[11]);
}

__global__ void __launch_bounds__(kWarps * 32, STL_LM_MINB)
k_lm_knn_a(const DevPack pk, DevWork wk, const DevParams pr, LmState lm) {
    lm_lane(pk, wk, lm);
    const int j = blockIdx.x % lm.sub, f = sel_kf(pk, blockIdx.x / lm.sub);
    int nq;
    if (!lm_frame_active(wk, pr, f, nq)) return;
    const int lane = threadIdx.x & 31, warp = threadIdx.x >> 5;
    const DevKf K = pk.kf[f];
    const ScanView S = make_view(pk, K);
    const int C = pk.n_covis;
    __shared__ int ticket;
    if (threadIdx.x == 0) ticket = 0;
    __syncthreads();
    for (;;) {
        const int qi = next_ticket(&ticket, lane) * lm.sub + j;
        if (qi >= nq) break;
        const uint2 ks = wk.q_kpsp[K.kp_off + qi];
        const uint32_t kp = ks.x, sp = ks.y;
        const long long slot = K.mp_off + qi;
        const bool obs = lane < C && pk.covis_valid[f * C + lane] && !isnan(pk.covis_uv[(K.kp_off + kp) * C + lane].x);
        const int ncov = __popc(__ballot_sync(kFull, obs));
        if (ncov == 0) {
            if (lane == 0) wk.nb_m[slot] = -1;
            continue;
        }
        if (pr.plane_index && !pr.use_gpr) {
            if (lane == 0) wk.nb_m[slot] = 0;
            continue;
        }
        SinkK kn(pr.k, pr.radius2);
        knn_around_point(S, sp, kn, lane);
        wk.nb[slot * kMaxK + lane] = lane < kn.count ? kn.kpos : 0xffffffffu;
        store_nb_coords(wk.nbx, wk.nbx_stride, slot, S, lane, kn.count, kn.kpos);
        const double last = __shfl_sync(kFull, kn.kd, kn.count > 0 ? kn.count - 1 : 0);
        if (lane == 0) { wk.nb_m[slot] = kn.count; wk.nb_last[slot] = last; }
    }
}

__global__ void __launch_bounds__(128)
k_lm_plane_a(const DevPack pk, DevWork wk, const DevParams pr, LmState lm) {
    lm_lane(pk, wk, lm);
    const int j = blockIdx.x % lm.sub, f = sel_kf(pk, blockIdx.x / lm.sub);
    int nq;
    if (!lm_frame_active(wk, pr, f, nq)) return;
    __shared__ int cnt[2];
    if (threadIdx.x < 2) cnt[threadIdx.x] = 0;
    __syncthreads();
    const DevKf K = pk.kf[f];
    const ScanView S = make_view(pk, K);
    const bool from_index = pr.plane_index && !pr.use_gpr;
    const int C = pk.n_covis;
    for (int qi = j * blockDim.x + threadIdx.x; qi < nq; qi += lm.sub * blockDim.x) {
        const long long slot = K.mp_off + qi;
        lm.stage[slot] = 0;
        const uint32_t ci = wk.q_corr[K.kp_off + qi];
        const uint32_t kp = wk.corr_kp[K.kp_off + ci], sp = wk.corr_sp[K.kp_off + ci];
        int m = 0;
        if (from_index) {
            bool any = false;
            for (int s = 0; s < C; ++s) any = any || (pk.covis_valid[f * C + s] && !isnan(pk.covis_uv[(K.kp_off + kp) * C + s].x));
            if (!any) continue;
        } else {
            m = wk.nb_m[slot];
            if (m < 0) continue;
        }
        const double cx = (double)S.px[sp], cy = (double)S.py[sp], cz = (double)S.pz[sp];
        const PlaneOut po = from_index ? plane_lookup(pk, K, sp)
                                       : plane_fit(NbCoords{wk.nbx + slot, wk.nbx_stride}, m, wk.nb_last[slot], cx, cy, cz, pr);
        if (!po.gates_ok) continue;
        const long long cs = slot;
        lm.slot_kf[cs] = f;
        lm.slot_kp[cs] = kp;
        double *pa = lm.plane_a + slot * 4;
        pa[0] = po.n.x; pa[1] = po.n.y; pa[2] = po.n.z; pa[3] = po.reg;
        if (po.reg < pr.reg_thr) {
            double *g = lm.geo2d + cs * 6;
            g[0] = cx; g[1] = cy; g[2] = cz; g[3] = po.n.x; g[4] = po.n.y; g[5] = po.n.z;
            lm.flag2d[cs] = 1;
            atomicAdd(&cnt[0], 1);
        } else if (pr.use_gpr) {
            for (int t = 0; t < kMaxK; ++t) lm.gpr_nb[slot * kMaxK + t] = wk.nb[slot * kMaxK + t];
            lm.gpr_m[slot] = po.m;
            lm.flagG[cs] = 1;
            atomicAdd(&cnt[1], 1);
        }
        lm.stage[slot] = 1;
    }
    __syncthreads();
    if (threadIdx.x < 2 && cnt[threadIdx.x] > 0) atomicAdd(lm.d_counts + 3 * threadIdx.x, cnt[threadIdx.x]);
}

__global__ void __launch_bounds__(kWarps * 32, STL_LM_MINB)
k_lm_knn_b(const DevPack pk, DevWork wk, const DevParams pr, LmState lm, const bool hints, const bool cert) {
    lm_lane(pk, wk, lm);
    const uint32_t *__restrict__ nn_hint = hints ? wk.nn_pos : nullptr;
    const float *__restrict__ nn_g2 = hints && cert ? wk.nn_g2 : nullptr;
    const int j = blockIdx.x % lm.sub, f = sel_kf(pk, blockIdx.x / lm.sub);
    int nq;
    if (!lm_frame_active(wk, pr, f, nq)) return;
    const int lane = threadIdx.x & 31;
    const DevKf K = pk.kf[f];
    const DevCand &c0 = wk.cand[0];
    const ScanView S = make_view(pk, K);
    const float *Tcw = pk.Tcw + (long long)f * 12;
    __shared__ int ticket;
    if (threadIdx.x == 0) ticket = 0;
    __syncthreads();
    for (;;) {
        const int base = next_ticket(&ticket, lane) * 32;
        if ((long long)base * lm.sub + j >= nq) break;
        const int qi = (base + lane) * lm.sub + j;
        const long long slot = K.mp_off + qi;
        const bool valid = qi < nq && lm.stage[slot] == 1;
        uint32_t sp = 0, hint = 0xffffffffu, nn_pos = 0xffffffffu;
        double qx = 0, qy = 0, qz = 0, nn_d = DBL_MAX;
        bool settled = false;
        if (valid) {
            const uint2 ks = wk.q_kpsp[K.kp_off + qi];
            const uint32_t kp = ks.x;
            sp = ks.y;
            double Mx, My, Mz;
            lm_map_point(pk, K, f, kp, Mx, My, Mz);
            xform(c0.Ri, c0.ti, dmul(Mx, c0.s), dmul(My, c0.s), dmul(Mz, c0.s), qx, qy, qz);
            hint = nn_hint ? nn_hint[slot] : sp;
            if (hint == 0xffffffffu) hint = sp;
            if (nn_hint && nn_g2 && nn_hint[slot] != 0xffffffffu) {
                const float *mp = pk.kp_mp + (K.kp_off + kp) * 3;
                const double wx = (double)__fmul_rn(mp[0], c0.sf), wy = (double)__fmul_rn(mp[1], c0.sf), wz = (double)__fmul_rn(mp[2], c0.sf);
                const double ex = dadd(dot3e((double)Tcw[0], (double)Tcw[1], (double)Tcw[2], wx, wy, wz), dmul((double)Tcw[3], c0.s));
                const double ey = dadd(dot3e((double)Tcw[4], (double)Tcw[5], (double)Tcw[6], wx, wy, wz), dmul((double)Tcw[7], c0.s));
                const double ez = dadd(dot3e((double)Tcw[8], (double)Tcw[9], (double)Tcw[10], wx, wy, wz), dmul((double)Tcw[11], c0.s));
                double ox, oy, oz;
                xform(c0.Ri, c0.ti, ex, ey, ez, ox, oy, oz);
                const double move = sqrt(dist3e(ox, oy, oz, qx, qy, qz)) * (1.0 + 1e-9) + 1e-12;
                const double dh = dist3e(qx, qy, qz, (double)S.px[hint], (double)S.py[hint], (double)S.pz[hint]);
                const double reach = (double)__fsqrt_rd(nn_g2[slot]) - move;
                if (reach > 0.0 && reach * reach > dh * (1.0 + 1e-6) + 1e-18) { settled = true; nn_pos = hint; nn_d = dh; }
            }
        }
        unsigned todo = __ballot_sync(kFull, valid && !settled);
        while (todo) {
            const int src = __ffs(todo) - 1;
            todo &= todo - 1;
            const double sx = __shfl_sync(kFull, qx, src), sy = __shfl_sync(kFull, qy, src), sz = __shfl_sync(kFull, qz, src);
            const uint32_t sh = __shfl_sync(kFull, hint, src);
            Sink1 nn;
            nn_near_leaf(S, pr.adj_r, (int)(sh >> 5), sx, sy, sz, nn, lane, sh);
            if (lane == src) { nn_pos = nn.pos; nn_d = nn.d; }
        }
        bool want_knn = false;
        if (valid) {
            if (nn_d > pr.max_3d_dist2) {
                lm.nnb_pos[slot] = 0xffffffffu;
            } else {
                lm.nnb_pos[slot] = nn_pos;
                if (nn_pos == sp) lm.nbb_m[slot] = -2;
                else if (pr.plane_index) lm.nbb_m[slot] = -3;
                else want_knn = true;
            }
        }
        unsigned kn_todo = __ballot_sync(kFull, want_knn);
        while (kn_todo) {
            const int src = __ffs(kn_todo) - 1;
            kn_todo &= kn_todo - 1;
            const uint32_t p = __shfl_sync(kFull, nn_pos, src);
            const long long sl = K.mp_off + ((long long)(base + src) * lm.sub + j);
            SinkK kn(pr.k, pr.radius2);
            knn_around_point(S, p, kn, lane);
            lm.nbb[sl * kMaxK + lane] = lane < kn.count ? kn.kpos : 0xffffffffu;
            store_nb_coords(lm.nbbx, lm.nbbx_stride, sl, S, lane, kn.count, kn.kpos);
            const double last = __shfl_sync(kFull, kn.kd, kn.count > 0 ? kn.count - 1 : 0);
            if (lane == 0) { lm.nbb_m[sl] = kn.count; lm.nbb_last[sl] = last; }
        }
    }
}

__device__ __forceinline__ bool block3d_geometry(const DevPack &pk, const DevParams &pr, const LmState &lm, long long slot, int f, uint32_t kp,
                                                 double g[9], int &type) {
    if (lm.stage[slot] != 1) return false;
    const uint32_t np = lm.nnb_pos[slot];
    if (np == 0xffffffffu) return false;
    const DevKf &K = pk.kf[f];
    const float *sx = pk.px + K.pt_off, *sy = pk.py + K.pt_off, *sz = pk.pz + K.pt_off;
    const double nx = (double)sx[np], ny = (double)sy[np], nz = (double)sz[np];
    bool gates_ok, state;
    double n3[3];
    const int m = lm.nbb_m[slot];
    if (m == -2) {
        const double *pa = lm.plane_a + slot * 4;
        gates_ok = true; n3[0] = pa[0]; n3[1] = pa[1]; n3[2] = pa[2];
        state = pa[3] < pr.reg_thr;
    } else {
        const PlaneOut p2 = m == -3 ? plane_lookup(pk, K, np) : plane_fit(NbCoords{lm.nbbx + slot, lm.nbbx_stride}, m, lm.nbb_last[slot], nx, ny, nz, pr);
        gates_ok = p2.gates_ok; n3[0] = p2.n.x; n3[1] = p2.n.y; n3[2] = p2.n.z;
        state = p2.gates_ok && p2.reg < pr.reg_thr;
    }
    lm_map_point(pk, K, f, kp, g[0], g[1], g[2]);
    g[3] = nx; g[4] = ny; g[5] = nz;
    g[6] = gates_ok ? n3[0] : 0.0; g[7] = gates_ok ? n3[1] : 0.0; g[8] = gates_ok ? n3[2] : 1.0;
    type = state ? 2 : 1;
    return true;
}

__global__ void __launch_bounds__(128)
k_lm_plane_b(const DevPack pk, DevWork wk, const DevParams pr, LmState lm) {
    lm_lane(pk, wk, lm, false);
    const int j = blockIdx.x % lm.sub, f = sel_kf(pk, blockIdx.x / lm.sub);
    int nq;
    if (!lm_frame_active(wk, pr, f, nq)) return;
    const DevKf K = pk.kf[f];
    __shared__ int cnt[2];
    if (threadIdx.x < 2) cnt[threadIdx.x] = 0;
    __syncthreads();
    for (int qi = j * blockDim.x + threadIdx.x; qi < nq; qi += lm.sub * blockDim.x) {
        const long long slot = K.mp_off + qi;
        if (lm.stage[slot] != 1) continue;
        if (lm.nnb_pos[slot] == 0xffffffffu) continue;
        const uint32_t ci = wk.q_corr[K.kp_off + qi];
        const uint32_t kp = wk.corr_kp[K.kp_off + ci];
        double g9[9];
        int type;
        if (!block3d_geometry(pk, pr, lm, slot, f, kp, g9, type)) continue;
        double *g = lm.geo3d + slot * 9;
#pragma unroll
        for (int i = 0; i < 9; ++i) g[i] = g9[i];
        lm.type3d[slot] = (uint8_t)type;
        lm.flag3d[slot] = 1;
        atomicAdd(&cnt[0], 1);
        if (type == 1) atomicAdd(&cnt[1], 1);
    }
    __syncthreads();
    if (threadIdx.x < 2 && cnt[threadIdx.x] > 0) atomicAdd(lm.d_counts + 1 + threadIdx.x, cnt[threadIdx.x]);
}

struct Acc {
    double v[kLinVals];
};

struct F7 {
    double a;
    double v[7];
};
static_assert(sizeof(F7) == sizeof(D7), "F7 views D7 storage");
__device__ __forceinline__ F7 f7_const(double x) { F7 r; r.a = x; for (int i = 0; i < 7; ++i) r.v[i] = 0.0; return r; }
__device__ __forceinline__ F7 operator+(const F7 &f, const F7 &g) { F7 r; r.a = f.a + g.a; for (int i = 0; i < 7; ++i) r.v[i] = f.v[i] + g.v[i]; return r; }
__device__ __forceinline__ F7 operator-(const F7 &f, const F7 &g) { F7 r; r.a = f.a - g.a; for (int i = 0; i < 7; ++i) r.v[i] = f.v[i] - g.v[i]; return r; }
__device__ __forceinline__ F7 operator*(const F7 &f, const F7 &g) { F7 r; r.a = f.a * g.a; for (int i = 0; i < 7; ++i) r.v[i] = fma(f.a, g.v[i], f.v[i] * g.a); return r; }
__device__ __forceinline__ F7 operator/(const F7 &f, const F7 &g) {
    F7 r;
    const double gi = 1.0 / g.a, q = f.a * gi;
    r.a = q;
    for (int i = 0; i < 7; ++i) r.v[i] = fma(-q, g.v[i], f.v[i]) * gi;
    return r;
}
__device__ __forceinline__ F7 operator*(const F7 &f, double c) { F7 r; r.a = f.a * c; for (int i = 0; i < 7; ++i) r.v[i] = f.v[i] * c; return r; }
__device__ __forceinline__ F7 operator+(const F7 &f, double c) { F7 r = f; r.a = f.a + c; return r; }
__device__ __forceinline__ F7 operator-(const F7 &f, double c) { F7 r = f; r.a = f.a - c; return r; }

__device__ __forceinline__ void huber(double sq, double delta, double &rho0, double &sr) {
    if (sq > delta * delta) {
        const double r = sqrt(sq);
        rho0 = 2.0 * delta * r - delta * delta;
        sr = sqrt(fmax(DBL_MIN, delta / r));
    } else {
        rho0 = sq;
        sr = 1.0;
    }
}

__device__ __forceinline__ void accumulate(Acc &A, const D7 &e, double sr) {
    const double r = sr * e.a;
    double J[7];
#pragma unroll
    for (int a = 0; a < 7; ++a) J[a] = sr * e.v[a];
    int h = 8;
#pragma unroll
    for (int a = 0; a < 7; ++a) {
        A.v[1 + a] += J[a] * r;
#pragma unroll
        for (int b = a; b < 7; ++b) A.v[h++] += J[a] * J[b];
    }
}

__device__ __forceinline__ void mv3(const D7 *M, const D7 *p, D7 *o) {
#pragma unroll
    for (int i = 0; i < 3; ++i) o[i] = (M[i * 3] * p[0] + M[i * 3 + 1] * p[1]) + M[i * 3 + 2] * p[2];
}
__device__ __forceinline__ void mv3(const F7 *M, const F7 *p, F7 *o) {
#pragma unroll
    for (int i = 0; i < 3; ++i) o[i] = (M[i * 3] * p[0] + M[i * 3 + 1] * p[1]) + M[i * 3 + 2] * p[2];
}
__device__ __forceinline__ void accumulate(Acc &A, const F7 &e, double sr) {
    const double r = sr * e.a;
    double J[7];
#pragma unroll
    for (int a = 0; a < 7; ++a) J[a] = sr * e.v[a];
    int h = 8;
#pragma unroll
    for (int a = 0; a < 7; ++a) {
        A.v[1 + a] = fma(J[a], r, A.v[1 + a]);
#pragma unroll
        for (int b = a; b < 7; ++b) { A.v[h] = fma(J[a], J[b], A.v[h]); ++h; }
    }
}

template <class T7>
__device__ __forceinline__ void put_row(const BlockOut &o, long long blk, int r, const T7 &e) {
    o.res[blk * o.rmax + r] = e.a;
    double *j = o.jac + (blk * o.rmax + r) * 7;
#pragma unroll
    for (int a = 0; a < 7; ++a) j[a] = e.v[a];
}
__device__ __forceinline__ void put_head(const BlockOut &o, long long blk, int type, int kf, uint32_t kp, int nres) {
    o.type[blk] = type; o.kf[blk] = kf; o.kp[blk] = (int32_t)kp; o.nres[blk] = nres;
}

__device__ __forceinline__ void lm_list_start(const LmState &lm, int p, int which, int *out) {
    if (threadIdx.x >= 32) return;
    int s = 0;
    for (int q = threadIdx.x; q < p; q += 32) s += lm.d_counts[q * 4 + which];
    for (int o = 16; o; o >>= 1) s += __shfl_down_sync(0xffffffffu, s, o);
    if (threadIdx.x == 0) *out = s;
}

__device__ __forceinline__ int sel_slot(const DevPack &pk, int v) {
    int lo = 0, hi = pk.n_sel;
    while (hi - lo > 1) {
        const int mid = (lo + hi) >> 1;
        if (pk.sel_mp[mid].x <= v) lo = mid; else hi = mid;
    }
    return v + pk.sel_mp[lo].y;
}

template <bool WB>
__global__ void __launch_bounds__(kLinThreads)
k_linearize(const DevPack pk, const DevParams pr, const LmState lm, const LmCand *__restrict__ cands, const int *__restrict__ cprob,
            double *__restrict__ partial, int partial_stride, const BlockOut bo) {
// ... 731 lines not shown
```

Before: 1074.

## Pack scan points with original index into float4 records for kNN traversal

Adds an interleaved float4 array holding x, y, z and the original point index, filled during the kd-tree refine pass. All kNN visit, seed and neighbour lookups now read one 16-byte record instead of four separate SoA loads. k_nn_knn is also templated on whether neighbour search is needed, so that branch is removed at compile time. The cost is extra device memory and an extra store per point at build time, plus a new debug accessor.

```diff
diff --git a/include/stlcalib.h b/include/stlcalib.h
--- a/include/stlcalib.h
+++ b/include/stlcalib.h
@@ -214,6 +214,8 @@
 
 stl_status_t stl_debug_trig(stl_ctx_t *ctx, const double *x, int32_t n, double *acos_out, double *cos_out);
 
+stl_status_t stl_debug_points(stl_ctx_t *ctx, int32_t kf, float *xyz, uint32_t *orig, float *rec, int32_t cap, int32_t *n);
+
 
 #define STL_STAGE_ASSOC2D 0
 #define STL_STAGE_KNN3D 1
diff --git a/spatial-temporal-lidar-camera-calibration_b200/_abi.py b/spatial-temporal-lidar-camera-calibration_b200/_abi.py
--- a/spatial-temporal-lidar-camera-calibration_b200/_abi.py
+++ b/spatial-temporal-lidar-camera-calibration_b200/_abi.py
@@ -168,6 +168,7 @@
                                   C.c_int32, _i32p]),
     "stl_debug_frame": (C.c_int, [_vp, C.c_int32, C.c_int32, _dp]),
     "stl_debug_trig": (C.c_int, [_vp, _dp, C.c_int32, _dp, _dp]),
+    "stl_debug_points": (C.c_int, [_vp, C.c_int32, C.POINTER(C.c_float), _u32p, C.POINTER(C.c_float), C.c_int32, _i32p]),
     "stl_knn3d": (C.c_int, [_vp, C.c_int32, _dp, C.c_int32, C.c_int32, C.c_double, _u32p, _dp, _i32p]),
     "stl_set_stream": (C.c_int, [_vp, _vp]),
     "stl_set_profiling": (C.c_int, [_vp, C.c_int32]),
diff --git a/spatial-temporal-lidar-camera-calibration_b200/capi.py b/spatial-temporal-lidar-camera-calibration_b200/capi.py
--- a/spatial-temporal-lidar-camera-calibration_b200/capi.py
+++ b/spatial-temporal-lidar-camera-calibration_b200/capi.py
@@ -338,6 +338,18 @@
         _check(self.lib, self.h, self.lib.stl_debug_trig(self.h, x.ctypes.data_as(_dp), len(x), a.ctypes.data_as(_dp), c.ctypes.data_as(_dp)))
         return a, c
 
+    def debug_points(self, kf: int):
+        n = C.c_int32(0)
+        _check(self.lib, self.h, self.lib.stl_debug_points(self.h, kf, None, None, None, 0, C.byref(n)))
+        k = n.value
+        xyz = np.zeros((max(k, 1), 3), np.float32)
+        orig = np.zeros(max(k, 1), np.uint32)
+        rec = np.zeros((max(k, 1), 4), np.float32)
+        fp = C.POINTER(C.c_float)
+        _check(self.lib, self.h, self.lib.stl_debug_points(self.h, kf, xyz.ctypes.data_as(fp), orig.ctypes.data_as(_abi._u32p),
+                                                           rec.ctypes.data_as(fp), k, C.byref(n)))
+        return xyz[:k], orig[:k], rec[:k]
+
     def knn3d(self, kf: int, q, k: int, radius2: float = 0.0):
         q = np.ascontiguousarray(q, dtype=np.float64).reshape(-1, 3)
         nq = q.shape[0]
diff --git a/spatial-temporal-lidar-camera-calibration_b200/csrc/build.cu b/spatial-temporal-lidar-camera-calibration_b200/csrc/build.cu
--- a/spatial-temporal-lidar-camera-calibration_b200/csrc/build.cu
+++ b/spatial-temporal-lidar-camera-calibration_b200/csrc/build.cu
@@ -117,7 +117,7 @@
 
 __global__ void __launch_bounds__(kRefThreads, 1)
 k_kd_refine(const DevKf *__restrict__ kf, int kf_begin, float *__restrict__ px, float *__restrict__ py, float *__restrict__ pz,
-            uint32_t *__restrict__ orig) {
+            uint32_t *__restrict__ orig, float4 *__restrict__ pt4) {
     extern __shared__ __align__(16) unsigned char refine_raw[];
     RefineSmem &S = *reinterpret_cast<RefineSmem *>(refine_raw);
     const DevKf K = kf[kf_begin + blockIdx.y];
@@ -192,6 +192,7 @@
         const int p = S.perm[i];
         px[base + i] = S.x[p]; py[base + i] = S.y[p]; pz[base + i] = S.z[p];
         orig[base + i] = S.o[p];
+        pt4[base + i] = make_float4(S.x[p], S.y[p], S.z[p], __uint_as_float(S.o[p]));
     }
 }
 
@@ -374,7 +375,7 @@
                 configured = true;
             }
             k_kd_refine<<<dim3((max_pad + kGroup - 1) / kGroup, nkf), kRefThreads, sizeof(RefineSmem), st>>>(pack.kf, kf_begin, pack.px, pack.py,
-                                                                                                          pack.pz, pack.orig);
+                                                                                                          pack.pz, pack.orig, pack.pt4);
         }
         k_leaf_aabb<<<dim3((max_n0 + 7) / 8, nkf), 256, 0, st>>>(pack.kf, kf_begin, pack.px, pack.py, pack.pz, pack.node_lo, pack.node_hi);
         k_inner_aabb<<<dim3((max_n1 + 7) / 8, nkf), 256, 0, st>>>(pack.kf, kf_begin, 1, pack.node_lo, pack.node_hi);
diff --git a/spatial-temporal-lidar-camera-calibration_b200/csrc/capi.cu b/spatial-temporal-lidar-camera-calibration_b200/csrc/capi.cu
--- a/spatial-temporal-lidar-camera-calibration_b200/csrc/capi.cu
+++ b/spatial-temporal-lidar-camera-calibration_b200/csrc/capi.cu
@@ -119,7 +119,7 @@
 
 void free_pack(stl_ctx *c) {
     DevPack &p = c->pk;
-    dfree(p.kf); dfree(p.px); dfree(p.py); dfree(p.pz); dfree(p.orig); dfree(p.node_lo); dfree(p.node_hi); dfree(p.adj); dfree(p.adj_cov);
+    dfree(p.kf); dfree(p.px); dfree(p.py); dfree(p.pz); dfree(p.orig); dfree(p.pt4); dfree(p.node_lo); dfree(p.node_hi); dfree(p.adj); dfree(p.adj_cov);
     dfree(p.pl_rec); dfree(p.pl_m);
     dfree(p.k1tab); dfree(p.bitmap); dfree(p.grid_start); dfree(p.grid_kp); dfree(p.kp_xy); dfree(p.kp_xyd); dfree(p.kp_mp); dfree(p.Tcw);
     dfree(p.relpose); dfree(p.covis_valid); dfree(p.covis_uv); dfree(p.he_Tc); dfree(p.he_Tl);
@@ -601,6 +601,7 @@
     const size_t npt = (size_t)std::max<long long>(L.n_pad_total, 4), nkk = (size_t)std::max<long long>(NK, 1);
     CK(cudaMalloc(&pk.kf, sizeof(DevKf) * F));
     CK(cudaMalloc(&pk.px, 4 * npt)); CK(cudaMalloc(&pk.py, 4 * npt)); CK(cudaMalloc(&pk.pz, 4 * npt)); CK(cudaMalloc(&pk.orig, 4 * npt));
+    CK(cudaMalloc(&pk.pt4, sizeof(float4) * npt));
     CK(cudaMalloc(&pk.node_lo, sizeof(float4) * nodes)); CK(cudaMalloc(&pk.node_hi, sizeof(float4) * nodes));
     if (ctx->adj_r2 > 0.f) { CK(cudaMalloc(&pk.adj, sizeof(uint16_t) * 32 * (size_t)nodes)); CK(cudaMalloc(&pk.adj_cov, sizeof(float) * (size_t)nodes)); }
     CK(cudaMalloc(&pk.k1tab, tab.k1tab.size()));
@@ -963,6 +964,29 @@
     if (e == cudaSuccess) e = cudaStreamSynchronize(st);
     cudaFree(d);
     if (e != cudaSuccess) return fail(ctx, STL_ERR_CUDA, "debug_trig: %s", cudaGetErrorString(e));
+    return STL_OK;
+}
+
+stl_status_t stl_debug_points(stl_ctx_t *ctx, int32_t kf, float *xyz, uint32_t *orig, float *rec, int32_t cap, int32_t *n) {
+    if (!ctx || !n || cap < 0) return STL_ERR_INVALID;
+    std::lock_guard<std::mutex> lk(ctx->mu);
+    CK(cudaSetDevice(ctx->device));
+    if (!ctx->has_pack) return fail(ctx, STL_ERR_STATE, "no pack uploaded");
+    if (kf < 0 || kf >= ctx->pk.n_kf) return fail(ctx, STL_ERR_INVALID, "keyframe out of range");
+    const DevKf &K = ctx->lay.kf[kf];
+    *n = K.n_pad;
+    const size_t m = (size_t)std::min(K.n_pad, cap);
+    if (m == 0) return STL_OK;
+    const DevPack &pk = ctx->pk;
+    if (xyz) {
+        std::vector<float> c(3 * m);
+        CK(cudaMemcpy(c.data(), pk.px + K.pt_off, 4 * m, cudaMemcpyDeviceToHost));
+        CK(cudaMemcpy(c.data() + m, pk.py + K.pt_off, 4 * m, cudaMemcpyDeviceToHost));
+        CK(cudaMemcpy(c.data() + 2 * m, pk.pz + K.pt_off, 4 * m, cudaMemcpyDeviceToHost));
+        for (size_t i = 0; i < m; ++i) for (int a = 0; a < 3; ++a) xyz[i * 3 + a] = c[a * m + i];
+    }
+    if (orig) CK(cudaMemcpy(orig, pk.orig + K.pt_off, 4 * m, cudaMemcpyDeviceToHost));
+    if (rec) CK(cudaMemcpy(rec, pk.pt4 + K.pt_off, 16 * m, cudaMemcpyDeviceToHost));
     return STL_OK;
 }
 
diff --git a/spatial-temporal-lidar-camera-calibration_b200/csrc/kernels.h b/spatial-temporal-lidar-camera-calibration_b200/csrc/kernels.h
--- a/spatial-temporal-lidar-camera-calibration_b200/csrc/kernels.h
+++ b/spatial-temporal-lidar-camera-calibration_b200/csrc/kernels.h
@@ -24,6 +24,7 @@
     DevKf *kf = nullptr;
     float *px = nullptr, *py = nullptr, *pz = nullptr;
     uint32_t *orig = nullptr;
+    float4 *pt4 = nullptr;
     float4 *node_lo = nullptr, *node_hi = nullptr;
     uint16_t *adj = nullptr;
     float *adj_cov = nullptr;
diff --git a/spatial-temporal-lidar-camera-calibration_b200/csrc/knn.cuh b/spatial-temporal-lidar-camera-calibration_b200/csrc/knn.cuh
--- a/spatial-temporal-lidar-camera-calibration_b200/csrc/knn.cuh
+++ b/spatial-temporal-lidar-camera-calibration_b200/csrc/knn.cuh
@@ -13,6 +13,7 @@
 struct ScanView {
     const float *px, *py, *pz;
     const uint32_t *orig;
+    const float4 *pt4;
     const float4 *lo, *hi;
     const uint16_t *adj;
     const float *adj_cov;
@@ -24,6 +25,7 @@
     ScanView v;
     v.px = pk.px + K.pt_off; v.py = pk.py + K.pt_off; v.pz = pk.pz + K.pt_off;
     v.orig = pk.orig + K.pt_off;
+    v.pt4 = pk.pt4 + K.pt_off;
     v.lo = pk.node_lo + K.node_off; v.hi = pk.node_hi + K.node_off;
     v.adj = pk.adj ? pk.adj + K.node_off * 32 : nullptr;
     v.adj_cov = pk.adj ? pk.adj_cov + K.node_off : nullptr;
@@ -61,19 +63,20 @@
     }
     __device__ __forceinline__ void note_bound(float b) { g2 = fminf(g2, b); }
     __device__ __forceinline__ void seed(const ScanView &S, uint32_t p, double qx, double qy, double qz) {
-        const double dd = dist3e(qx, qy, qz, (double)S.px[p], (double)S.py[p], (double)S.pz[p]);
-        if (dd == dd) { d = dd; df = __double2float_ru(dd); oi = S.orig[p]; pos = p; }
-    }
-    __device__ __forceinline__ void visit(const ScanView &S, int leaf, double qx, double qy, double qz, int lane) {
+        const float4 r = S.pt4[p];
+        const double dd = dist3e(qx, qy, qz, (double)r.x, (double)r.y, (double)r.z);
+        if (dd == dd) { d = dd; df = __double2float_ru(dd); oi = __float_as_uint(r.w); pos = p; }
+    }
+    __device__ __forceinline__ void visit(float4 r, int leaf, double qx, double qy, double qz, int lane) {
         const int g = leaf * kLeaf + lane;
-        const double dd = dist3e(qx, qy, qz, (double)S.px[g], (double)S.py[g], (double)S.pz[g]);
+        const double dd = dist3e(qx, qy, qz, (double)r.x, (double)r.y, (double)r.z);
         const float lowf = dd == dd ? below(dd) : __int_as_float(0x7f800000);
         const bool q = dd <= d;
         if (!__any_sync(kFull, q)) {
             note_pruned(lowf, (uint32_t)g != pos);
             return;
         }
-        const uint32_t o = q ? S.orig[g] : 0xffffffffu;
+        const uint32_t o = q ? __float_as_uint(r.w) : 0xffffffffu;
         unsigned hi = q ? (unsigned)__double2hiint(dd) : 0xffffffffu;
         const unsigned mhi = __reduce_min_sync(kFull, hi);
         unsigned lo = (q && hi == mhi) ? (unsigned)__double2loint(dd) : 0xffffffffu;
@@ -110,13 +113,13 @@
     __device__ __forceinline__ bool may_contain(float lb) const { return lb <= r2f && (count < k || lb <= wdf); }
     __device__ __forceinline__ void note_pruned(float, bool) {}
     __device__ __forceinline__ void note_bound(float) {}
-    __device__ __forceinline__ void visit(const ScanView &S, int leaf, double qx, double qy, double qz, int lane) {
+    __device__ __forceinline__ void visit(float4 r, int leaf, double qx, double qy, double qz, int lane) {
         const int g = leaf * kLeaf + lane;
-        const double dd = dist3e(qx, qy, qz, (double)S.px[g], (double)S.py[g], (double)S.pz[g]);
+        const double dd = dist3e(qx, qy, qz, (double)r.x, (double)r.y, (double)r.z);
         const bool pre = dd < r2 && (count < k || dd <= wd);
         unsigned mask = __ballot_sync(kFull, pre);
         if (!mask) return;
-        const uint32_t o = pre ? S.orig[g] : 0xffffffffu;
+        const uint32_t o = pre ? __float_as_uint(r.w) : 0xffffffffu;
         if (__popc(mask) >= (count == 0 ? 4 : 8)) {
             bulk_merge(pre ? dd : (double)INFINITY, o, (uint32_t)g, lane);
             return;
@@ -199,7 +202,7 @@
 
 template <class Sink>
 __device__ __forceinline__ void traverse(const ScanView &S, double qx, double qy, double qz, Sink &sink, int lane, int first_leaf = -1) {
-    if (first_leaf >= 0) sink.visit(S, first_leaf, qx, qy, qz, lane);
+    if (first_leaf >= 0) sink.visit(S.pt4[first_leaf * kLeaf + lane], first_leaf, qx, qy, qz, lane);
     const float4 *lo2 = S.lo + S.n0 + S.n1, *hi2 = S.hi + S.n0 + S.n1;
     const float4 *lo1 = S.lo + S.n0, *hi1 = S.hi + S.n0;
     const QueryF qf = make_queryf(qx, qy, qz);
@@ -232,7 +235,8 @@
                 if (m0 == 0xffffffffu) break;
                 const int s0 = __ffs(__ballot_sync(kFull, c0 && key0 == m0)) - 1;
                 done0 |= 1u << s0;
-                sink.visit(S, (s2 * 32 + s1) * 32 + s0, qx, qy, qz, lane);
+                const int leaf = (s2 * 32 + s1) * 32 + s0;
+                sink.visit(S.pt4[leaf * kLeaf + lane], leaf, qx, qy, qz, lane);
             }
             sink.note_pruned(lb0, !((done0 >> lane) & 1u));
         }
@@ -263,14 +267,16 @@
         if (m == 0xffffffffu) break;
         const int s = __ffs(__ballot_sync(kFull, c && key == m)) - 1;
         done |= 1u << s;
-        sink.visit(S, (int)__shfl_sync(kFull, id, s), qx, qy, qz, lane);
+        const int leaf = (int)__shfl_sync(kFull, id, s);
+        sink.visit(S.pt4[leaf * kLeaf + lane], leaf, qx, qy, qz, lane);
     }
     sink.note_pruned(lb, !((done >> lane) & 1u));
     return cov;
 }
 
 __device__ __forceinline__ void knn_around_point(const ScanView &S, uint32_t pos, SinkK &kn, int lane) {
-    const double x = (double)S.px[pos], y = (double)S.py[pos], z = (double)S.pz[pos];
+    const float4 r = S.pt4[pos];
+    const double x = (double)r.x, y = (double)r.y, z = (double)r.z;
     const float cov = scan_adjacent(S, (int)(pos >> 5), x, y, z, kn, lane);
     const bool done = cov > 3.0e38f || (cov >= 0.f && kn.count == kn.k && kn.wdf < cov);
     if (S.stats && lane == 0) { atomicAdd(S.stats + 0, 1ull); atomicAdd(S.stats + (done ? 1 : (cov >= 0.f ? 2 : 3)), 1ull); }
@@ -331,8 +337,8 @@
     const ScanView &S;
     const uint32_t *__restrict__ nb;
     __device__ __forceinline__ void get(int j, double &x, double &y, double &z) const {
-        const uint32_t p = nb[j];
-        x = (double)S.px[p]; y = (double)S.py[p]; z = (double)S.pz[p];
+        const float4 r = S.pt4[nb[j]];
+        x = (double)r.x; y = (double)r.y; z = (double)r.z;
     }
 };
 struct NbCoords {
@@ -346,7 +352,10 @@
 __device__ __forceinline__ void store_nb_coords(float4 *__restrict__ nbx, long long stride, long long slot, const ScanView &S, int lane,
                                                 int count, uint32_t kpos) {
     float4 v = make_float4(0.f, 0.f, 0.f, 0.f);
-    if (lane < count) v = make_float4(S.px[kpos], S.py[kpos], S.pz[kpos], __uint_as_float(kpos));
+    if (lane < count) {
+        const float4 r = S.pt4[kpos];
+        v = make_float4(r.x, r.y, r.z, __uint_as_float(kpos));
+    }
     nbx[(long long)lane * stride + slot] = v;
 }
 
diff --git a/spatial-temporal-lidar-camera-calibration_b200/csrc/knn3d.cu b/spatial-temporal-lidar-camera-calibration_b200/csrc/knn3d.cu
--- a/spatial-temporal-lidar-camera-calibration_b200/csrc/knn3d.cu
+++ b/spatial-temporal-lidar-camera-calibration_b200/csrc/knn3d.cu
@@ -27,6 +27,7 @@
     xform(c.Ri, c.ti, cxm, cym, czm, qx, qy, qz);
 }
 
+template <bool kNeighbours>
 __global__ void __launch_bounds__(kWarps * 32, STL_KNN_MINB)
 k_nn_knn(const DevPack pk, const DevWork wk, const DevParams pr, const int B, const int batch, uint32_t *__restrict__ lm_pos,
          int *__restrict__ lm_m) {
@@ -58,8 +59,9 @@
             const uint2 ks = wk.q_kpsp[cbase + qi];
             hint = ks.y;
             map_point_lidar(pk, K, c, f, ks.x, qx, qy, qz);
-            const double dd = dist3e(qx, qy, qz, (double)S.px[hint], (double)S.py[hint], (double)S.pz[hint]);
-            if (dd == dd) { sd = dd; soi = S.orig[hint]; spos = hint; }
+            const float4 r = S.pt4[hint];
+            const double dd = dist3e(qx, qy, qz, (double)r.x, (double)r.y, (double)r.z);
+            if (dd == dd) { sd = dd; soi = __float_as_uint(r.w); spos = hint; }
             delta = home_box_delta(S, (int)(hint >> 5), qx, qy, qz);
         }
         uint32_t out_pos = 0xffffffffu;
@@ -77,7 +79,7 @@
             if (nn.pos != 0xffffffffu) nn.df = __double2float_ru(nn.d);
             nn_near_leaf_seeded(S, pr.adj_r, (int)(h >> 5), x, y, z, nn, lane, __shfl_sync(kFull, delta, src));
             if (lane == src) { out_pos = nn.pos; out_g2 = nn.g2; }
-            if (pr.use_plane && !pr.plane_index) {
+            if (kNeighbours) {
                 const long long slot = qbase + (long long)(t0 + src) * sub + j;
                 SinkK kn(pr.k, pr.radius2);
                 knn_around_point(S, nn.pos, kn, lane);
@@ -103,7 +105,8 @@
                 need = true;
                 if (out_pos != 0xffffffffu) {
                     const double move = sqrt(dist3e(qx, qy, qz, lx, ly, lz)) * (1.0 + 1e-9) + 1e-12;
-                    const double dh = dist3e(lx, ly, lz, (double)S.px[out_pos], (double)S.py[out_pos], (double)S.pz[out_pos]);
+                    const float4 r = S.pt4[out_pos];
+                    const double dh = dist3e(lx, ly, lz, (double)r.x, (double)r.y, (double)r.z);
                     const double reach = (double)__fsqrt_rd(out_g2) - move;
                     if (reach > 0.0 && reach * reach > dh * (1.0 + 1e-6) + 1e-18) { need = false; nn_p = out_pos; nn_d = dh; }
                 }
@@ -152,7 +155,8 @@
             double qx, qy, qz;
             map_point_lidar(pk, K, c, f, kp, qx, qy, qz);
             const uint32_t np = wk.nn_pos[qbase + qi];
-            const double nx = (double)S.px[np], ny = (double)S.py[np], nz = (double)S.pz[np];
+            const float4 r = S.pt4[np];
+            const double nx = (double)r.x, ny = (double)r.y, nz = (double)r.z;
             const double dx = dsub(nx, qx), dy = dsub(ny, qy), dz = dsub(nz, qz);
             double dist = sqrt(dot3e(dx, dy, dz, dx, dy, dz));
             int is_plane = 0, m = 0;
@@ -172,7 +176,7 @@
             c3d += 1.0;
             if (debug) {
                 const long long o = K.kp_off + qi;
-                wk.dbg_nn[o] = S.orig[np];
+                wk.dbg_nn[o] = __float_as_uint(r.w);
                 wk.dbg_m[o] = m;
                 wk.dbg_plane[o] = is_plane;
                 wk.dbg_dist[o] = dist;
@@ -292,7 +296,9 @@
     if (pk.n_sel <= 0) return after_traversal ? cudaEventRecord(after_traversal, st) : cudaSuccess;
     int batch = (long long)pk.n_sel * B >= 600 ? 8 : 4;
     if (const char *e = getenv("STL_K2_BATCH")) batch = std::max(1, std::min(32, atoi(e)));
-    k_nn_knn<<<(unsigned)(pk.n_sel * B * wk.sub), kWarps * 32, 0, st>>>(pk, wk, pr, B, batch, lm_pos, lm_m);
+    const unsigned grid = (unsigned)(pk.n_sel * B * wk.sub);
+    if (pr.use_plane && !pr.plane_index) k_nn_knn<true><<<grid, kWarps * 32, 0, st>>>(pk, wk, pr, B, batch, lm_pos, lm_m);
+    else k_nn_knn<false><<<grid, kWarps * 32, 0, st>>>(pk, wk, pr, B, batch, lm_pos, lm_m);
     cudaError_t e = cudaGetLastError();
     if (e != cudaSuccess) return e;
     if (after_traversal && (e = cudaEventRecord(after_traversal, st)) != cudaSuccess) return e;
diff --git a/spatial-temporal-lidar-camera-calibration_b200/csrc/lm.cu b/spatial-temporal-lidar-camera-calibration_b200/csrc/lm.cu
--- a/spatial-temporal-lidar-camera-calibration_b200/csrc/lm.cu
+++ b/spatial-temporal-lidar-camera-calibration_b200/csrc/lm.cu
@@ -121,7 +121,8 @@
             m = wk.nb_m[slot];
             if (m < 0) continue;
         }
-        const double cx = (double)S.px[sp], cy = (double)S.py[sp], cz = (double)S.pz[sp];
+        const float4 r = S.pt4[sp];
+        const double cx = (double)r.x, cy = (double)r.y, cz = (double)r.z;
         const PlaneOut po = from_index ? plane_lookup(pk, K, sp)
                                        : plane_fit(NbCoords{wk.nbx + slot, wk.nbx_stride}, m, wk.nb_last[slot], cx, cy, cz, pr);
         if (!po.gates_ok) continue;
@@ -190,7 +191,8 @@
                 double ox, oy, oz;
                 xform(c0.Ri, c0.ti, ex, ey, ez, ox, oy, oz);
                 const double move = sqrt(dist3e(ox, oy, oz, qx, qy, qz)) * (1.0 + 1e-9) + 1e-12;
-                const double dh = dist3e(qx, qy, qz, (double)S.px[hint], (double)S.py[hint], (double)S.pz[hint]);
+                const float4 r = S.pt4[hint];
+                const double dh = dist3e(qx, qy, qz, (double)r.x, (double)r.y, (double)r.z);
                 const double reach = (double)__fsqrt_rd(nn_g2[slot]) - move;
                 if (reach > 0.0 && reach * reach > dh * (1.0 + 1e-6) + 1e-18) { settled = true; nn_pos = hint; nn_d = dh; }
             }
@@ -238,8 +240,8 @@
     const uint32_t np = lm.nnb_pos[slot];
     if (np == 0xffffffffu) return false;
     const DevKf &K = pk.kf[f];
-    const float *sx = pk.px + K.pt_off, *sy = pk.py + K.pt_off, *sz = pk.pz + K.pt_off;
-    const double nx = (double)sx[np], ny = (double)sy[np], nz = (double)sz[np];
+    const float4 r = pk.pt4[K.pt_off + np];
+    const double nx = (double)r.x, ny = (double)r.y, nz = (double)r.z;
     bool gates_ok, state;
     double n3[3];
     const int m = lm.nbb_m[slot];
```

Measured after the change: 1123 (median of 6 runs). +4.6%, better.
